# ooowedyn/InkLayer

Hardware: AMD Instinct MI355X
Metric: sketches/sec end-to-end (GroundingDINO+SAM) at 1024x1024 (higher is better)
Workload: dtype f16 (MFMA, f32 accumulate; f32 residual/norm/softmax; split-f16 = fp32-grade operands for patch-embed, neck, mask decoder); 1 GPU; full GroundingDINO Swin-T + SAM ViT-H pipeline, batch=8 per GPU, 1024x1024 synthetic sketches, 16 boxes/sketch, random-init weights; global_batch=8, parallelism=image-parallel x1

## Files before the change

### include/inklayer_hip.h

```cpp
#ifndef INKLAYER_HIP_H
#define INKLAYER_HIP_H

#include <stdint.h>

#ifdef __cplusplus
extern "C" {
#endif

#define INK_ABI_VERSION 10
int ink_abi_version(void);

typedef struct InkGemm {
  const void* A;
  const void* W;
  const float* bias;
  const float* col_scale;
  const float* residual;
  const int32_t* row_map;
  void* C;
  int32_t M, N, K;
  int32_t lda, ldw, ldr, ldc;
  int32_t act;
  int32_t c_f16;
} InkGemm;
#define INK_ACT_NONE 0
#define INK_ACT_GELU 1
#define INK_ACT_RELU 2
int ink_gemm_f16(const InkGemm* p, void* stream);
int ink_gemm_set_variant(int32_t v);
int ink_gemm_query_variant(int32_t M, int32_t N, int32_t K);

int ink_layernorm_rows(const float* x, int64_t ldx, const float* gamma, const float* beta,
                       float eps, const int32_t* gather, int32_t rows_out, int32_t C,
                       void* out_f16, float* out_f32, int64_t ldo, int32_t act, int32_t split,
                       const float* add, int64_t ld_add, const int32_t* add_batch_rows, int32_t rows_per_batch,
                       void* stream);

int ink_add_cvt_f16(const float* a, const float* b, int64_t n_b, void* out_f16, int64_t n,
                    void* stream);
int ink_add_split_f16(const float* a, const float* b, int64_t n_b, void* out_f16, int64_t n, int32_t C,
                      void* stream);
int ink_add_f32(const float* a, const float* b, int64_t n_b, float* out, int64_t n, void* stream);

typedef struct InkAttn {
  const void* Q; const void* K; const void* V;
  void* O;
  int64_t ldq, ldk, ldv, ldo;
  int32_t n_batch, n_heads, n_q, n_k, head_dim;
  float scale;
  int32_t bias_mode;
  int32_t grid_w;
  const int32_t* q_batch_rows;
  const int32_t* kv_batch_rows;
  const float* rel_h; const float* rel_w;
  const void* rel_aug;
  const float* dense_bias; const float* dense_mask;
  int32_t n_mask; int32_t rel_f16;
  const int32_t* tok_rows;
  const void* pad_k; const void* pad_v;
} InkAttn;
int ink_flash_attn(const InkAttn* p, void* stream);

int ink_swin_attn(const void* Q, const void* K, const void* V, int64_t ldq, int64_t ldk, int64_t ldv,
                  void* O, int64_t ldo, int32_t n_windows, int32_t n_heads, int32_t ws, float scale,
                  const float* bias_table, const uint8_t* region, int32_t nW, void* stream);

int ink_relpos_bias64_f16(const void* Q, int64_t ldq, const float* rel_pos_h, const float* rel_pos_w, int32_t n_batch,
                          int32_t n_heads, int32_t head_dim, float scale, void* out_h_f16, void* out_w_f16, void* stream);

int ink_relpos_bias(const void* Q, int64_t ldq, const float* rel_pos_h, const float* rel_pos_w,
                    int32_t S, int32_t n_batch, int32_t n_heads, int32_t head_dim, float scale,
                    const int32_t* tok_rows, float* out_h, float* out_w, void* out_aug_f16,
                    void* stream);

int ink_sam_patchify(const void* image_u8, int32_t h, int32_t w, int32_t L, int32_t P,
                     const float* mean3, const float* std3, int32_t chan_reverse, int32_t split,
                     void* out_f16, void* stream);

int ink_resize_u8(const void* src_u8, int32_t h, int32_t w, int32_t channels, void* dst_u8, int32_t oh, int32_t ow,
                  const int32_t* xbounds, const int32_t* xcoef, int32_t kx, const int32_t* ybounds,
                  const int32_t* ycoef, int32_t ky, void* tmp_u8, void* stream);

int ink_im2col3x3_f16(const void* in_f16, int32_t B, int32_t H, int32_t W, int32_t C, int32_t stride, int32_t relu,
                      void* out_f16, void* stream);

int ink_sam_pe_encode(const float* coords01, const float* gauss, int32_t N, int32_t F,
                      const float* add, int32_t n_add, float* out, void* stream);

int ink_sam_prompt_tokens(const float* points, const int32_t* labels, int32_t n_pts, int32_t pad, const float* boxes,
                          const float* gauss, int32_t F, const float* point_emb, const float* not_a_point,
                          const float* out_tok, float input_size, int32_t P, float* out, void* stream);

int ink_sam_mask_embed(const float* mask, const float* emb, const int32_t* emb_rows, const float* params,
                       int32_t n_params, float eps, int32_t P, int32_t g, float* keys, void* split_f16, void* stream);

int ink_sam_mask_logits(const float* up, const float* hyper, int32_t n, int32_t g, int32_t C,
                        float* out, void* stream);

int ink_sam_postprocess(const float* low, int32_t n, int32_t S, int32_t L, int32_t in_h,
                        int32_t in_w, int32_t out_h, int32_t out_w, float thr, void* out_u8,
                        float* out_logits, void* stream);

int ink_ms_deform_attn_forward(const float* value, const int64_t* spatial_shapes_host,
                               const int64_t* level_start_index_host, const float* sampling_loc,
                               const float* attn_weight, int32_t B, int32_t S, int32_t M, int32_t C,
                               int32_t Q, int32_t L, int32_t P, int32_t im2col_step, float* out,
                               void* stream);

int ink_ms_deform_attn_forward_dev(const void* value, const int64_t* spatial_shapes,
                                   const int64_t* level_start_index, const void* sampling_loc,
                                   const void* attn_weight, int32_t dtype, int32_t B, int32_t S, int32_t M,
                                   int32_t C, int32_t Q, int32_t L, int32_t P, int32_t im2col_step,
                                   void* out, void* stream);
int ink_ms_deform_attn_backward_dev(const void* value, const int64_t* spatial_shapes,
                                    const int64_t* level_start_index, const void* sampling_loc,
                                    const void* attn_weight, const void* grad_output, int32_t dtype,
                                    int32_t B, int32_t S, int32_t M, int32_t C, int32_t Q, int32_t L,
                                    int32_t P, int32_t im2col_step, void* grad_value,
                                    void* grad_sampling_loc, void* grad_attn_weight, void* stream);

int ink_msda_fused(const void* value_f16, const float* proj, int64_t ldp, const float* ref,
                   int32_t ref_dim, int64_t ref_q_stride, int64_t ref_b_stride,
                   const int32_t* shapes_host, int32_t B, int32_t S, int32_t Q, void* out_f16,
                   void* stream);

int ink_swin_patchify(const void* image_u8, int32_t h, int32_t w, const float* mean3,
                      const float* std3, void* out_f16, void* stream);

int ink_layernorm_merge4(const float* x, int64_t ldx, const float* gamma, const float* beta, float eps,
                         const int32_t* gather4, int32_t rows, int32_t C, void* out_f16, void* stream);

int ink_groupnorm_nhwc(const float* x, int32_t B, int32_t T, int32_t C, int32_t G, const float* gamma,
                       const float* beta, float eps, float* stats_ws, float* out,
                       int64_t out_batch_stride, void* stream);

int ink_gather_rows(const float* x, int64_t ldx, int64_t x_batch_rows, const int32_t* idx,
                    int64_t idx_batch_stride, int32_t rows_per_batch, int32_t B, int32_t C,
                    void* out_f16, float* out_f32, void* stream);

int ink_attn_fewkeys(const void* Q, int64_t ldq, const void* K, int64_t ldk, const void* V, int64_t ldv,
                     int32_t B, int32_t n_q, int32_t n_k, int32_t n_heads, int32_t head_dim, float scale,
                     const uint8_t* blocked, const int32_t* q_batch_rows, const float* q_add, int32_t io_f32, void* O,
                     int64_t ldo, void* stream);

int ink_attn_midkeys(const void* Q, int64_t ldq, const void* K, int64_t ldk, const void* V, int64_t ldv, int32_t B,
                     int32_t n_q, int32_t n_k, int32_t n_heads, int32_t head_dim, float scale, const uint8_t* blocked,
                     void* O, int64_t ldo, void* stream);

int ink_biattn_wide_workspace(int32_t B, int32_t S, int32_t T, int64_t* out_floats);
int ink_biattn_wide(const void* QV_f16, const void* KL_f16, int32_t B, int32_t S, int32_t T, int32_t E, float scale,
                    float* ws, void* out_v_f16, void* out_l_f16, void* stream);

int ink_biattn_wide_varlen(const void* QV_f16, const void* KL_f16, int32_t B, int32_t S, int32_t Tmax,
                           const int32_t* t_len , int32_t E, float scale, float* ws,
                           void* out_v_f16, void* out_l_f16 , void* stream);

int ink_attn_midkeys_varlen(const void* Q, int64_t ldq, const void* K, int64_t ldk, const void* V, int64_t ldv,
                            int32_t B, int32_t n_q, int32_t n_k, int32_t n_heads, int32_t head_dim, float scale,
                            const uint8_t* blocked, int64_t blocked_batch_stride, const int32_t* k_len,
                            void* O, int64_t ldo, void* stream);

int ink_text_embed_ln(const int32_t* ids, const int32_t* pos_ids, int32_t R, const float* word, int32_t V,
                      const float* pos, int32_t P, const float* type_row, const float* gamma, const float* beta,
                      float eps, int32_t C, float* out_f32, void* out_split_f16, void* stream);

int ink_attn_text_f32(const float* Q, int64_t ldq, const float* K, int64_t ldk, const float* V, int64_t ldv,
                      const int32_t* row_start , int32_t B, int32_t R, int32_t Tmax,
                      int32_t n_heads, int32_t head_dim, float scale, const uint8_t* blocked,
                      int64_t blocked_batch_stride, void* out_split_f16, int64_t ldo, float* out_f32, int64_t ldf,
                      void* stream);

int ink_attn_fewq(const void* Q, int64_t ldq, const void* K, int64_t ldk, const void* V, int64_t ldv,
                  int32_t n_batch, int32_t n_q, int32_t n_k, int32_t n_heads, int32_t head_dim, float scale,
                  const int32_t* q_batch_rows, const int32_t* kv_batch_rows, const float* k_add, void* O, int64_t ldo,
                  void* stream);

int ink_biattn_colstats(const float* scores, int32_t B, int32_t S, int32_t HT, float* part_ws, float* stats, void* stream);

int ink_fusion_fold_workspace(int32_t B, int32_t S, int64_t* out_floats);
int ink_fusion_fold(float* v_f32, int32_t B, int32_t S, const float* lnv_g, const float* lnv_b, float eps,
                    const float* text_k_f32, const float* text_vl_f32, int64_t ld_text, int32_t T, const void* Wq_f16,
                    const float* bq, const void* Wvv_f16, const float* bvv, const void* Wo_f16, const float* bo,
                    const float* gamma_v, float scale, float* ws, void* out_l_f16, const float* pos, void* out16_pos,
                    void* out16, void* stream);

int ink_sam_upscale_pack(const void* ws_f16, void* blob_f16, void* stream);
int ink_sam_upscale_tail(const float* u0, int64_t ld_tok, int32_t n, int32_t g, const float* ln_g, const float* ln_b, float eps,
                         const void* blob_f16, const float* b3, const float* hyper, int32_t n_masks, float* low,
                         void* stream);

int ink_proj256_ln_pack(const void* ws_f16, void* blob_f16, void* stream);
int ink_proj256_ln(const float* a_f32, const void* blob_f16, const float* bias, const float* res_f32,
                   const int32_t* res_batch_rows, int32_t rows_per_batch, const float* ln_g, const float* ln_b, float eps,
                   int64_t rows, float* out_f32, void* out_split_f16, void* stream);

int ink_ffn256_pack_bytes(int32_t hid, int32_t with_pre, int64_t* out_bytes);
int ink_ffn256_pack(const void* w1_f16, const float* b1, const void* w2_f16, int32_t hid, const void* wpre_f16, void* blob,
                    void* stream);
int ink_ffn256_fused(const void* x_f16, int64_t ldx, const float* res_f32, const void* blob, const float* b2,
                     const float* ln_g, const float* ln_b, float eps, int32_t M, int32_t hid, const float* pre_bias,
                     const float* pre_ln_g, const float* pre_ln_b, float* out_f32, void* stream);

int ink_topk_rowmax(const float* logits, int32_t B, int32_t S, int32_t T, int32_t K, int32_t* out_idx,
                    float* out_val, void* cand_ws, void* stream);

int ink_sine_embed4(const float* ref, const float* dim_t, int32_t N, void* out_f16, void* stream);

int ink_box_refine(const float* delta, int64_t ldd, const float* ref, int32_t N, int32_t ref_is_logit,
                   float* out, void* stream);

int ink_class_scores(const float* logits, int64_t ld_row, const float* pos_map, int64_t pm_image_stride,
                     const int32_t* n_cls, int32_t B, int32_t nq, int32_t T, int32_t C, float* out, void* stream);

int ink_select_boxes(const int32_t* idx, const float* boxes, const float* scale_wh, int32_t B, int32_t K, int32_t nq,
                     int32_t Cmax, float* out_boxes, int32_t* labels, int32_t* query, void* stream);

int ink_mask_cleanup_workspace_ints(int32_t n, int32_t H, int32_t W, int32_t k, int64_t* out_ints);
int ink_mask_cleanup(const void* masks_u8, int32_t n, int32_t H, int32_t W, int32_t k, int32_t area_threshold,
                     double aspect_threshold, void* tmp_a_u8, void* tmp_b_u8, int32_t* workspace, void* out_u8,
                     void* stream);

int ink_mask_sketch_iou_counts(const void* masks_u8, const void* sketch_rgb_u8, int32_t n, int32_t H, int32_t W,
                               void* bits_ws_u64, int32_t* counts, void* stream);

int ink_sam_amg_stats(const float* low, int32_t n, const int32_t* index, int32_t m, const int32_t* m_dev, int32_t S,
                      int32_t L, int32_t in_h, int32_t in_w, int32_t crop_h, int32_t crop_w, double thr, double offset,
                      int32_t x0, int32_t y0, int32_t orig_h, int32_t orig_w, int32_t* table, void* planes_u64,
                      float* out_logits, void* stream);

int ink_mask_rle_counts(const void* planes_u64, const int32_t* select, int32_t k, int32_t H, int32_t W,
                        int32_t* n_counts, void* stream);
int ink_mask_rle_write(const void* planes_u64, const int32_t* select, int32_t k, int32_t H, int32_t W,
                       const int32_t* offsets, int32_t* counts, void* stream);

int ink_mask_small_regions_workspace_ints(int32_t k, int32_t H, int32_t W, int64_t* out_ints);
int ink_mask_small_regions(const void* planes_u64, int32_t k, int32_t H, int32_t W, int32_t min_area, int32_t holes,
                           void* tmp_planes_u64, int32_t* workspace, void* out_planes_u64, int32_t* changed, void* stream);

int ink_box_nms(const float* boxes, const float* scores, int32_t n, float iou_threshold, void* workspace_u64,
                int32_t* keep, int32_t* n_keep, void* stream);

int ink_refine_sketch_planes(const void* rgb_u8, int32_t H, int32_t W, void* planes4_u64, int32_t* max_ws, void* stream);

int ink_bitplane_pack(const void* img_u8, int32_t n, int32_t H, int32_t W, int32_t thresh, void* planes_u64, void* stream);

int ink_refine_depth_samples(const void* mask_planes, int32_t n, const float* depth, const int32_t* pts_yx, int32_t P,
                             int32_t H, int32_t W, float* vals, void* inside_u8, void* stream);

int ink_refine_pair_tables(const void* mask_planes, const void* sketch_planes4, int32_t n, int32_t H, int32_t W,
                           const int32_t* rect, void* dil_ws_planes, int32_t* pair, int32_t* per_mask,
                           int32_t* sketch_area, void* stream);

int ink_refine_composite(const void* mask_planes, const int32_t* order, int32_t n_ranks, int32_t H, int32_t W,
                         void* label_u8, int32_t* hist256, void* stream);

int ink_refine_relabel_clean(const void* label_u8, const void* map256_u8, int32_t H, int32_t W, void* out_label_u8,
                             void* stream);

int ink_refine_grow_workspace(int32_t H, int32_t W, int64_t* plane_words, int64_t* cc_ints);
int ink_refine_grow(const void* label_u8, const void* sketch_planes4, int32_t H, int32_t W, void* planes_ws,
                    int32_t* cc_ws, int32_t* flags256, void* out_label_u8, int32_t* bbox256x4, int32_t* unl_yx,
                    int32_t unl_cap, int32_t* unl_count, void* stream);

int ink_refine_query_dists(const void* label_u8, const int32_t* q_yx, const void* cand256_bits, int32_t Q, int32_t H,
                           int32_t W, int32_t* d2_Qx256, void* stream);

int ink_refine_finalize(void* label_u8, const int32_t* assign_yxl, int32_t A, const void* sketch_planes4, int32_t H,
                        int32_t W, void* planes_ws3, void* extra_plane, int32_t* extra_count, void* stream);

int ink_host_sparse_sample(const uint8_t* rgb_u8, int32_t H, int32_t W, int32_t* out_yx, int32_t cap, int32_t* count);
int ink_host_assign_unlabeled(const int32_t* q_yx, int32_t Q, const int32_t* boxes, int32_t nb, const int32_t* box2mask,
                              const int32_t* d2, const uint8_t* nonempty, int32_t n_masks, int32_t* out_label);

int ink_depth_patchify(const void* image_u8, int32_t H, int32_t W, int32_t nh, int32_t nw, int32_t P, int32_t KP,
                       const double* mean3, const double* std3, int32_t chan_reverse, void* out_f16, void* stream);

int ink_resize_bilinear_ac_nhwc(const float* in, int32_t B, int32_t h, int32_t w, int32_t C, int32_t H, int32_t W,
                                float* out_f32, void* out_f16, void* stream);

int ink_conv3x3_f16(const void* in_f16, int32_t B, int32_t H, int32_t W, int32_t C, const void* wt_f16, int32_t N,
                    const float* bias, int32_t stride, int32_t relu_in, int32_t act, const float* residual, void* out,
                    int32_t out_f16, void* stream);

int ink_layers_otsu_planes(const void* gray_u8, int32_t n, int32_t H, int32_t W, int32_t invert, int32_t* hist,
                           int32_t* thresh, void* out_planes, void* stream);

int ink_layers_dilate(const void* planes, int32_t n, int32_t H, int32_t W, int32_t kernel_size, int32_t iterations,
                      void* tmp_planes, void* out_planes, void* stream);

int ink_layers_border_band(const void* planes, int32_t n, int32_t H, int32_t W, int32_t band, int32_t* flags,
                           void* stream);

int ink_layers_components_workspace_ints(int32_t n, int32_t H, int32_t W, int64_t* out_ints);
int ink_layers_components(const void* planes, int32_t n, int32_t H, int32_t W, int32_t mode, void* tmp_planes3,
                          int32_t* workspace, void* out_planes, void* stream);

int ink_layers_chamfer_workspace_ints(int32_t n, int32_t H, int32_t W, int64_t* out_ints);
int ink_layers_chamfer(const void* mask_planes, const void* stroke_planes, int32_t n, int32_t H, int32_t W,
                       int32_t safety_margin, int32_t full, int32_t* dist, int32_t* workspace, int32_t* min_out,
                       int32_t* shrink_out, void* out_planes, void* stream);

int ink_layers_mask_tables(const void* masks_u8, int32_t n, int32_t H, int32_t W, int32_t* bbox, int32_t* overlap,
                           void* stream);

int ink_layers_assemble(const void* sketch_rgb_u8, const void* masks_u8, const void* bg_planes, const int32_t* bbox,
                        const int32_t* overlap, int32_t n, int32_t H, int32_t W, void* sketch_layers_u8,
                        void* edit_masks_u8, void* debug_u8, void* stream);

int ink_layers_composite(const void* inpainted_rgb_u8, const void* sketch_layer_u8, int32_t H, int32_t W,
                         void* out_rgb_u8, void* stream);

int ink_layers_gray(const void* rgb_u8, int32_t n, int32_t H, int32_t W, void* gray_u8, void* stream);

int ink_layers_rgba(const void* gray_u8, const void* bg_planes, int32_t n, int32_t H, int32_t W, void* rgba_u8,
                    void* stream);


int ink_inp_contrast(const void* rgb_u8, int32_t H, int32_t W, float factor, void* sum_u64, void* out_rgb_u8,
                     void* stream);

int ink_inp_bilateral(const void* rgb_u8, int32_t H, int32_t W, const float* tables, void* out_rgb_u8, void* stream);

int ink_inp_mask_prepare(const void* mask_u8, int32_t H, int32_t W, int32_t dilate_iterations, int32_t blur,
                         void* tmp2_u8, void* out_u8, void* stream);

int ink_inp_condition(const void* rgb_u8, const void* mask_u8, int32_t H, int32_t W, float* out_f32, void* stream);

int ink_inp_cleanup(const void* result_rgb_u8, int32_t H, int32_t W, const float* taps11, float* tmp_f32,
                    void* thresh_u8, void* clean_rgb_u8, void* stream);

int ink_inp_soft_blend(const void* clean_rgb_u8, const void* original_rgb_u8, const void* mask_u8, int32_t H, int32_t W,
                       const double* taps2, double* tmp_f64, void* out_rgb_u8, void* stream);

int ink_inp_luma(const void* rgb_u8, int32_t H, int32_t W, int32_t out_channels, void* out_u8, void* stream);

int ink_inp_unsharp(const void* img_u8, int32_t H, int32_t W, int32_t channels, uint32_t ww, uint32_t fw,
                    int32_t percent, int32_t threshold, void* tmp2_u8, void* out_u8, void* stream);

int ink_inp_rgba_cut(const void* rgb_u8, const void* mask_u8, int32_t H, int32_t W, void* rgba_u8, void* stream);


int ink_vis_gray_min(const void* sketch_u8, int32_t channels, int32_t H, int32_t W, int32_t* gray_min, void* stream);
// ... 23 lines not shown
```

### inklayer_amd/_lib.py

```python
from __future__ import annotations

import ctypes as C
import os
from pathlib import Path

_LIB_PATH = Path(__file__).resolve().parent / "lib" / "libinklayer_hip.so"
_lib = None

c_void_p, c_int, c_i64, c_float = C.c_void_p, C.c_int32, C.c_int64, C.c_float


class InkGemm(C.Structure):
    _fields_ = [
        ("A", c_void_p), ("W", c_void_p), ("bias", c_void_p), ("col_scale", c_void_p),
        ("residual", c_void_p), ("row_map", c_void_p), ("C", c_void_p),
        ("M", c_int), ("N", c_int), ("K", c_int),
        ("lda", c_int), ("ldw", c_int), ("ldr", c_int), ("ldc", c_int),
        ("act", c_int), ("c_f16", c_int),
    ]


class InkAttn(C.Structure):
    _fields_ = [
        ("Q", c_void_p), ("K", c_void_p), ("V", c_void_p), ("O", c_void_p),
        ("ldq", c_i64), ("ldk", c_i64), ("ldv", c_i64), ("ldo", c_i64),
        ("n_batch", c_int), ("n_heads", c_int), ("n_q", c_int), ("n_k", c_int),
        ("head_dim", c_int), ("scale", c_float), ("bias_mode", c_int), ("grid_w", c_int),
        ("q_batch_rows", c_void_p), ("kv_batch_rows", c_void_p),
        ("rel_h", c_void_p), ("rel_w", c_void_p), ("rel_aug", c_void_p),
        ("dense_bias", c_void_p), ("dense_mask", c_void_p), ("n_mask", c_int), ("rel_f16", c_int),
        ("tok_rows", c_void_p), ("pad_k", c_void_p), ("pad_v", c_void_p),
    ]


SIGNATURES = {
    "ink_abi_version": [],
    "ink_gemm_f16": [C.POINTER(InkGemm), c_void_p],
    "ink_gemm_set_variant": [c_int],
    "ink_gemm_query_variant": [c_int, c_int, c_int],
    "ink_layernorm_rows": [c_void_p, c_i64, c_void_p, c_void_p, c_float, c_void_p, c_int, c_int,
                           c_void_p, c_void_p, c_i64, c_int, c_int, c_void_p, c_i64, c_void_p, c_int, c_void_p],
    "ink_add_split_f16": [c_void_p, c_void_p, c_i64, c_void_p, c_i64, c_int, c_void_p],
    "ink_add_cvt_f16": [c_void_p, c_void_p, c_i64, c_void_p, c_i64, c_void_p],
    "ink_add_f32": [c_void_p, c_void_p, c_i64, c_void_p, c_i64, c_void_p],
    "ink_flash_attn": [C.POINTER(InkAttn), c_void_p],
    "ink_swin_attn": [c_void_p, c_void_p, c_void_p, c_i64, c_i64, c_i64, c_void_p, c_i64, c_int, c_int, c_int, c_float,
                      c_void_p, c_void_p, c_int, c_void_p],
    "ink_sam_patchify": [c_void_p, c_int, c_int, c_int, c_int, C.POINTER(c_float), C.POINTER(c_float),
                         c_int, c_int, c_void_p, c_void_p],
    "ink_im2col3x3_f16": [c_void_p, c_int, c_int, c_int, c_int, c_int, c_int, c_void_p, c_void_p],
    "ink_resize_u8": [c_void_p, c_int, c_int, c_int, c_void_p, c_int, c_int, c_void_p, c_void_p, c_int,
                      c_void_p, c_void_p, c_int, c_void_p, c_void_p],
    "ink_sam_pe_encode": [c_void_p, c_void_p, c_int, c_int, c_void_p, c_int, c_void_p, c_void_p],
    "ink_sam_mask_logits": [c_void_p, c_void_p, c_int, c_int, c_int, c_void_p, c_void_p],
    "ink_sam_prompt_tokens": [c_void_p, c_void_p, c_int, c_int, c_void_p, c_void_p, c_int, c_void_p, c_void_p,
                              c_void_p, c_float, c_int, c_void_p, c_void_p],
    "ink_sam_mask_embed": [c_void_p, c_void_p, c_void_p, c_void_p, c_int, c_float, c_int, c_int, c_void_p, c_void_p,
                           c_void_p],
    "ink_sam_postprocess": [c_void_p, c_int, c_int, c_int, c_int, c_int, c_int, c_int, c_float,
                            c_void_p, c_void_p, c_void_p],
    "ink_sam_amg_stats": [c_void_p, c_int, c_void_p, c_int, c_void_p, c_int, c_int, c_int, c_int, c_int, c_int, C.c_double,
                          C.c_double, c_int, c_int, c_int, c_int, c_void_p, c_void_p, c_void_p, c_void_p],
    "ink_mask_rle_counts": [c_void_p, c_void_p, c_int, c_int, c_int, c_void_p, c_void_p],
    "ink_mask_rle_write": [c_void_p, c_void_p, c_int, c_int, c_int, c_void_p, c_void_p, c_void_p],
    "ink_mask_small_regions_workspace_ints": [c_int, c_int, c_int, C.POINTER(c_i64)],
    "ink_mask_small_regions": [c_void_p, c_int, c_int, c_int, c_int, c_int, c_void_p, c_void_p, c_void_p, c_void_p,
                               c_void_p],
    "ink_box_nms": [c_void_p, c_void_p, c_int, c_float, c_void_p, c_void_p, c_void_p, c_void_p],
    "ink_ms_deform_attn_forward": [c_void_p, C.POINTER(c_i64), C.POINTER(c_i64), c_void_p, c_void_p, c_int,
                                   c_int, c_int, c_int, c_int, c_int, c_int, c_int, c_void_p, c_void_p],
    "ink_ms_deform_attn_forward_dev": [c_void_p, c_void_p, c_void_p, c_void_p, c_void_p, c_int, c_int, c_int, c_int,
                                       c_int, c_int, c_int, c_int, c_int, c_void_p, c_void_p],
    "ink_ms_deform_attn_backward_dev": [c_void_p, c_void_p, c_void_p, c_void_p, c_void_p, c_void_p, c_int, c_int, c_int,
                                        c_int, c_int, c_int, c_int, c_int, c_int, c_void_p, c_void_p, c_void_p,
                                        c_void_p],
    "ink_msda_fused": [c_void_p, c_void_p, c_i64, c_void_p, c_int, c_i64, c_i64, C.POINTER(c_int), c_int,
                       c_int, c_int, c_void_p, c_void_p],
    "ink_swin_patchify": [c_void_p, c_int, c_int, C.POINTER(c_float), C.POINTER(c_float), c_void_p, c_void_p],
    "ink_layernorm_merge4": [c_void_p, c_i64, c_void_p, c_void_p, c_float, c_void_p, c_int, c_int, c_void_p,
                             c_void_p],
    "ink_groupnorm_nhwc": [c_void_p, c_int, c_int, c_int, c_int, c_void_p, c_void_p, c_float, c_void_p,
                           c_void_p, c_i64, c_void_p],
    "ink_gather_rows": [c_void_p, c_i64, c_i64, c_void_p, c_i64, c_int, c_int, c_int, c_void_p, c_void_p,
                        c_void_p],
    "ink_biattn_colstats": [c_void_p, c_int, c_int, c_int, c_void_p, c_void_p, c_void_p],
    "ink_fusion_fold_workspace": [c_int, c_int, C.POINTER(c_i64)],
    "ink_relpos_bias64_f16": [c_void_p, c_i64, c_void_p, c_void_p, c_int, c_int, c_int, c_float, c_void_p, c_void_p, c_void_p],
    "ink_proj256_ln_pack": [c_void_p, c_void_p, c_void_p],
    "ink_proj256_ln": [c_void_p, c_void_p, c_void_p, c_void_p, c_void_p, c_int, c_void_p, c_void_p, c_float, c_i64, c_void_p,
                       c_void_p, c_void_p],
    "ink_sam_upscale_pack": [c_void_p, c_void_p, c_void_p],
    "ink_sam_upscale_tail": [c_void_p, c_i64, c_int, c_int, c_void_p, c_void_p, c_float, c_void_p, c_void_p, c_void_p,
                             c_int, c_void_p, c_void_p],
    "ink_ffn256_pack_bytes": [c_int, c_int, C.POINTER(c_i64)],
    "ink_ffn256_pack": [c_void_p, c_void_p, c_void_p, c_int, c_void_p, c_void_p, c_void_p],
    "ink_ffn256_fused": [c_void_p, c_i64, c_void_p, c_void_p, c_void_p, c_void_p, c_void_p, c_float, c_int, c_int,
                         c_void_p, c_void_p, c_void_p, c_void_p, c_void_p],
    "ink_fusion_fold": [c_void_p, c_int, c_int, c_void_p, c_void_p, c_float, c_void_p, c_void_p, c_i64, c_int, c_void_p,
                        c_void_p, c_void_p, c_void_p, c_void_p, c_void_p, c_void_p, c_float, c_void_p, c_void_p, c_void_p,
                        c_void_p, c_void_p, c_void_p],
    "ink_attn_fewkeys": [c_void_p, c_i64, c_void_p, c_i64, c_void_p, c_i64, c_int, c_int, c_int, c_int, c_int,
                         c_float, c_void_p, c_void_p, c_void_p, c_int, c_void_p, c_i64, c_void_p],
    "ink_attn_midkeys": [c_void_p, c_i64, c_void_p, c_i64, c_void_p, c_i64, c_int, c_int, c_int, c_int, c_int,
                         c_float, c_void_p, c_void_p, c_i64, c_void_p],
    "ink_biattn_wide_workspace": [c_int, c_int, c_int, C.POINTER(c_i64)],
    "ink_biattn_wide": [c_void_p, c_void_p, c_int, c_int, c_int, c_int, c_float, c_void_p, c_void_p, c_void_p,
                        c_void_p],
    "ink_biattn_wide_varlen": [c_void_p, c_void_p, c_int, c_int, c_int, c_void_p, c_int, c_float, c_void_p, c_void_p,
                               c_void_p, c_void_p],
    "ink_attn_midkeys_varlen": [c_void_p, c_i64, c_void_p, c_i64, c_void_p, c_i64, c_int, c_int, c_int, c_int, c_int,
                                c_float, c_void_p, c_i64, c_void_p, c_void_p, c_i64, c_void_p],
    "ink_text_embed_ln": [c_void_p, c_void_p, c_int, c_void_p, c_int, c_void_p, c_int, c_void_p, c_void_p, c_void_p,
                          c_float, c_int, c_void_p, c_void_p, c_void_p],
    "ink_attn_text_f32": [c_void_p, c_i64, c_void_p, c_i64, c_void_p, c_i64, c_void_p, c_int, c_int, c_int, c_int, c_int,
                          c_float, c_void_p, c_i64, c_void_p, c_i64, c_void_p, c_i64, c_void_p],
    "ink_attn_fewq": [c_void_p, c_i64, c_void_p, c_i64, c_void_p, c_i64, c_int, c_int, c_int, c_int, c_int,
                      c_float, c_void_p, c_void_p, c_void_p, c_void_p, c_i64, c_void_p],
    "ink_topk_rowmax": [c_void_p, c_int, c_int, c_int, c_int, c_void_p, c_void_p, c_void_p, c_void_p],
    "ink_class_scores": [c_void_p, c_i64, c_void_p, c_i64, c_void_p, c_int, c_int, c_int, c_int, c_void_p, c_void_p],
    "ink_select_boxes": [c_void_p, c_void_p, c_void_p, c_int, c_int, c_int, c_int, c_void_p, c_void_p, c_void_p,
                         c_void_p],
    "ink_sine_embed4": [c_void_p, c_void_p, c_int, c_void_p, c_void_p],
    "ink_box_refine": [c_void_p, c_i64, c_void_p, c_int, c_int, c_void_p, c_void_p],
    "ink_mask_cleanup_workspace_ints": [c_int, c_int, c_int, c_int, C.POINTER(c_i64)],
    "ink_mask_cleanup": [c_void_p, c_int, c_int, c_int, c_int, c_int, C.c_double, c_void_p, c_void_p, c_void_p,
                         c_void_p, c_void_p],
    "ink_mask_sketch_iou_counts": [c_void_p, c_void_p, c_int, c_int, c_int, c_void_p, c_void_p, c_void_p],
    "ink_refine_sketch_planes": [c_void_p, c_int, c_int, c_void_p, c_void_p, c_void_p],
    "ink_bitplane_pack": [c_void_p, c_int, c_int, c_int, c_int, c_void_p, c_void_p],
    "ink_refine_depth_samples": [c_void_p, c_int, c_void_p, c_void_p, c_int, c_int, c_int, c_void_p, c_void_p, c_void_p],
    "ink_refine_pair_tables": [c_void_p, c_void_p, c_int, c_int, c_int, c_void_p, c_void_p, c_void_p, c_void_p,
                               c_void_p, c_void_p],
    "ink_refine_composite": [c_void_p, c_void_p, c_int, c_int, c_int, c_void_p, c_void_p, c_void_p],
    "ink_refine_relabel_clean": [c_void_p, c_void_p, c_int, c_int, c_void_p, c_void_p],
    "ink_refine_grow_workspace": [c_int, c_int, C.POINTER(c_i64), C.POINTER(c_i64)],
    "ink_refine_grow": [c_void_p, c_void_p, c_int, c_int, c_void_p, c_void_p, c_void_p, c_void_p, c_void_p, c_void_p,
                        c_int, c_void_p, c_void_p],
    "ink_refine_query_dists": [c_void_p, c_void_p, c_void_p, c_int, c_int, c_int, c_void_p, c_void_p],
    "ink_refine_finalize": [c_void_p, c_void_p, c_int, c_void_p, c_int, c_int, c_void_p, c_void_p, c_void_p, c_void_p],
    "ink_host_sparse_sample": [c_void_p, c_int, c_int, c_void_p, c_int, c_void_p],
    "ink_host_assign_unlabeled": [c_void_p, c_int, c_void_p, c_int, c_void_p, c_void_p, c_void_p, c_int, c_void_p],
    "ink_depth_patchify": [c_void_p, c_int, c_int, c_int, c_int, c_int, c_int, C.POINTER(C.c_double), C.POINTER(C.c_double),
                           c_int, c_void_p, c_void_p],
    "ink_resize_bilinear_ac_nhwc": [c_void_p, c_int, c_int, c_int, c_int, c_int, c_int, c_void_p, c_void_p, c_void_p],
    "ink_conv3x3_f16": [c_void_p, c_int, c_int, c_int, c_int, c_void_p, c_int, c_void_p, c_int, c_int, c_int, c_void_p,
                        c_void_p, c_int, c_void_p],
    "ink_layers_otsu_planes": [c_void_p, c_int, c_int, c_int, c_int, c_void_p, c_void_p, c_void_p, c_void_p],
    "ink_layers_dilate": [c_void_p, c_int, c_int, c_int, c_int, c_int, c_void_p, c_void_p, c_void_p],
    "ink_layers_border_band": [c_void_p, c_int, c_int, c_int, c_int, c_void_p, c_void_p],
    "ink_layers_components_workspace_ints": [c_int, c_int, c_int, C.POINTER(c_i64)],
    "ink_layers_components": [c_void_p, c_int, c_int, c_int, c_int, c_void_p, c_void_p, c_void_p, c_void_p],
    "ink_layers_chamfer_workspace_ints": [c_int, c_int, c_int, C.POINTER(c_i64)],
    "ink_layers_chamfer": [c_void_p, c_void_p, c_int, c_int, c_int, c_int, c_int, c_void_p, c_void_p, c_void_p, c_void_p,
                           c_void_p, c_void_p],
    "ink_layers_mask_tables": [c_void_p, c_int, c_int, c_int, c_void_p, c_void_p, c_void_p],
    "ink_layers_assemble": [c_void_p, c_void_p, c_void_p, c_void_p, c_void_p, c_int, c_int, c_int, c_void_p, c_void_p,
                            c_void_p, c_void_p],
    "ink_layers_composite": [c_void_p, c_void_p, c_int, c_int, c_void_p, c_void_p],
    "ink_layers_gray": [c_void_p, c_int, c_int, c_int, c_void_p, c_void_p],
    "ink_layers_rgba": [c_void_p, c_void_p, c_int, c_int, c_int, c_void_p, c_void_p],
    "ink_inp_contrast": [c_void_p, c_int, c_int, c_float, c_void_p, c_void_p, c_void_p],
    "ink_inp_bilateral": [c_void_p, c_int, c_int, c_void_p, c_void_p, c_void_p],
    "ink_inp_mask_prepare": [c_void_p, c_int, c_int, c_int, c_int, c_void_p, c_void_p, c_void_p],
    "ink_inp_condition": [c_void_p, c_void_p, c_int, c_int, c_void_p, c_void_p],
    "ink_inp_cleanup": [c_void_p, c_int, c_int, c_void_p, c_void_p, c_void_p, c_void_p, c_void_p],
    "ink_inp_soft_blend": [c_void_p, c_void_p, c_void_p, c_int, c_int, c_void_p, c_void_p, c_void_p, c_void_p],
    "ink_inp_luma": [c_void_p, c_int, c_int, c_int, c_void_p, c_void_p],
    "ink_inp_unsharp": [c_void_p, c_int, c_int, c_int, C.c_uint32, C.c_uint32, c_int, c_int, c_void_p, c_void_p, c_void_p],
    "ink_inp_rgba_cut": [c_void_p, c_void_p, c_int, c_int, c_void_p, c_void_p],
    "ink_vis_gray_min": [c_void_p, c_int, c_int, c_int, c_void_p, c_void_p],
    "ink_vis_colour": [c_void_p, c_int, c_void_p, c_int, c_int, c_void_p, c_void_p, c_int, c_int, c_void_p, c_void_p],
    "ink_eval_label_ranks": [c_void_p, c_int, c_int, c_int, c_void_p, c_void_p, c_int, c_void_p, c_void_p, c_void_p],
    "ink_eval_contingency": [c_void_p, c_int, c_int, c_void_p, c_int, c_void_p, c_int, c_int, c_int, c_int, c_void_p,
                             c_void_p],
    "ink_eval_label_boxes": [c_void_p, c_int, c_int, c_int, c_void_p, c_void_p],
    "ink_eval_paint_labels": [c_void_p, c_void_p, c_int, c_int, c_int, c_void_p, c_void_p],
    "ink_relpos_bias": [c_void_p, c_i64, c_void_p, c_void_p, c_int, c_int, c_int, c_int, c_float,
                        c_void_p, c_void_p, c_void_p, c_void_p, c_void_p],
}


class InkLayerHipError(RuntimeError):
    pass


def lib_path() -> Path:
    return Path(os.environ.get("INKLAYER_HIP_LIB", _LIB_PATH))


def lib() -> C.CDLL:
    global _lib
    if _lib is None:
        p = lib_path()
        if not p.exists():
            raise InkLayerHipError(
                f"{p} not found: build it with `python -m inklayer_amd.build` "
                "(there is no CPU/eager fallback for the InkLayer hot path)")
        try:
            import torch
        except ImportError:
            pass
        l = C.CDLL(str(p))
        for name, argtypes in SIGNATURES.items():
            fn = getattr(l, name)
            fn.argtypes = argtypes
            fn.restype = C.c_int
        _lib = l
    return _lib


def check(rc: int, what: str) -> None:
    if rc != 0:
        raise InkLayerHipError(f"{what} failed: " + {1: "bad argument", 2: "HIP launch error"}.get(rc, str(rc)))
```

### inklayer_amd/csrc/gemm.hip

```cpp
#include <stdlib.h>

#include "mfma_util.h"
#include "../../include/inklayer_hip.h"

namespace {

template <int BK> struct Swz;
template <> struct Swz<64> {
  static __device__ __forceinline__ int f(int row) { return row & 7; }
};
template <> struct Swz<32> {
  static __device__ __forceinline__ int f(int row) { return (-(row >> 2)) & 3; }
};

__device__ __forceinline__ bool residual_preloaded(const InkGemm& p) {
  return p.residual && p.act == INK_ACT_NONE && !p.col_scale;
}

template <int TM>
__device__ __forceinline__ void wave_rows(int (&rows)[TM], const InkGemm& p, int mw, int lane) {
#pragma unroll
  for (int ti = 0; ti < TM; ++ti) {
    const int m = mw + ti * 16 + (lane & 15);
    int r = -1;
    if (m < p.M) r = p.row_map ? p.row_map[m] : m;
    rows[ti] = r;
  }
}

template <int TM, int TN>
__device__ __forceinline__ void init_wave_tile(f32x4 (&acc)[TM][TN], const InkGemm& p, const int (&rows)[TM], int nw,
                                               int lane) {
  const int fq = lane >> 4;
  const bool pre = residual_preloaded(p);
#pragma unroll
  for (int ti = 0; ti < TM; ++ti) {
    const int r = pre ? rows[ti] : -1;
    const float* rp = p.residual + (size_t)max(r, 0) * p.ldr + nw + fq * 4;
#pragma unroll
    for (int j = 0; j < TN; ++j) {
      acc[ti][j] = (f32x4){0.f, 0.f, 0.f, 0.f};
      if (r >= 0 && nw + j * 16 + fq * 4 < p.N) acc[ti][j] = *(const f32x4*)(rp + j * 16);
    }
  }
}

template <int TM, int TN>
__device__ __forceinline__ void add_bias_wave_tile(f32x4 (&acc)[TM][TN], const InkGemm& p, int nw, int lane) {
  const int fq = lane >> 4;
#pragma unroll
  for (int j = 0; j < TN; ++j) {
    const int n = nw + j * 16 + fq * 4;
    f32x4 bv = (f32x4){0.f, 0.f, 0.f, 0.f};
    if (p.bias && n < p.N) bv = *(const f32x4*)(p.bias + n);
#pragma unroll
    for (int ti = 0; ti < TM; ++ti) acc[ti][j] += bv;
  }
}

template <int TM, int TN, int OUT, int MODE = -1>
__device__ __forceinline__ void store_wave_tile(f32x4 (&acc)[TM][TN], const InkGemm& p, char* er,
                                                const int (&rows)[TM], int nw, int lane) {
  constexpr bool F16O = OUT == 1;
  constexpr int WNC = TN * 16, EP = WNC * 4 + 16;
  constexpr int ES = OUT == 0 ? 4 : 8;
  constexpr int CPRW = WNC / ES;
  constexpr int NIT = (16 * CPRW + 63) / 64;
  const int fr = lane & 15, fq = lane >> 4;
  const bool wide16 = OUT != 0 && (p.ldc % 8 == 0);
  const bool res_late = MODE < 0 && p.residual && !residual_preloaded(p);
  const int act = MODE < 0 ? p.act : MODE;
  const bool scaled = MODE < 0 && p.col_scale != nullptr;
  int row_of[NIT], n_of[NIT];
#pragma unroll
  for (int it = 0; it < NIT; ++it) {
    const int c = it * 64 + lane;
    row_of[it] = c < 16 * CPRW ? c / CPRW : 16;
    n_of[it] = nw + (c % CPRW) * ES;
  }

  add_bias_wave_tile<TM, TN>(acc, p, nw, lane);

#pragma unroll
  for (int ti = 0; ti < TM; ++ti) {
#pragma unroll
    for (int j = 0; j < TN; ++j) {
      f32x4 v = acc[ti][j];
      if (act == INK_ACT_GELU) {
#pragma unroll
        for (int r = 0; r < 4; ++r) v[r] = gelu_erf(v[r]);
      } else if (act == INK_ACT_RELU) {
#pragma unroll
        for (int r = 0; r < 4; ++r) v[r] = fmaxf(v[r], 0.f);
      }
      if (scaled) {
        const int n = nw + j * 16 + fq * 4;
        if (n < p.N) v *= *(const f32x4*)(p.col_scale + n);
      }
      if (F16O) {
        *(f16x4*)(er + fr * EP + (j * 16 + fq * 4) * 2) = (f16x4){(f16)v[0], (f16)v[1], (f16)v[2], (f16)v[3]};
      } else {
        *(f32x4*)(er + fr * EP + (j * 16 + fq * 4) * 4) = v;
      }
    }
#pragma unroll
    for (int it = 0; it < NIT; ++it) {
      int r = __builtin_amdgcn_ds_bpermute((row_of[it] & 15) << 2, rows[ti]);
      if (row_of[it] >= 16 || n_of[it] >= p.N) r = -1;
      if (r >= 0) {
        const int c_n = n_of[it];
        const char* src = er + row_of[it] * EP + (c_n - nw) * (F16O ? 2 : 4);
        if (F16O) {
          f16x8 d = *(const f16x8*)src;
          f16* dst = (f16*)p.C + (size_t)r * p.ldc + c_n;
          if (res_late) {
            const float* rp = p.residual + (size_t)r * p.ldr + c_n;
#pragma unroll
            for (int e = 0; e < 8; ++e)
              if (c_n + e < p.N) d[e] = (f16)((float)d[e] + rp[e]);
          }
          if (wide16 && c_n + 8 <= p.N) {
            *(f16x8*)dst = d;
          } else {
            *(f16x4*)dst = (f16x4){d[0], d[1], d[2], d[3]};
            if (c_n + 8 <= p.N) *(f16x4*)(dst + 4) = (f16x4){d[4], d[5], d[6], d[7]};
          }
        } else {
          f32x4 d = *(const f32x4*)src;
          if (res_late) d += *(const f32x4*)(p.residual + (size_t)r * p.ldr + c_n);
          *(f32x4*)((float*)p.C + (size_t)r * p.ldc + c_n) = d;
        }
      }
    }
  }
}

__device__ __forceinline__ void tile_of(int id, int ntm, int ntn, int group_m, int& mt, int& nt) {
  if (group_m > 1) {
    const int per = group_m * ntn;
    const int first = (id / per) * group_m;
    const int gsz = min(ntm - first, group_m);
    mt = first + (id % per) % gsz;
    nt = (id % per) / gsz;
  } else {
    mt = id / ntn;
    nt = id % ntn;
  }
}

constexpr int NS = 2;
template <int BM, int BN, int BK, int WM, int WN>
__global__ __launch_bounds__(WM * WN * 64) void gemm_f16_nt(InkGemm p, int group_m) {
  constexpr int NT = WM * WN * 64;
  constexpr int CPR = BK / 8;
  constexpr int ROWB = BK * 2;
  constexpr int TILE_A = BM * ROWB, TILE_W = BN * ROWB;
  constexpr int STAGE = TILE_A + TILE_W;
  constexpr int IT_A = (BM * CPR) / NT, IT_W = (BN * CPR) / NT;
  constexpr int TM = BM / WM / 16, TN = BN / WN / 16;
  static_assert((BM * CPR) % NT == 0 && (BN * CPR) % NT == 0, "tile/threads mismatch");
  extern __shared__ __attribute__((aligned(16))) char smem[];

  const int tid = threadIdx.x;
  const int lane = tid & 63;
  const int wave = tid >> 6;
  const int wm = wave / WN, wn = wave % WN;

  const int ntn = (p.N + BN - 1) / BN;
  const int ntm = (p.M + BM - 1) / BM;
  int mt, nt;
  tile_of(xcd_remap(blockIdx.x, ntm * ntn), ntm, ntn, group_m, mt, nt);
  const int m0 = mt * BM;
  const int n0 = nt * BN;

  const f16* __restrict__ A = (const f16*)p.A;
  const f16* __restrict__ W = (const f16*)p.W;

  const f16* srcA[IT_A];
  const f16* srcW[IT_W];
#pragma unroll
  for (int it = 0; it < IT_A; ++it) {
    const int pch = it * NT + tid;
    const int row = pch / CPR;
    const int lch = (pch % CPR) ^ Swz<BK>::f(row);
    srcA[it] = A + (size_t)min(m0 + row, p.M - 1) * p.lda + lch * 8;
  }
#pragma unroll
  for (int it = 0; it < IT_W; ++it) {
    const int pch = it * NT + tid;
    const int row = pch / CPR;
    const int lch = (pch % CPR) ^ Swz<BK>::f(row);
    srcW[it] = W + (size_t)min(n0 + row, p.N - 1) * p.ldw + lch * 8;
  }

  auto stage = [&](int buf, int kt) {
    char* base = smem + buf * STAGE;
#pragma unroll
    for (int it = 0; it < IT_A; ++it)
      __builtin_amdgcn_global_load_lds((gptr_t)(srcA[it] + kt * BK), (lptr_t)(base + (it * NT + wave * 64) * 16), 16, 0, 0);
#pragma unroll
    for (int it = 0; it < IT_W; ++it)
      __builtin_amdgcn_global_load_lds((gptr_t)(srcW[it] + kt * BK), (lptr_t)(base + TILE_A + (it * NT + wave * 64) * 16), 16, 0, 0);
  };

  int rows[TM];
  wave_rows<TM>(rows, p, m0 + wm * (BM / WM), lane);
  f32x4 acc[TM][TN];

  const int fr = lane & 15, fq = lane >> 4;
  const int offA = (wm * (BM / WM) + fr) * ROWB;
  const int offW = (wn * (BN / WN) + fr) * ROWB;
  const int swz = Swz<BK>::f(fr);

  const int nk = p.K / BK;
  auto compute = [&](int cur) {
    const char* bA = smem + cur * STAGE;
    const char* bW = bA + TILE_A;
#pragma unroll
    for (int kk = 0; kk < BK / 32; ++kk) {
      constexpr int AG = TM > 4 ? 4 : TM;
      f16x8 a[AG], w[TN];
      const int co = ((kk * 4 + fq) ^ swz) << 4;
#pragma unroll
      for (int j = 0; j < TN; ++j) w[j] = *(const f16x8*)(bW + offW + j * 16 * ROWB + co);
#pragma unroll
      for (int i0 = 0; i0 < TM; i0 += AG) {
#pragma unroll
        for (int i = 0; i < AG; ++i) a[i] = *(const f16x8*)(bA + offA + (i0 + i) * 16 * ROWB + co);
#pragma unroll
        for (int i = 0; i < AG; ++i)
#pragma unroll
          for (int j = 0; j < TN; ++j)
            acc[i0 + i][j] = __builtin_amdgcn_mfma_f32_16x16x32_f16(w[j], a[i], acc[i0 + i][j], 0, 0, 0);
      }
    }
  };

  stage(0, 0);
  init_wave_tile<TM, TN>(acc, p, rows, n0 + wn * (BN / WN), lane);
  for (int kt = 0; kt < nk; ++kt) {
    asm volatile("s_waitcnt vmcnt(0)" ::: "memory");
    __syncthreads();
    if (kt + 1 < nk) stage((kt + 1) & 1, kt + 1);
    compute(kt & 1);
  }

  constexpr int WNC = BN / WN;
  constexpr int EP = WNC * 4 + 16;
  static_assert(WM * WN * 16 * EP <= NS * STAGE, "epilogue patch must fit in the staging LDS");
  __syncthreads();
  char* er = smem + wave * (16 * EP);
  if (p.c_f16 == 1) {
    store_wave_tile<TM, TN, 1>(acc, p, er, rows, n0 + wn * WNC, lane);
  } else {
    store_wave_tile<TM, TN, 0>(acc, p, er, rows, n0 + wn * WNC, lane);
  }
}

constexpr int PP_RING = 4, PP_TN = 5;
__global__ __launch_bounds__(512) void gemm_f16_nt_pp(InkGemm p, int group_m) {
  constexpr int RING = PP_RING, TN = PP_TN;
  constexpr int BM = 256, BN = 64 * TN, BK = 32, NT = 512;
  constexpr int CPR = BK / 8, ROWB = BK * 2;
  constexpr int TILE_A = BM * ROWB, TILE_W = BN * ROWB, GRAN = TILE_A + TILE_W;
  constexpr int IT_A = (BM * CPR) / NT, IT_W = (BN * CPR) / NT;
  constexpr bool W_TAIL = (BN * CPR) % NT != 0;
  static_assert(!W_TAIL || (BN * CPR) % NT == NT / 2, "tail is exactly the first four waves");
  constexpr int LOADS = IT_A + IT_W;
  constexpr int TM = 8, WNC = 16 * TN;
  constexpr int AHEAD = RING - 2;
  constexpr int AG = 4;
  constexpr int EP = WNC * 4 + 16;
  static_assert(8 * 16 * EP <= RING * GRAN, "patch fits");
  extern __shared__ __attribute__((aligned(16))) char smem[];
  const int tid = threadIdx.x, lane = tid & 63;
  const int wave = __builtin_amdgcn_readfirstlane(tid >> 6);
  const int grp = wave >> 2, wn = wave & 3;
  const int fr = lane & 15, fq = lane >> 4;

  const int ntn = (p.N + BN - 1) / BN, ntm = (p.M + BM - 1) / BM;
  int mt, nt;
  tile_of(xcd_remap(blockIdx.x, ntm * ntn), ntm, ntn, group_m, mt, nt);
  const int m0 = mt * BM, n0 = nt * BN;
  const int G = p.K / BK;
  const f16* __restrict__ A = (const f16*)p.A;
  const f16* __restrict__ W = (const f16*)p.W;
  const f16* srcA[IT_A];
  const f16* srcW[IT_W + (W_TAIL ? 1 : 0)];
#pragma unroll
  for (int it = 0; it < IT_A; ++it) {
    const int pch = it * NT + tid, row = pch / CPR, lch = (pch % CPR) ^ Swz<BK>::f(row);
    srcA[it] = A + (size_t)min(m0 + row, p.M - 1) * p.lda + lch * 8;
  }
#pragma unroll
  for (int it = 0; it < IT_W + (W_TAIL ? 1 : 0); ++it) {
    const int pch = it * NT + tid, row = min(pch / CPR, BN - 1), lch = (pch % CPR) ^ Swz<BK>::f(row);
    srcW[it] = W + (size_t)min(n0 + row, p.N - 1) * p.ldw + lch * 8;
  }
  auto dma = [&](int g, int slot) {
    char* base = smem + slot * GRAN;
#pragma unroll
    for (int it = 0; it < IT_A; ++it)
      __builtin_amdgcn_global_load_lds((gptr_t)(srcA[it] + g * BK), (lptr_t)(base + (it * NT + wave * 64) * 16), 16, 0, 0);
#pragma unroll
    for (int it = 0; it < IT_W; ++it)
      __builtin_amdgcn_global_load_lds((gptr_t)(srcW[it] + g * BK), (lptr_t)(base + TILE_A + (it * NT + wave * 64) * 16), 16, 0, 0);
    if (W_TAIL && grp == 0)
      __builtin_amdgcn_global_load_lds((gptr_t)(srcW[IT_W] + g * BK), (lptr_t)(base + TILE_A + (IT_W * NT + wave * 64) * 16), 16, 0, 0);
  };
  auto wait_ahead = [&]() {
    if (W_TAIL && grp == 0) {
      asm volatile("s_waitcnt vmcnt(%0)" ::"n"((AHEAD - 1) * (LOADS + 1)) : "memory");
    } else {
      asm volatile("s_waitcnt vmcnt(%0)" ::"n"((AHEAD - 1) * LOADS) : "memory");
    }
  };
  auto slot_end = [&]() {
    __builtin_amdgcn_sched_barrier(0);
    __builtin_amdgcn_s_barrier();
    __builtin_amdgcn_sched_barrier(0);
  };

  int rows[TM];
  wave_rows<TM>(rows, p, m0 + grp * 128, lane);
#pragma unroll
  for (int g = 0; g < AHEAD; ++g) dma(g, g);
  f32x4 acc[TM][TN];
  init_wave_tile<TM, TN>(acc, p, rows, n0 + wn * WNC, lane);
  if (residual_preloaded(p)) {
    asm volatile("s_waitcnt vmcnt(0)" ::: "memory");
  } else {
    wait_ahead();
  }
  slot_end();
  if (grp == 1) slot_end();

  const int offA = (grp * 128 + fr) * ROWB;
  const int offW = (wn * WNC + fr) * ROWB;
  const int co = (fq ^ Swz<BK>::f(fr)) << 4;
  f16x8 a[AG], w[TN];
  int cslot = 0, islot = AHEAD % RING;
  auto iter = [&](int g) __attribute__((always_inline)) {
    const char* bA = smem + cslot * GRAN;
    const char* bW = bA + TILE_A;
#pragma unroll
    for (int i = 0; i < AG; ++i) a[i] = *(const f16x8*)(bA + offA + i * 16 * ROWB + co);
#pragma unroll
    for (int j = 0; j < TN; ++j) w[j] = *(const f16x8*)(bW + offW + j * 16 * ROWB + co);
    if (g + AHEAD < G) {
      dma(g + AHEAD, islot);
      wait_ahead();
    } else {
      asm volatile("s_waitcnt vmcnt(0)" ::: "memory");
    }
    slot_end();
    asm volatile("s_waitcnt lgkmcnt(0)" ::: "memory");
    __builtin_amdgcn_sched_barrier(0);
    __builtin_amdgcn_s_setprio(1);
#pragma unroll
    for (int i0 = 0; i0 < TM; i0 += AG) {
#pragma unroll
      for (int i = 0; i < AG; ++i) {
#pragma unroll
        for (int j = 0; j < TN; ++j)
          acc[i0 + i][j] = __builtin_amdgcn_mfma_f32_16x16x32_f16(w[j], a[i], acc[i0 + i][j], 0, 0, 0);
        if (i0 + AG < TM) {
          a[i] = *(const f16x8*)(bA + offA + (i0 + AG + i) * 16 * ROWB + co);
          __builtin_amdgcn_sched_barrier(0);
        }
      }
    }
    __builtin_amdgcn_s_setprio(0);
    slot_end();
    cslot = (cslot + 1 == RING) ? 0 : cslot + 1;
    islot = (islot + 1 == RING) ? 0 : islot + 1;
  };
  for (int g = 0; g < G; ++g) iter(g);
  if (grp == 0) slot_end();

  char* er = smem + wave * (16 * EP);
  const bool plain = !p.col_scale && !(p.residual && !residual_preloaded(p));
  if (p.c_f16) {
    if (plain && p.act == INK_ACT_GELU) {
      store_wave_tile<TM, TN, 1, INK_ACT_GELU>(acc, p, er, rows, n0 + wn * WNC, lane);
    } else if (plain && p.act == INK_ACT_NONE) {
      store_wave_tile<TM, TN, 1, INK_ACT_NONE>(acc, p, er, rows, n0 + wn * WNC, lane);
    } else {
      store_wave_tile<TM, TN, 1>(acc, p, er, rows, n0 + wn * WNC, lane);
    }
  } else {
    if (plain && p.act == INK_ACT_NONE) {
      store_wave_tile<TM, TN, 0, INK_ACT_NONE>(acc, p, er, rows, n0 + wn * WNC, lane);
    } else {
      store_wave_tile<TM, TN, 0>(acc, p, er, rows, n0 + wn * WNC, lane);
    }
  }
}

static int launch_gemm_pp(const InkGemm& p, hipStream_t s, int group_m) {
  if (p.K / 32 < PP_RING) return INK_ERR_ARG;
  constexpr int BN = 64 * PP_TN;
  constexpr int lds = PP_RING * (256 + BN) * 32 * 2;
  static_assert(lds <= 160 * 1024, "LDS budget");
  ink_dyn_lds<gemm_f16_nt_pp>(lds);
  const int ntiles = ((p.M + 255) / 256) * ((p.N + BN - 1) / BN);
  hipLaunchKernelGGL(gemm_f16_nt_pp, dim3(ntiles), dim3(512), lds, s, p, group_m);
  return ink_launch_status();
}

template <int BM, int BN, int BK, int WM, int WN>
static int launch_gemm(const InkGemm& p, hipStream_t s, int group_m = 1) {
  constexpr int lds = NS * (BM + BN) * BK * 2;
  static_assert(lds <= 160 * 1024, "LDS budget");
  ink_dyn_lds<gemm_f16_nt<BM, BN, BK, WM, WN>>(lds);
  const int ntm = (p.M + BM - 1) / BM, ntn = (p.N + BN - 1) / BN;
  hipLaunchKernelGGL((gemm_f16_nt<BM, BN, BK, WM, WN>), dim3(ntm * ntn), dim3(WM * WN * 64), lds, s, p, group_m);
  return ink_launch_status();
}

struct ConvGeom {
  int H, W, C, OH, OW, stride;
};
__device__ __attribute__((aligned(128))) const uint32_t g_conv_zero_row[32] = {};

template <int BK, bool RELU_IN>
__global__ __launch_bounds__(256) void conv3x3_f16_nt(InkGemm p, ConvGeom g) {
  constexpr int BM = 128, BN = 128, WM = 2, WN = 2;
  constexpr int NT = WM * WN * 64;
  constexpr int CPR = BK / 8;
  constexpr int ROWB = BK * 2;
  constexpr int TILE_A = BM * ROWB, TILE_W = BN * ROWB;
  constexpr int STAGE = TILE_A + TILE_W;
  constexpr int IT_A = (BM * CPR) / NT, IT_W = (BN * CPR) / NT;
  constexpr int TM = BM / WM / 16, TN = BN / WN / 16;
  extern __shared__ __attribute__((aligned(16))) char smem[];

  const int tid = threadIdx.x;
  const int lane = tid & 63;
  const int wave = tid >> 6;
  const int wm = wave / WN, wn = wave % WN;

  const int ntn = (p.N + BN - 1) / BN;
  const int ntm = (p.M + BM - 1) / BM;
  int mt, nt;
  tile_of(xcd_remap(blockIdx.x, ntm * ntn), ntm, ntn, 1, mt, nt);
  const int m0 = mt * BM;
  const int n0 = nt * BN;

  const f16* __restrict__ A = (const f16*)p.A;
  const f16* __restrict__ W = (const f16*)p.W;

  const f16* ctrA[IT_A];
  const f16* zeroA[IT_A];
  int maskA[IT_A];
  const f16* srcW[IT_W];
#pragma unroll
  for (int it = 0; it < IT_A; ++it) {
    const int pch = it * NT + tid;
    const int row = pch / CPR;
    const int lch = (pch % CPR) ^ Swz<BK>::f(row);
    const int m = min(m0 + row, p.M - 1);
    const int b = m / (g.OH * g.OW);
    const int rem = m - b * (g.OH * g.OW);
    const int oy = rem / g.OW;
    const int iy = oy * g.stride, ix = (rem - oy * g.OW) * g.stride;
    ctrA[it] = A + (((size_t)b * g.H + iy) * g.W + ix) * g.C + lch * 8;
    zeroA[it] = (const f16*)g_conv_zero_row + lch * 8;
    const int rowok = (iy > 0 ? 1 : 0) | 2 | (iy + 1 < g.H ? 4 : 0);
    const int colok = (ix > 0 ? 1 : 0) | 2 | (ix + 1 < g.W ? 4 : 0);
    int mask = 0;
#pragma unroll
    for (int ky = 0; ky < 3; ++ky)
      if ((rowok >> ky) & 1) mask |= colok << (ky * 3);
    maskA[it] = mask;
  }
#pragma unroll
  for (int it = 0; it < IT_W; ++it) {
    const int pch = it * NT + tid;
    const int row = pch / CPR;
    const int lch = (pch % CPR) ^ Swz<BK>::f(row);
    srcW[it] = W + (size_t)min(n0 + row, p.N - 1) * p.ldw + lch * 8;
  }

  int s_tap = 0, s_c0 = 0;
  auto stage = [&](int buf, int kt) {
    char* base = smem + buf * STAGE;
    const int ky = s_tap / 3, kx = s_tap - ky * 3;
    const ptrdiff_t doff = ((ptrdiff_t)(ky - 1) * g.W + (kx - 1)) * g.C + s_c0;
#pragma unroll
    for (int it = 0; it < IT_A; ++it) {
      const f16* src = ((maskA[it] >> s_tap) & 1) ? ctrA[it] + doff : zeroA[it];
      __builtin_amdgcn_global_load_lds((gptr_t)src, (lptr_t)(base + (it * NT + wave * 64) * 16), 16, 0, 0);
    }
#pragma unroll
    for (int it = 0; it < IT_W; ++it)
      __builtin_amdgcn_global_load_lds((gptr_t)(srcW[it] + kt * BK), (lptr_t)(base + TILE_A + (it * NT + wave * 64) * 16), 16, 0, 0);
    s_c0 += BK;
    if (s_c0 == g.C) {
      s_c0 = 0;
      ++s_tap;
    }
  };

  int rows[TM];
  wave_rows<TM>(rows, p, m0 + wm * (BM / WM), lane);
  f32x4 acc[TM][TN];

  const int fr = lane & 15, fq = lane >> 4;
  const int offA = (wm * (BM / WM) + fr) * ROWB;
  const int offW = (wn * (BN / WN) + fr) * ROWB;
  const int swz = Swz<BK>::f(fr);

  const int nk = p.K / BK;
  auto compute = [&](int cur) {
    const char* bA = smem + cur * STAGE;
    const char* bW = bA + TILE_A;
#pragma unroll
    for (int kk = 0; kk < BK / 32; ++kk) {
      f16x8 a[TM], w[TN];
      const int co = ((kk * 4 + fq) ^ swz) << 4;
#pragma unroll
      for (int j = 0; j < TN; ++j) w[j] = *(const f16x8*)(bW + offW + j * 16 * ROWB + co);
#pragma unroll
      for (int i = 0; i < TM; ++i) {
        a[i] = *(const f16x8*)(bA + offA + i * 16 * ROWB + co);
        if (RELU_IN) a[i] = __builtin_elementwise_max(a[i], (f16x8)(f16)0);
      }
#pragma unroll
      for (int i = 0; i < TM; ++i)
#pragma unroll
        for (int j = 0; j < TN; ++j)
          acc[i][j] = __builtin_amdgcn_mfma_f32_16x16x32_f16(w[j], a[i], acc[i][j], 0, 0, 0);
    }
  };

  stage(0, 0);
  init_wave_tile<TM, TN>(acc, p, rows, n0 + wn * (BN / WN), lane);
  for (int kt = 0; kt < nk; ++kt) {
    asm volatile("s_waitcnt vmcnt(0)" ::: "memory");
    __syncthreads();
    if (kt + 1 < nk) stage((kt + 1) & 1, kt + 1);
    compute(kt & 1);
  }

  constexpr int WNC = BN / WN;
  constexpr int EP = WNC * 4 + 16;
  static_assert(WM * WN * 16 * EP <= NS * STAGE, "epilogue patch must fit in the staging LDS");
  __syncthreads();
  char* er = smem + wave * (16 * EP);
  if (p.c_f16 == 1) {
    store_wave_tile<TM, TN, 1>(acc, p, er, rows, n0 + wn * WNC, lane);
  } else {
    store_wave_tile<TM, TN, 0>(acc, p, er, rows, n0 + wn * WNC, lane);
  }
}

template <int BK, bool RELU_IN>
static int launch_conv3x3(const InkGemm& p, const ConvGeom& g, hipStream_t s) {
  constexpr int lds = NS * (128 + 128) * BK * 2;
  ink_dyn_lds<conv3x3_f16_nt<BK, RELU_IN>>(lds);
  const int ntm = (p.M + 127) / 128, ntn = (p.N + 127) / 128;
  hipLaunchKernelGGL((conv3x3_f16_nt<BK, RELU_IN>), dim3(ntm * ntn), dim3(256), lds, s, p, g);
  return ink_launch_status();
}

}

extern "C" int ink_conv3x3_f16(const void* in_f16, int32_t B, int32_t H, int32_t W, int32_t C, const void* wt_f16,
                               int32_t N, const float* bias, int32_t stride, int32_t relu_in, int32_t act,
                               const float* residual, void* out, int32_t out_f16, void* stream) {
  INK_CHECK_ARG(in_f16 && wt_f16 && out);
  INK_CHECK_ARG(B > 0 && H > 0 && W > 0 && C > 0 && N > 0);
  INK_CHECK_ARG(C % 32 == 0 && N % 4 == 0);
  INK_CHECK_ARG(stride == 1 || stride == 2);
  INK_CHECK_ARG(ink_aligned<16>(in_f16, wt_f16, out, residual, bias));
  INK_CHECK_ARG(relu_in == 0 || relu_in == 1);
  INK_CHECK_ARG(act == INK_ACT_NONE || act == INK_ACT_RELU);
  INK_CHECK_ARG(out_f16 == 0 || out_f16 == 1);
  const int OH = (H - 1) / stride + 1, OW = (W - 1) / stride + 1;
  const int64_t M = (int64_t)B * OH * OW;
  INK_CHECK_ARG(M <= INT32_MAX - 128 && (int64_t)9 * C <= INT32_MAX);
  InkGemm p = {};
  p.A = in_f16;
  p.W = wt_f16;
  p.bias = bias;
  p.residual = residual;
  p.C = out;
  p.M = (int32_t)M;
  p.N = N;
  p.K = 9 * C;
  p.lda = p.ldw = 9 * C;
  p.ldr = p.ldc = N;
  p.act = act;
  p.c_f16 = out_f16;
  const ConvGeom g = {H, W, C, OH, OW, stride};
  hipStream_t s = (hipStream_t)stream;
  if (C % 64 == 0) return relu_in ? launch_conv3x3<64, true>(p, g, s) : launch_conv3x3<64, false>(p, g, s);
  return relu_in ? launch_conv3x3<32, true>(p, g, s) : launch_conv3x3<32, false>(p, g, s);
}

static int g_variant = -1;
extern "C" int ink_gemm_query_variant(int32_t M, int32_t N, int32_t K) {
  if (K % 64 != 0) return 32;
  if (N % 320 == 0 && K >= 128 && (long)((M + 255) / 256) * (N / 320) >= 384) return 45;
  const long tiles256 = (long)((M + 255) / 256) * ((N + 255) / 256);
  const bool n_fits = (N % 256 == 0) || N >= 1024;
  return (tiles256 >= 200 && n_fits) ? 10 : 0;
}
extern "C" int ink_abi_version(void) { return INK_ABI_VERSION; }
extern "C" int ink_gemm_set_variant(int32_t v) {
  INK_CHECK_ARG(v == -1 || v == 0 || v == 10 || v == 45);
  g_variant = v;
  return INK_OK;
}

extern "C" int ink_gemm_f16(const InkGemm* pp, void* stream) {
  INK_CHECK_ARG(pp != nullptr);
  const InkGemm& p = *pp;
  INK_CHECK_ARG(p.A && p.W && p.C);
  INK_CHECK_ARG(p.M > 0 && p.N > 0 && p.K > 0);
  INK_CHECK_ARG(p.K % 32 == 0 && p.N % 4 == 0);
  INK_CHECK_ARG(p.lda % 8 == 0 && p.ldw % 8 == 0 && p.lda >= p.K && p.ldw >= p.K);
  INK_CHECK_ARG(p.ldc % 4 == 0 && p.ldc >= p.N);
  INK_CHECK_ARG(!p.residual || (p.ldr % 4 == 0 && p.ldr >= p.N));
  INK_CHECK_ARG(ink_aligned<16>(p.A, p.W, p.C));
  INK_CHECK_ARG(p.act >= 0 && p.act <= 2);
  INK_CHECK_ARG(p.c_f16 == 0 || p.c_f16 == 1);
  hipStream_t s = (hipStream_t)stream;
  if (p.K % 64 != 0) return launch_gemm<128, 128, 32, 2, 2>(p, s);
  int v = g_variant;
  if (v < 0) v = ink_gemm_query_variant(p.M, p.N, p.K);
  switch (v) {
    case 10: return launch_gemm<256, 256, 64, 4, 4>(p, s, 4);
    case 45: return launch_gemm_pp(p, s, 4);
    default: return launch_gemm<128, 128, 64, 2, 2>(p, s);
  }
}
```

### inklayer_amd/csrc/norm.hip

```cpp
#include "common.h"
#include "../../include/inklayer_hip.h"

namespace {

template <int NV>
__global__ __launch_bounds__(256) void layernorm_rows_kernel(
    const float* __restrict__ x, int64_t ldx, const float* __restrict__ gamma,
    const float* __restrict__ beta, float eps, const int32_t* __restrict__ gather, int rows_out,
    int C, f16* __restrict__ out_h, float* __restrict__ out_f, int64_t ldo, int act, int split,
    const float* __restrict__ add, int64_t ld_add, const int32_t* __restrict__ add_batch_rows, int rows_per_batch) {
  const int lane = threadIdx.x & 63;
  const int row = blockIdx.x * 4 + (threadIdx.x >> 6);
  if (row >= rows_out) return;
  const int nv = C >> 2;
  const int64_t ldf = split ? ldo / 3 : ldo;
  const int src = gather ? gather[row] : row;
  if (src < 0) {
    for (int v = lane; v < nv; v += 64) {
      if (out_h && split) split_store(out_h + row * ldo + v * 4, C, (f32x4){0.f, 0.f, 0.f, 0.f});
      else if (out_h) *(f16x4*)(out_h + row * ldo + v * 4) = (f16x4){0, 0, 0, 0};
      if (out_f) *(f32x4*)(out_f + row * ldf + v * 4) = (f32x4){0.f, 0.f, 0.f, 0.f};
    }
    return;
  }
  const float* xr = x + (int64_t)src * ldx;
  const float* ar = nullptr;
  if (add) {
    const int b = row / rows_per_batch, i = row - b * rows_per_batch;
    ar = add + ((int64_t)(add_batch_rows ? add_batch_rows[b] : b * rows_per_batch) + i) * ld_add;
  }
  f32x4 r[NV];
  float s = 0.f;
#pragma unroll
  for (int j = 0; j < NV; ++j) {
    const int v = lane + 64 * j;
    r[j] = v < nv ? *(const f32x4*)(xr + v * 4) : (f32x4){0.f, 0.f, 0.f, 0.f};
    if (ar && v < nv) r[j] += *(const f32x4*)(ar + v * 4);
    s += (r[j][0] + r[j][1]) + (r[j][2] + r[j][3]);
  }
  const float mean = wave_sum(s) / (float)C;
  float q = 0.f;
#pragma unroll
  for (int j = 0; j < NV; ++j) {
    const int v = lane + 64 * j;
    if (v < nv) {
      const f32x4 d = r[j] - mean;
      q += (d[0] * d[0] + d[1] * d[1]) + (d[2] * d[2] + d[3] * d[3]);
    }
  }
  const float rstd = 1.0f / sqrtf(wave_sum(q) / (float)C + eps);
#pragma unroll
  for (int j = 0; j < NV; ++j) {
    const int v = lane + 64 * j;
    if (v < nv) {
      f32x4 y = (r[j] - mean) * rstd;
      if (gamma) y *= *(const f32x4*)(gamma + v * 4);
      if (beta) y += *(const f32x4*)(beta + v * 4);
      if (act == INK_ACT_GELU) {
#pragma unroll
        for (int e = 0; e < 4; ++e) y[e] = gelu_erf(y[e]);
      }
      if (out_h && split) split_store(out_h + row * ldo + v * 4, C, y);
      else if (out_h) *(f16x4*)(out_h + row * ldo + v * 4) = (f16x4){(f16)y[0], (f16)y[1], (f16)y[2], (f16)y[3]};
      if (out_f) *(f32x4*)(out_f + row * ldf + v * 4) = y;
    }
  }
}

__global__ __launch_bounds__(256) void add_split_f16_kernel(const float* __restrict__ a,
                                                            const float* __restrict__ b,
                                                            f16* __restrict__ o, int64_t n4, int64_t nb4,
                                                            int C) {
  const int c4n = C >> 2;
  for (int64_t i = blockIdx.x * 256 + threadIdx.x; i < n4; i += (int64_t)gridDim.x * 256) {
    f32x4 v = *(const f32x4*)(a + i * 4);
    if (b) v += *(const f32x4*)(b + (i % nb4) * 4);
    const int64_t row = i / c4n;
    const int c = (int)(i - row * c4n) * 4;
    split_store(o + row * 3 * C + c, C, v);
  }
}

__global__ __launch_bounds__(256) void add_cvt_f16_kernel(const float* __restrict__ a,
                                                          const float* __restrict__ b,
                                                          f16* __restrict__ o,
                                                          float* __restrict__ of, int64_t n4,
                                                          int64_t nb4) {
  for (int64_t i = blockIdx.x * 256 + threadIdx.x; i < n4; i += (int64_t)gridDim.x * 256) {
    f32x4 v = *(const f32x4*)(a + i * 4);
    if (b) v += *(const f32x4*)(b + (i % nb4) * 4);
    if (o) *(f16x4*)(o + i * 4) = (f16x4){(f16)v[0], (f16)v[1], (f16)v[2], (f16)v[3]};
    if (of) *(f32x4*)(of + i * 4) = v;
  }
}

}

extern "C" int ink_layernorm_rows(const float* x, int64_t ldx, const float* gamma,
                                  const float* beta, float eps, const int32_t* gather,
                                  int32_t rows_out, int32_t C, void* out_f16, float* out_f32,
                                  int64_t ldo, int32_t act, int32_t split, const float* add, int64_t ld_add,
                                  const int32_t* add_batch_rows, int32_t rows_per_batch, void* stream) {
  INK_CHECK_ARG(x && (out_f16 || out_f32));
  INK_CHECK_ARG(!add || (!gather && rows_per_batch > 0 && ld_add >= C && ld_add % 4 == 0));
  INK_CHECK_ARG(split == 0 || (split == 1 && out_f16 && ldo >= 3 * (int64_t)C && (!out_f32 || ldo % 12 == 0)));
  INK_CHECK_ARG(act == INK_ACT_NONE || act == INK_ACT_GELU);
  INK_CHECK_ARG(rows_out > 0 && C > 0 && C % 4 == 0 && C <= 2048);
  INK_CHECK_ARG(ldx % 4 == 0 && ldo % 4 == 0 && ldx >= C && ldo >= C);
  const dim3 grid((rows_out + 3) / 4), block(256);
  hipStream_t s = (hipStream_t)stream;
  const int nv = (C / 4 + 63) / 64;
#define INK_LN(NV)                                                                          \
  hipLaunchKernelGGL(layernorm_rows_kernel<NV>, grid, block, 0, s, x, ldx, gamma, beta, eps, \
                     gather, rows_out, C, (f16*)out_f16, out_f32, ldo, act, split, add, ld_add, add_batch_rows, \
                     rows_per_batch)
  switch (nv) {
    case 1: INK_LN(1); break;
    case 2: INK_LN(2); break;
    case 3: INK_LN(3); break;
    case 4: INK_LN(4); break;
    case 5: INK_LN(5); break;
    default: INK_LN(8); break;
  }
#undef INK_LN
  return ink_launch_status();
}

extern "C" int ink_add_cvt_f16(const float* a, const float* b, int64_t n_b, void* out_f16,
                               int64_t n, void* stream) {
  INK_CHECK_ARG(a && out_f16 && n > 0 && n % 4 == 0);
  INK_CHECK_ARG(!b || (n_b > 0 && n_b % 4 == 0 && n % n_b == 0));
  const int64_t n4 = n / 4;
  const int blocks = (int)((n4 + 255) / 256 < 2048 ? (n4 + 255) / 256 : 2048);
  hipLaunchKernelGGL(add_cvt_f16_kernel, dim3(blocks), dim3(256), 0, (hipStream_t)stream, a, b,
                     (f16*)out_f16, (float*)nullptr, n4, b ? n_b / 4 : 1);
  return ink_launch_status();
}

extern "C" int ink_add_split_f16(const float* a, const float* b, int64_t n_b, void* out_f16, int64_t n,
                                 int32_t C, void* stream) {
  INK_CHECK_ARG(a && out_f16 && n > 0 && C > 0 && C % 4 == 0 && n % C == 0);
  INK_CHECK_ARG(!b || (n_b > 0 && n_b % 4 == 0 && n % n_b == 0));
  const int64_t n4 = n / 4;
  const int blocks = (int)((n4 + 255) / 256 < 4096 ? (n4 + 255) / 256 : 4096);
  hipLaunchKernelGGL(add_split_f16_kernel, dim3(blocks), dim3(256), 0, (hipStream_t)stream, a, b,
                     (f16*)out_f16, n4, b ? n_b / 4 : 1, C);
  return ink_launch_status();
}

extern "C" int ink_add_f32(const float* a, const float* b, int64_t n_b, float* out, int64_t n,
                           void* stream) {
  INK_CHECK_ARG(a && out && n > 0 && n % 4 == 0);
  INK_CHECK_ARG(!b || (n_b > 0 && n_b % 4 == 0 && n % n_b == 0));
  const int64_t n4 = n / 4;
  const int blocks = (int)((n4 + 255) / 256 < 2048 ? (n4 + 255) / 256 : 2048);
  hipLaunchKernelGGL(add_cvt_f16_kernel, dim3(blocks), dim3(256), 0, (hipStream_t)stream, a, b,
                     (f16*)nullptr, out, n4, b ? n_b / 4 : 1);
  return ink_launch_status();
}
```

### inklayer_amd/gdino.py

```python
from __future__ import annotations

import math
from dataclasses import dataclass, replace
from typing import Dict, List, NamedTuple, Optional, Sequence, Tuple

import numpy as np
import torch

from . import ops
from ._lru import LRU

F16, F32, I32 = torch.float16, torch.float32, torch.int32


@dataclass
class GDinoConfig:
    embed_dim: int = 96
    depths: Tuple[int, ...] = (2, 2, 6, 2)
    num_heads: Tuple[int, ...] = (3, 6, 12, 24)
    window_size: int = 7
    out_indices: Tuple[int, ...] = (1, 2, 3)
    hidden_dim: int = 256
    nheads: int = 8
    enc_layers: int = 6
# ... 2 lines not shown
    num_queries: int = 900
    num_feature_levels: int = 4
    n_points: int = 4
    max_text_len: int = 256
    pe_temperature: float = 20.0
    box_threshold: float = 0.2
    pixel_mean: Tuple[float, ...] = (0.485, 0.456, 0.406)
    pixel_std: Tuple[float, ...] = (0.229, 0.224, 0.225)


GDINO_CONFIGS: Dict[str, GDinoConfig] = {
    "swin_T_224_1k": GDinoConfig(),
    "swin_B_224_22k": GDinoConfig(embed_dim=128, depths=(2, 2, 18, 2), num_heads=(4, 8, 16, 32), window_size=7),
    "swin_B_384_22k": GDinoConfig(embed_dim=128, depths=(2, 2, 18, 2), num_heads=(4, 8, 16, 32), window_size=12),
}
GDINO_ALIASES = {"swin_t": "swin_T_224_1k", "swin_b": "swin_B_384_22k"}
WINDOW_SIZES = (7, 12)
HEAD_DIM = 32


def config_for(name: str) -> GDinoConfig:
    key = GDINO_ALIASES.get(name, name)
    if key not in GDINO_CONFIGS:
        raise ValueError(f"unknown GroundingDINO model {name!r}: one of {sorted(GDINO_CONFIGS) + sorted(GDINO_ALIASES)}")
    return replace(GDINO_CONFIGS[key])


def model_name(cfg: GDinoConfig) -> Optional[str]:
    key = (cfg.embed_dim, tuple(cfg.depths), tuple(cfg.num_heads), cfg.window_size)
    return next((n for n, c in GDINO_CONFIGS.items()
                 if (c.embed_dim, tuple(c.depths), tuple(c.num_heads), c.window_size) == key), None)


def check_config(cfg: GDinoConfig) -> None:
    widths = [cfg.embed_dim * 2 ** i / nh for i, nh in enumerate(cfg.num_heads)]
    if len(cfg.depths) != len(cfg.num_heads) or any(wd != HEAD_DIM for wd in widths):
        raise ValueError(f"no kernels for this Swin backbone: head widths {widths} (embed dim {cfg.embed_dim}, heads "
                         f"{tuple(cfg.num_heads)}, depths {tuple(cfg.depths)}); the window attention kernels serve head "
                         f"width {HEAD_DIM}")
    if cfg.window_size not in WINDOW_SIZES:
        raise ValueError(f"no kernels for this Swin backbone: window size {cfg.window_size}; the window attention "
                         f"kernels serve {' and '.join(map(str, WINDOW_SIZES))}")
    if cfg.embed_dim * 2 ** (len(cfg.depths) - 1) > 2048:
        raise ValueError(f"no kernels for this Swin backbone: {cfg.embed_dim * 2 ** (len(cfg.depths) - 1)} channels in "
                         f"the last stage; the row LayerNorm serves at most 2048 (and the patch merging half of that)")
    if (cfg.hidden_dim, cfg.nheads, cfg.num_feature_levels, cfg.n_points) != (256, 8, 4, 4):
        raise ValueError(f"no kernels for this detector transformer: hidden_dim {cfg.hidden_dim}, nheads {cfg.nheads}, "
                         f"num_feature_levels {cfg.num_feature_levels}, n_points {cfg.n_points}; the kernels serve "
                         f"hidden_dim 256, 8 heads, 4 levels, 4 points")


def config_from_state_dict(sd) -> GDinoConfig:
    sd = clean_state_dict(sd)

    def shape(k):
        if k not in sd:
            raise ValueError(f"not a GroundingDINO state dict: {k} is missing")
        v = sd[k]
        return tuple(int(d) for d in (v.shape if hasattr(v, "shape") else v))

    def count(prefix):
        ids = {int(k[len(prefix):].split(".", 1)[0]) for k in sd if k.startswith(prefix)}
        if ids != set(range(len(ids))):
            raise ValueError(f"not a GroundingDINO state dict: {prefix}* holds indices {sorted(ids)}")
        return len(ids)

    bb, t = "backbone.0.", "transformer."
    C0 = shape(bb + "patch_embed.proj.weight")[0]
    depths = tuple(count(f"{bb}layers.{i}.blocks.") for i in range(count(bb + "layers.")))
    if not depths or 0 in depths:
        raise ValueError(f"not a GroundingDINO state dict: Swin stage depths {depths}")
    tabs = [[shape(f"{bb}layers.{i}.blocks.{b}.attn.relative_position_bias_table") for b in range(d)]
            for i, d in enumerate(depths)]
    flat = [tb for st in tabs for tb in st]
    sides = sorted({math.isqrt(tb[0]) for tb in flat})
    heads = tuple(st[0][1] for st in tabs)
    if (any(len(tb) != 2 for tb in flat) or any(tb[1] != st[0][1] for st in tabs for tb in st) or len(sides) != 1
            or sides[0] ** 2 != flat[0][0] or sides[0] % 2 == 0):
        raise ValueError(f"inconsistent Swin backbone: relative_position_bias_table shapes {sorted(set(flat))}")
    ws = (sides[0] + 1) // 2
    out_indices = tuple(i for i in range(len(depths)) if f"{bb}norm{i}.weight" in sd)
    lv = shape(t + "level_embed")
    so = shape(t + "encoder.layers.0.self_attn.sampling_offsets.weight")
    cfg = GDinoConfig(embed_dim=C0, depths=depths, num_heads=heads, window_size=ws, out_indices=out_indices,
                      hidden_dim=lv[1], num_feature_levels=lv[0], enc_layers=count(t + "encoder.layers."),
                      dec_layers=count(t + "decoder.layers."), num_queries=shape(t + "tgt_embed.weight")[0],
                      dim_feedforward=shape(t + "encoder.layers.0.linear1.weight")[0])
    check_config(cfg)
    if so != (cfg.nheads * lv[0] * cfg.n_points * 2, lv[1]):
        raise ValueError(f"no kernels for this detector transformer: sampling_offsets.weight has shape {so}, not "
                         f"{(cfg.nheads * lv[0] * cfg.n_points * 2, lv[1])} (8 heads x 4 levels x 4 points x 2)")
    return cfg


DEFAULT_TOKEN_IDS = (101, 4874, 1012, 102)
SPECIAL_TOKENS = (101, 102, 1012, 1029)


def resize_shape(w: int, h: int, size: int = 800, max_size: int = 1333) -> Tuple[int, int]:
    mn, mx = float(min(w, h)), float(max(w, h))
    if mx / mn * size > max_size:
        size = int(round(max_size * mn / mx))
    if (w <= h and w == size) or (h <= w and h == size):
        return h, w
    if w < h:
        return int(size * h / w), size
    return size, int(size * w / h)


def resize_for_detector(image_rgb: np.ndarray) -> np.ndarray:
    from PIL import Image
    im = Image.fromarray(image_rgb)
    oh, ow = resize_shape(im.size[0], im.size[1])
    if (ow, oh) != im.size:
        im = im.resize((ow, oh), Image.BILINEAR)
    return np.ascontiguousarray(np.asarray(im))


def text_masks_and_position_ids(input_ids: Sequence[int], special: Sequence[int] = SPECIAL_TOKENS):
    n = len(input_ids)
    attn = torch.eye(n, dtype=torch.bool)
    pos = torch.zeros(n, dtype=torch.long)
    prev = 0
    for col, tok in enumerate(input_ids):
        if tok not in special:
            continue
        if col == 0 or col == n - 1:
            attn[col, col] = True
            pos[col] = 0
        else:
            attn[prev + 1: col + 1, prev + 1: col + 1] = True
            pos[prev + 1: col + 1] = torch.arange(0, col - prev)
        prev = col
    return attn, pos


SEPARATOR_TOKENS = (101, 102, 1012)


def phrase_token_ids(posmap: Sequence[bool], token_ids: Sequence[int], left_idx: int = 0, right_idx: int = 255) -> List[int]:
    return [int(token_ids[i]) for i, on in enumerate(posmap) if on and left_idx < i < right_idx]


def phrases_from_probs(probs: torch.Tensor, token_ids: Sequence[int], text_threshold: float,
                       remove_combined: bool = False, tokenizer=None) -> list:
    import bisect
    T = len(token_ids)
    sep_idx = [i for i, t in enumerate(token_ids) if t in SEPARATOR_TOKENS]
    out = []
    for row in probs:
        posmap = (row > text_threshold).tolist()
        left, right = 0, 255
        if remove_combined:
            at = bisect.bisect_left(sep_idx, int(row.argmax()))
            right = sep_idx[at] if at < len(sep_idx) else T
            left = sep_idx[at - 1]
        ids = phrase_token_ids(posmap, token_ids, left, right)
        out.append(tokenizer.decode(ids).replace(".", "") if tokenizer is not None
                   else tuple(t for t in ids if t != 1012))
    return out


def _interleaved_sincos(v: torch.Tensor) -> torch.Tensor:
    return torch.stack((v[..., 0::2].sin(), v[..., 1::2].cos()), dim=-1).flatten(-2)


class _Plan:

    def __init__(self, eng: "GDinoEngine", h: int, w: int, B: int):
        cfg, dev = eng.cfg, eng.dev
        ws, sh = cfg.window_size, cfg.window_size // 2
        self.B = B
        H, W = -(-h // 4), -(-w // 4)
        self.stage_hw: List[Tuple[int, int]] = []
        self.win_map: List[List[torch.Tensor]] = []
        self.nW: List[int] = []
        self.shift_mask: List[torch.Tensor] = []
        self.region: List[torch.Tensor] = []
        self.merge_map: List[Optional[torch.Tensor]] = []
        scale = HEAD_DIM ** -0.5
        for i in range(len(cfg.depths)):
            self.stage_hw.append((H, W))
            Hp, Wp = -(-H // ws) * ws, -(-W // ws) * ws
            nW = (Hp // ws) * (Wp // ws)
            self.nW.append(nW)
            wy, wx, iy, ix = torch.meshgrid(torch.arange(Hp // ws), torch.arange(Wp // ws), torch.arange(ws),
                                            torch.arange(ws), indexing="ij")
            maps = []
            for shift in (0, sh):
                y = (wy * ws + iy + shift) % Hp
                x = (wx * ws + ix + shift) % Wp
                tok = torch.where((y < H) & (x < W), y * W + x, torch.full_like(y, -1)).reshape(-1)
                full = torch.cat([torch.where(tok >= 0, tok + b * H * W, tok) for b in range(B)])
                maps.append(full.to(I32).to(dev))
            self.win_map.append(maps)
            mw = swin_regions(Hp, Wp, ws)
            if ws == 7:
                diff = mw[:, None, :] - mw[:, :, None]
                m = torch.zeros((nW, ws * ws, 64))
                m[:, :, :ws * ws] = torch.where(diff != 0, torch.tensor(-100.0), torch.tensor(0.0)) / scale
                self.shift_mask.append(m.to(dev).contiguous())
            else:
                self.region.append(mw.to(torch.uint8).to(dev).contiguous())
            if i < len(cfg.depths) - 1:
                H2, W2 = (H + 1) // 2, (W + 1) // 2
                y2, x2 = torch.meshgrid(torch.arange(H2), torch.arange(W2), indexing="ij")
                cols = []
                for dy, dx in ((0, 0), (1, 0), (0, 1), (1, 1)):
                    yy, xx = 2 * y2 + dy, 2 * x2 + dx
                    cols.append(torch.where((yy < H) & (xx < W), yy * W + xx, torch.full_like(yy, -1)).reshape(-1))
                g4 = torch.stack(cols, -1)
                full = torch.cat([torch.where(g4 >= 0, g4 + b * H * W, g4) for b in range(B)])
                self.merge_map.append(full.to(I32).contiguous().to(dev))
                H, W = H2, W2
            else:
                self.merge_map.append(None)
        shapes = [self.stage_hw[i] for i in cfg.out_indices]
        H3, W3 = shapes[-1]
        for _ in range(cfg.num_feature_levels - len(shapes)):
            shapes.append(((shapes[-1][0] - 1) // 2 + 1, (shapes[-1][1] - 1) // 2 + 1))
        self.shapes = shapes
        self.S = sum(a * b for a, b in shapes)
        starts = np.cumsum([0] + [a * b for a, b in shapes])[:-1]
        self.level_start = [int(s) for s in starts]
        H4, W4 = shapes[len(cfg.out_indices)]
        y4, x4, ky, kx = torch.meshgrid(torch.arange(H4), torch.arange(W4), torch.arange(3), torch.arange(3),
                                        indexing="ij")
        yy, xx = 2 * y4 + ky - 1, 2 * x4 + kx - 1
        self.lvl4_map = torch.where((yy >= 0) & (yy < H3) & (xx >= 0) & (xx < W3), yy * W3 + xx,
                                    torch.full_like(yy, -1)).reshape(-1).to(I32).to(dev)
        npf = cfg.hidden_dim // 2
        dim_t = torch.arange(npf, dtype=torch.float32)
        dim_t = cfg.pe_temperature ** (2 * torch.div(dim_t, 2, rounding_mode="floor") / npf)
        pos = []
        for l, (hh, ww) in enumerate(shapes):
            ye = torch.arange(1, hh + 1, dtype=torch.float32)[:, None].expand(hh, ww) / (float(hh) + 1e-6) * (2 * math.pi)
            xe = torch.arange(1, ww + 1, dtype=torch.float32)[None, :].expand(hh, ww) / (float(ww) + 1e-6) * (2 * math.pi)
            px, py = _interleaved_sincos(xe[:, :, None] / dim_t), _interleaved_sincos(ye[:, :, None] / dim_t)
            pos.append(torch.cat((py, px), dim=2).reshape(hh * ww, 2 * npf) + eng.level_embed_cpu[l])
        self.pos = torch.cat(pos, 0).to(dev).contiguous()
        refs, props = [], []
        for lvl, (hh, ww) in enumerate(shapes):
            ry, rx = torch.meshgrid(torch.linspace(0.5, hh - 0.5, hh), torch.linspace(0.5, ww - 0.5, ww), indexing="ij")
            refs.append(torch.stack((rx.reshape(-1) / ww, ry.reshape(-1) / hh), -1))
            gy, gx = torch.meshgrid(torch.linspace(0, hh - 1, hh), torch.linspace(0, ww - 1, ww), indexing="ij")
            grid = (torch.stack((gx, gy), -1) + 0.5) / torch.tensor([float(ww), float(hh)])
            props.append(torch.cat((grid, torch.ones_like(grid) * 0.05 * (2.0 ** lvl)), -1).view(-1, 4))
        self.enc_ref = torch.cat(refs, 0).to(dev).contiguous()
        pr = torch.cat(props, 0)
        valid = ((pr > 0.01) & (pr < 0.99)).all(-1)
        pr = torch.log(pr / (1 - pr)).masked_fill(~valid[:, None], float("inf"))
        self.props_unsig = pr.to(dev).contiguous()
        self.valid_map = torch.where(valid, torch.arange(self.S), torch.full((self.S,), -1)).to(I32).to(dev)


def swin_regions(Hp: int, Wp: int, ws: int) -> torch.Tensor:
    sh = ws // 2
    img = torch.zeros((Hp, Wp))
    cnt = 0
    for hs in (slice(0, -ws), slice(-ws, -sh), slice(-sh, None)):
        for wsl in (slice(0, -ws), slice(-ws, -sh), slice(-sh, None)):
            img[hs, wsl] = cnt
            cnt += 1
    return img.view(Hp // ws, ws, Wp // ws, ws).permute(0, 2, 1, 3).reshape(-1, ws * ws)


def swin_dense_bias(table: torch.Tensor, ws: int, nh: int, scale: float) -> torch.Tensor:
    co = torch.stack(torch.meshgrid(torch.arange(ws), torch.arange(ws), indexing="ij")).flatten(1)
    rel = (co[:, :, None] - co[:, None, :]).permute(1, 2, 0).contiguous()
    rel[:, :, 0] += ws - 1
    rel[:, :, 1] += ws - 1
    rel[:, :, 0] *= 2 * ws - 1
    rel_index = rel.sum(-1).view(-1)
    bias = torch.zeros((nh, ws * ws, 64))
    bias[:, :, :ws * ws] = table[rel_index].view(ws * ws, ws * ws, nh).permute(2, 0, 1) / scale
    return bias


def swin_bias_table(table: torch.Tensor, ws: int, nh: int) -> torch.Tensor:
    assert tuple(table.shape) == ((2 * ws - 1) ** 2, nh)
    return table.to(torch.float32).t().contiguous()


def clean_state_dict(sd: Dict[str, torch.Tensor]) -> Dict[str, torch.Tensor]:
    if any(k.startswith("module.") for k in sd):
        return {(k[7:] if k.startswith("module.") else k): v for k, v in sd.items()}
    return sd


class _TextBatch(NamedTuple):
    text0: torch.Tensor
    t_len: torch.Tensor
    blocked: torch.Tensor
    pos_text: torch.Tensor
    bias: torch.Tensor
    Tmax: int
    Tc: int


class GDinoEngine:
    fuse_ffn = True
    fuse_ffn_pre = True
    fold_fusion = True

    def __init__(self, state_dict: Dict[str, torch.Tensor], cfg: Optional[GDinoConfig] = None,
                 device: str | torch.device = "cuda", encoded_text: Optional[torch.Tensor] = None,
                 token_ids: Sequence[int] = DEFAULT_TOKEN_IDS):
        cfg = cfg or GDinoConfig()
        self.cfg, self.dev = cfg, torch.device(device)
        assert self.dev.type == "cuda", "the InkLayer detector runs on MI355X only"
        check_config(cfg)
        sd, dev = clean_state_dict(state_dict), self.dev
        self.w: Dict[str, torch.Tensor] = {}
        w = self.w

        def h(name, shape=None):
            t = sd[name].detach().to(torch.float32)
            return (t.reshape(shape) if shape is not None else t).to(dev, F16).contiguous()

        def f(name):
            return ops.own_f32(sd[name], dev)

        def lin(dst, src):
            w[dst + ".w"], w[dst + ".b"] = h(src + ".weight"), f(src + ".bias")

        def ln(dst, src):
            w[dst + ".w"], w[dst + ".b"] = f(src + ".weight"), f(src + ".bias")

        def cat_lin(dst, srcs):
            w[dst + ".w"] = torch.cat([h(s + ".weight") for s in srcs]).contiguous()
            w[dst + ".b"] = torch.cat([f(s + ".bias") for s in srcs]).contiguous()

        bb = "backbone.0."
        pw = sd[bb + "patch_embed.proj.weight"].detach().to(torch.float32).cpu().reshape(cfg.embed_dim, 48)
        w["pe.w"] = torch.cat([pw, torch.zeros(cfg.embed_dim, 16)], 1).to(dev, F16).contiguous()
        w["pe.b"] = f(bb + "patch_embed.proj.bias")
        ln("pe.norm", bb + "patch_embed.norm")
        ws = cfg.window_size
        scale = HEAD_DIM ** -0.5
        for i, (dep, nh) in enumerate(zip(cfg.depths, cfg.num_heads)):
            for b in range(dep):
                p, d = f"{bb}layers.{i}.blocks.{b}.", f"s{i}b{b}"
                ln(d + ".norm1", p + "norm1")
                ln(d + ".norm2", p + "norm2")
                lin(d + ".qkv", p + "attn.qkv")
                lin(d + ".proj", p + "attn.proj")
                lin(d + ".fc1", p + "mlp.fc1")
                lin(d + ".fc2", p + "mlp.fc2")
                tab = sd[p + "attn.relative_position_bias_table"].detach().to(torch.float32).cpu()
                if ws == 7:
                    w[d + ".bias"] = swin_dense_bias(tab, ws, nh, scale).to(dev).contiguous()
                else:
                    w[d + ".table"] = swin_bias_table(tab, ws, nh).to(dev).contiguous()
            if i < len(cfg.depths) - 1:
                ln(f"s{i}.merge.norm", f"{bb}layers.{i}.downsample.norm")
                w[f"s{i}.merge.w"] = h(f"{bb}layers.{i}.downsample.reduction.weight")
            if i in cfg.out_indices:
                ln(f"s{i}.outnorm", f"{bb}norm{i}")
        for l in range(cfg.num_feature_levels):
            cw = sd[f"input_proj.{l}.0.weight"].detach().to(torch.float32)
            if cw.shape[-1] == 1:
                w[f"ip{l}.w"] = cw.reshape(cw.shape[0], cw.shape[1]).to(dev, F16).contiguous()
            else:
                w[f"ip{l}.w"] = cw.permute(0, 2, 3, 1).reshape(cw.shape[0], -1).to(dev, F16).contiguous()
            w[f"ip{l}.b"] = f(f"input_proj.{l}.0.bias")
            ln(f"ip{l}.gn", f"input_proj.{l}.1")
        t = "transformer."
        self.level_embed_cpu = sd[t + "level_embed"].detach().to(torch.float32).cpu()

        def msda(dst, src):
            cat_lin(dst + ".proj", [src + "sampling_offsets", src + "attention_weights"])
            lin(dst + ".value", src + "value_proj")
            lin(dst + ".out", src + "output_proj")

        def mha(dst, src):
            W, b = sd[src + "in_proj_weight"].detach().to(torch.float32), sd[src + "in_proj_bias"].detach().to(torch.float32)
            D = W.shape[1]
            w[dst + ".qk.w"], w[dst + ".qk.b"] = W[:2 * D].to(dev, F16).contiguous(), b[:2 * D].to(dev).contiguous()
            w[dst + ".q.w"], w[dst + ".q.b"] = W[:D].to(dev, F16).contiguous(), b[:D].to(dev).contiguous()
            w[dst + ".kv.w"], w[dst + ".kv.b"] = W[D:].to(dev, F16).contiguous(), b[D:].to(dev).contiguous()
            w[dst + ".v.w"], w[dst + ".v.b"] = W[2 * D:].to(dev, F16).contiguous(), b[2 * D:].to(dev).contiguous()
            lin(dst + ".out", src + "out_proj")

        for i in range(cfg.enc_layers):
            p, d = f"{t}encoder.layers.{i}.", f"e{i}"
            msda(d + ".msda", p + "self_attn.")
            ln(d + ".norm1", p + "norm1"); lin(d + ".lin1", p + "linear1"); lin(d + ".lin2", p + "linear2"); ln(d + ".norm2", p + "norm2")
            if w[d + ".lin1.w"].shape[1] == 256 and w[d + ".lin1.w"].shape[0] % 64 == 0 and w[d + ".lin1.w"].shape[0] <= 2048:
                w[d + ".ffn.blob"] = ops.ffn256_pack(w[d + ".lin1.w"], w[d + ".lin1.b"], w[d + ".lin2.w"])
                w[d + ".ffn.blob_pre"] = ops.ffn256_pack(w[d + ".lin1.w"], w[d + ".lin1.b"], w[d + ".lin2.w"],
                                                         w[d + ".msda.out.w"])
            p = f"{t}encoder.text_layers.{i}."
            mha(d + ".txt", p + "self_attn.")
            lin(d + ".txt.lin1", p + "linear1"); lin(d + ".txt.lin2", p + "linear2")
            ln(d + ".txt.norm1", p + "norm1"); ln(d + ".txt.norm2", p + "norm2")
            p = f"{t}encoder.fusion_layers.{i}."
            ln(d + ".fu.lnv", p + "layer_norm_v"); ln(d + ".fu.lnl", p + "layer_norm_l")
            cat_lin(d + ".fu.qv", [p + "attn.v_proj", p + "attn.values_v_proj"])
            cat_lin(d + ".fu.kl", [p + "attn.l_proj", p + "attn.values_l_proj"])
            lin(d + ".fu.outv", p + "attn.out_v_proj"); lin(d + ".fu.outl", p + "attn.out_l_proj")
            w[d + ".fu.gv"], w[d + ".fu.gl"] = f(p + "gamma_v"), f(p + "gamma_l")
        for i in range(cfg.dec_layers):
            p, d = f"{t}decoder.layers.{i}.", f"d{i}"
            msda(d + ".msda", p + "cross_attn.")
            ln(d + ".norm1", p + "norm1")
            mha(d + ".ca", p + "ca_text."); ln(d + ".canorm", p + "catext_norm")
            mha(d + ".sa", p + "self_attn."); ln(d + ".norm2", p + "norm2")
            lin(d + ".lin1", p + "linear1"); lin(d + ".lin2", p + "linear2"); ln(d + ".norm3", p + "norm3")
        ln("dec.norm", t + "decoder.norm")
        lin("rph0", t + "decoder.ref_point_head.layers.0")
        lin("rph1", t + "decoder.ref_point_head.layers.1")
        w["tgt"] = f(t + "tgt_embed.weight")
        lin("enc_output", t + "enc_output"); ln("enc_output_norm", t + "enc_output_norm")
        for j in range(3):
            lin(f"encbox{j}", f"{t}enc_out_bbox_embed.layers.{j}")
            lin(f"box{j}", f"bbox_embed.0.layers.{j}")
        dt = torch.arange(128, dtype=torch.float32)
        w["dim_t"] = (10000 ** (2 * torch.div(dt, 2, rounding_mode="floor") / 128)).to(dev)
        self._graphs = LRU(self.graph_cache_size)
        self._plans = LRU(self.plan_cache_size)
        self._seen: Dict[Tuple[int, int, int], int] = {}
        self._captions = LRU(self.caption_cache_size)
        self.text_weights: Optional[Dict[str, torch.Tensor]] = None
        self.set_text(encoded_text, token_ids)

    @classmethod
    def text_state_only(cls, cfg: Optional[GDinoConfig] = None, device: str | torch.device = "cpu") -> "GDinoEngine":
        eng = cls.__new__(cls)
        eng.cfg, eng.dev, eng.w = cfg or GDinoConfig(), torch.device(device), {}
        eng._graphs, eng._plans, eng._seen = LRU(cls.graph_cache_size), LRU(cls.plan_cache_size), {}
        eng._captions, eng.text_weights = LRU(cls.caption_cache_size), None
        return eng

    def set_text(self, encoded_text: Optional[torch.Tensor], token_ids: Sequence[int]) -> None:
        if encoded_text is None:
            raise ValueError("encoded_text [T,256] is required: fold BERT + feat_map once at load "
                             "(inklayer_amd.text_branch) or pass precomputed features")
        assert encoded_text.shape[0] == len(token_ids), "one feature row per token id"
        token_ids = list(token_ids)[:self.cfg.max_text_len]
        encoded_text = encoded_text[:self.cfg.max_text_len]
        T = len(token_ids)
        assert T >= 1
        self._graphs.clear()
        self._seen.clear()
        self.captions = self.t_lens = self.t_len = self.Tmax = self.text_position_ids = None
        self.T = T
        self.token_ids = tuple(int(t) for t in token_ids)
        self._text_attn = ops.attn_fewkeys if T <= 16 else ops.attn_midkeys
        self.text0 = encoded_text.detach().to(self.dev, F32).contiguous()
        self._captions.put(self.token_ids, encoded_text.detach().to("cpu", F32))
        self.Tc, self.logit_bias = -(-T // 4) * 4, None
        if self.Tc != T:
            self.logit_bias = torch.zeros(self.Tc, dtype=F32)
            self.logit_bias[T:] = float("-inf")
            self.logit_bias = self.logit_bias.to(self.dev)
        sm, pid = text_masks_and_position_ids(token_ids)
        self.text_blocked = (~sm).to(torch.uint8).to(self.dev).contiguous()
        dim_t = torch.arange(256, dtype=torch.float32)
        dim_t = 10000.0 ** (2 * torch.div(dim_t, 2, rounding_mode="floor") / 256)
        self.pos_text = _interleaved_sincos(pid.float()[:, None] * (2 * math.pi) / dim_t).to(self.dev).contiguous()

    caption_cache_size = 8
    tokenizer = None

    text_encoder = "auto"
    _text_enc = None

    def set_caption(self, token_ids: Sequence[int], sd: Optional[Dict[str, torch.Tensor]] = None,
                    encoded_text: Optional[torch.Tensor] = None) -> None:
        ids = tuple(int(t) for t in token_ids)[:self.cfg.max_text_len]
        self._take_text_weights(sd)
        self.set_text(self._captions_features([ids], [encoded_text])[0], ids)

    def _take_text_weights(self, sd: Optional[Dict[str, torch.Tensor]]) -> None:
        if sd is not None:
            sd = clean_state_dict(sd)
            self.text_weights = {k: v for k, v in sd.items() if k.startswith(("bert.", "feat_map."))}
            self._captions.clear()
            self.release_text_encoder()

    def release_text_encoder(self) -> None:
        self._text_enc = None

    def _gpu_text(self) -> bool:
        mode = self.text_encoder
        if mode not in ("auto", "gpu", "host"):
            raise ValueError(f'text_encoder is "auto", "gpu" or "host", not {mode!r}')
        if mode == "gpu" and self.dev.type != "cuda":
            raise ValueError('text_encoder = "gpu" needs an engine on a GPU; this one is on ' + str(self.dev))
        if mode == "host" or self.dev.type != "cuda":
            return False
        from . import _lib
        from .text_encoder import HIDDEN, bert_hidden_size
        able = bool(self.text_weights) and bert_hidden_size(self.text_weights) == HIDDEN and _lib.lib_path().exists()
        if mode == "gpu" and not able:
            raise ValueError('text_encoder = "gpu" needs the built library and a state dict with a 768-wide bert.*')
        return able

    def _captions_features(self, caps: Sequence[Tuple[int, ...]],
                           encoded_texts: Sequence[Optional[torch.Tensor]]) -> List[torch.Tensor]:
        gpu = self._gpu_text()
        feats = [f if f is not None else self._captions.get(ids) for ids, f in zip(caps, encoded_texts)]
        missing = list(dict.fromkeys(ids for ids, f in zip(caps, feats) if f is None))
        if missing:
            if not self.text_weights:
                raise ValueError("set_caption needs encoded_text [T, 256] or a state dict with the checkpoint's bert.* "
                                 "and feat_map.* tensors")
            if gpu:
                if self._text_enc is None:
                    from .text_encoder import BertTextEncoder
                    self._text_enc = BertTextEncoder(self.text_weights, self.dev)
                new = [f.to("cpu", F32) for f in self._text_enc.encode(missing)]
            else:
                from .text_branch import encode_caption_from_checkpoint
                new = [encode_caption_from_checkpoint(self.text_weights, ids) for ids in missing]
            new = dict(zip(missing, new))
            feats = [f if f is not None else new[ids] for ids, f in zip(caps, feats)]
        return [f[:len(ids)] for ids, f in zip(caps, feats)]

    def set_captions(self, token_id_lists: Sequence[Sequence[int]], sd: Optional[Dict[str, torch.Tensor]] = None,
                     encoded_texts: Optional[Sequence[Optional[torch.Tensor]]] = None) -> None:
        caps = [tuple(int(t) for t in ids)[:self.cfg.max_text_len] for ids in token_id_lists]
        if not caps or any(len(c) < 1 for c in caps):
            raise ValueError("set_captions needs at least one caption, each of at least one token id")
        if encoded_texts is not None and len(encoded_texts) != len(caps):
            raise ValueError("one encoded_text (or None) per caption")
        feats_in = list(encoded_texts) if encoded_texts is not None else [None] * len(caps)
        if len(set(caps)) == 1:
            return self.set_caption(caps[0], sd=sd, encoded_text=feats_in[0])
        self._take_text_weights(sd)
        feats = [f.detach().to("cpu", F32) for f in self._captions_features(caps, feats_in)]
        for ids, f in zip(caps, feats):
            assert f.shape[0] == len(ids), "one feature row per token id"
            self._captions.put(ids, f)
        B, Tmax = len(caps), max(len(c) for c in caps)
        self._graphs.clear()
        self._seen.clear()
        self.T = self.token_ids = self._text_attn = None
        self.captions, self.t_lens, self.Tmax, self.Tc = tuple(caps), tuple(len(c) for c in caps), Tmax, -(-Tmax // 4) * 4
        text0 = torch.zeros(B, Tmax, 256, dtype=F32)
        blocked = ~torch.eye(Tmax, dtype=torch.bool).repeat(B, 1, 1)
        pid = torch.zeros(B, Tmax, dtype=torch.long)
        bias = torch.zeros(B, self.Tc, dtype=F32)
        for b, (ids, f) in enumerate(zip(caps, feats)):
            n = len(ids)
            sm, p = text_masks_and_position_ids(ids)
            text0[b, :n], blocked[b, :n, :n], pid[b, :n] = f, ~sm, p
            bias[b, n:] = float("-inf")
        self.text_position_ids = pid
        self.text0 = text0.view(B * Tmax, 256).to(self.dev).contiguous()
        self.t_len = torch.tensor(self.t_lens, dtype=I32).to(self.dev)
        self.text_blocked = blocked.to(torch.uint8).to(self.dev).contiguous()
        dim_t = torch.arange(256, dtype=torch.float32)
        dim_t = 10000.0 ** (2 * torch.div(dim_t, 2, rounding_mode="floor") / 256)
        self.pos_text = _interleaved_sincos(pid.view(-1).float()[:, None] * (2 * math.pi) / dim_t).to(self.dev).contiguous()
        self.logit_bias = bias.to(self.dev)

    def predict(self, images_u8: Sequence[torch.Tensor], box_threshold: float, text_threshold: float,
                remove_combined: bool = False):
        logits, boxes = self.forward(images_u8)
        both = torch.cat([logits, boxes], dim=-1).cpu()
        TL, res = logits.shape[-1], []
        for b in range(both.shape[0]):
            T, ids = (self.T, self.token_ids) if self.captions is None else (self.t_lens[b], self.captions[b])
            prob = both[b, :, :T].contiguous().sigmoid()
            keep = prob.max(dim=1)[0] > box_threshold
            kept = prob[keep]
            phrases = phrases_from_probs(kept, ids, text_threshold, remove_combined, self.tokenizer)
            res.append((both[b, keep, TL:], kept.max(dim=1)[0] if len(kept) else kept.new_zeros(0), phrases))
        return res

    def _positive_maps(self, positive_maps, B: int):
        T = self.T if self.captions is None else self.Tmax
        t_of = [self.T] * B if self.captions is None else list(self.t_lens)

        def cut(pm, Tb):
            pm = torch.as_tensor(pm, dtype=F32).detach().cpu()
            if pm.dim() != 2 or pm.shape[0] < 1 or pm.shape[1] < Tb:
                raise ValueError(f"a positive map is [C >= 1, >= {Tb} token columns], not {tuple(pm.shape)}")
            if bool((pm[:, Tb:] != 0).any()):
                raise ValueError(f"a positive map marks tokens beyond its caption's {Tb}: it was built for another caption")
            return pm[:, :Tb]

        if not isinstance(positive_maps, (list, tuple)):
            if self.captions is not None:
                raise ValueError("one positive map for all images needs one caption for all images (set_caption); after "
                                 "set_captions pass one map per image")
            pm = cut(positive_maps, self.T)
            return pm.contiguous().to(self.dev), None, [pm.shape[0]] * B
        if len(positive_maps) != B:
            raise ValueError(f"{len(positive_maps)} positive maps for {B} images")
        maps = [cut(pm, t_of[b]) for b, pm in enumerate(positive_maps)]
        counts = [m.shape[0] for m in maps]
        full = torch.zeros((B, max(counts), T), dtype=F32)
        for b, m in enumerate(maps):
            full[b, :m.shape[0], :m.shape[1]] = m
        return full.to(self.dev), torch.tensor(counts, dtype=I32).to(self.dev), counts

    def predict_classes(self, images_u8: Sequence[torch.Tensor], positive_maps, num_select: int = 300,
                        sizes: Optional[Sequence[Tuple[int, int]]] = None):
        B, nq = len(images_u8), self.cfg.num_queries
        pm, n_cls, counts = self._positive_maps(positive_maps, B)
        if num_select < 1:
            raise ValueError("num_select >= 1")
        if sizes is not None and len(sizes) != B:
            raise ValueError(f"{len(sizes)} sizes for {B} images")
        Cmax = pm.shape[-2]
        K = min(int(num_select), nq * Cmax)
        nchunk = -(-(nq * Cmax) // 16384)
        if nchunk > 1 and (nchunk * K > 16384 or (nq * Cmax) // nchunk < K):
            raise ValueError(f"num_select = {num_select} of {nq * Cmax} (query, class) pairs is more than the selection "
                             f"kernel merges ({16384 // nchunk} here)")
        scale = torch.ones((B, 2), dtype=F32) if sizes is None else \
            torch.tensor([[float(w_), float(h)] for h, w_ in sizes], dtype=F32)
        logits, boxes = self.forward(images_u8)
        prob = ops.class_scores(logits, pm, n_cls)
        idx, val = ops.topk_rowmax(prob.view(B, nq * Cmax, 1), K, want_values=True)
        xyxy, labels, _ = ops.select_boxes(idx, boxes.contiguous(), scale.to(self.dev), Cmax)
        out = torch.cat([val[..., None], labels.to(F32)[..., None], xyxy], dim=-1).cpu()
        res = []
        for b in range(B):
            k = min(K, nq * counts[b])
            res.append((out[b, :k, 2:].contiguous(), out[b, :k, 0].contiguous(), out[b, :k, 1].to(torch.int64)))
        return res

    def predict_spans(self, images_u8: Sequence[torch.Tensor], positive_maps, box_threshold: float):
        B = len(images_u8)
        pm, n_cls, counts = self._positive_maps(positive_maps, B)
        logits, boxes = self.forward(images_u8)
        prob = ops.class_scores(logits, pm, n_cls)
        both = torch.cat([prob, boxes], dim=-1).cpu()
        P, res = prob.shape[-1], []
        for b in range(B):
            bx, sc, ph = [], [], []
            for p in range(counts[b]):
                keep = both[b, :, p] > box_threshold
                bx.append(both[b, keep, P:])
                sc.append(both[b, keep, p])
                ph.append(torch.full((int(keep.sum()),), p, dtype=torch.int64))
            res.append((torch.cat(bx), torch.cat(sc), torch.cat(ph)))
        return res

    graph_max_batch = 1
    graph_cache_size = 4
    plan_cache_size = 8

    def _forward_graphed(self, images_u8: Sequence[torch.Tensor], h: int, w_: int):
        B = len(images_u8)
        key = (h, w_, B)
        g = self._graphs.get(key)
        if g is None:
            self._seen[key] = self._seen.get(key, 0) + 1
            if len(self._seen) > 4096:
                self._seen.clear()
            if self._seen[key] < 2:
                return self._forward_eager(images_u8)
            static_in = [torch.empty_like(im) for im in images_u8]
            for dst, src in zip(static_in, images_u8):
                dst.copy_(src)
            side = torch.cuda.Stream(device=self.dev)
            side.wait_stream(torch.cuda.current_stream(self.dev))
            with torch.cuda.stream(side):
                for _ in range(2):
                    self._forward_eager(static_in)
            torch.cuda.current_stream(self.dev).wait_stream(side)
            graph = torch.cuda.CUDAGraph()
            with torch.cuda.graph(graph):
                out = self._forward_eager(static_in)
            g = (graph, static_in, out, self.plan(h, w_, B))
            self._graphs.put(key, g)
        graph, static_in, out = g[:3]
        for dst, src in zip(static_in, images_u8):
            dst.copy_(src)
        graph.replay()
        return out[0].clone(), out[1].clone()

    def plan(self, h: int, w: int, B: int) -> _Plan:
        return self._plans.get_or_make((h, w, B), lambda: _Plan(self, h, w, B))

    def _mlp3(self, prefix: str, x16: torch.Tensor) -> torch.Tensor:
        w = self.w
        a = ops.gemm(x16, w[prefix + "0.w"], w[prefix + "0.b"], act="relu", out_dtype=F16)
        a = ops.gemm(a, w[prefix + "1.w"], w[prefix + "1.b"], act="relu", out_dtype=F16)
        return ops.gemm(a, w[prefix + "2.w"], w[prefix + "2.b"])

    def _swin_block(self, x: torch.Tensor, i: int, b: int, pl: _Plan) -> None:
        cfg, w = self.cfg, self.w
        C, nh, nW = cfg.embed_dim * 2 ** i, cfg.num_heads[i], pl.nW[i]
        d = f"s{i}b{b}"
        shifted = b % 2 == 1
        wm = pl.win_map[i][1 if shifted else 0]
        y = ops.layernorm_rows(x, w[d + ".norm1.w"], w[d + ".norm1.b"], 1e-5, gather=wm)
        qkv = ops.gemm(y, w[d + ".qkv.w"], w[d + ".qkv.b"], out_dtype=F16)
        ws, scale = cfg.window_size, HEAD_DIM ** -0.5
        if ws == 7:
            o = ops.flash_attn(qkv[:, :C], qkv[:, C:2 * C], qkv[:, 2 * C:], n_batch=pl.B * nW, n_heads=nh,
                               head_dim=HEAD_DIM, scale=scale, n_q=ws * ws, n_k=ws * ws, dense_bias=w[d + ".bias"],
                               dense_mask=pl.shift_mask[i] if shifted else None)
        else:
            o = ops.swin_attn(qkv[:, :C], qkv[:, C:2 * C], qkv[:, 2 * C:], n_windows=pl.B * nW, n_heads=nh, ws=ws,
                              scale=scale, bias_table=w[d + ".table"], region=pl.region[i] if shifted else None, nW=nW)
        ops.gemm(o, w[d + ".proj.w"], w[d + ".proj.b"], residual=x, row_map=wm, out=x)
        y = ops.layernorm_rows(x, w[d + ".norm2.w"], w[d + ".norm2.b"], 1e-5)
        hmid = ops.gemm(y, w[d + ".fc1.w"], w[d + ".fc1.b"], act="gelu", out_dtype=F16)
        ops.gemm(hmid, w[d + ".fc2.w"], w[d + ".fc2.b"], residual=x, out=x)

    def backbone(self, images_u8: Sequence[torch.Tensor], pl: _Plan) -> Dict[int, Tuple[torch.Tensor, torch.Tensor]]:
        cfg, w, dev = self.cfg, self.w, self.dev
        B = len(images_u8)
        H0, W0 = pl.stage_hw[0]
        T0 = H0 * W0
        patches = torch.empty((B * T0, 64), device=dev, dtype=F16)
        for b, img in enumerate(images_u8):
            ops.swin_patchify(img, cfg.pixel_mean, cfg.pixel_std, patches[b * T0:(b + 1) * T0])
        x = ops.gemm(patches, w["pe.w"], w["pe.b"])
        x = ops.layernorm_rows(x, w["pe.norm.w"], w["pe.norm.b"], 1e-5, out_dtype=F32)
        outs = {}
        for i, dep in enumerate(cfg.depths):
            for b in range(dep):
                self._swin_block(x, i, b, pl)
            if i in cfg.out_indices:
                o32 = torch.empty_like(x)
                o16 = torch.empty(x.shape, device=dev, dtype=F16)
                ops.layernorm_rows(x, w[f"s{i}.outnorm.w"], w[f"s{i}.outnorm.b"], 1e-5, out=o32, out2=o16)
                outs[i] = (o32, o16)
            if i < len(cfg.depths) - 1:
                m = ops.layernorm_merge4(x, w[f"s{i}.merge.norm.w"], w[f"s{i}.merge.norm.b"], 1e-5, pl.merge_map[i])
                x = ops.gemm(m, w[f"s{i}.merge.w"])
        return outs

    def neck(self, feats, pl: _Plan, B: int) -> torch.Tensor:
        cfg, w, dev = self.cfg, self.w, self.dev
        S = pl.S
        src = torch.empty((B * S, 256), device=dev, dtype=F32)
        nfeat = len(cfg.out_indices)
        for l in range(cfg.num_feature_levels):
            hh, ww = pl.shapes[l]
            Tl = hh * ww
            if l < nfeat:
                a16 = feats[cfg.out_indices[l]][1]
            else:
                f32_last = feats[cfg.out_indices[-1]][0]
                T3 = pl.shapes[nfeat - 1][0] * pl.shapes[nfeat - 1][1]
                col = ops.gather_rows(f32_last, pl.lvl4_map, B, Tl * 9, x_batch_rows=T3, idx_batch_stride=0)
                a16 = col.view(B * Tl, -1)
            y = ops.gemm(a16, w[f"ip{l}.w"], w[f"ip{l}.b"])
            ops.groupnorm_nhwc(y, B, Tl, 32, w[f"ip{l}.gn.w"], w[f"ip{l}.gn.b"], 1e-5,
                               src[pl.level_start[l]:], S * 256)
        return src

    def encoder(self, src: torch.Tensor, pl: _Plan, B: int):
        S = pl.S
        tb = self._tb
        text = self.text0.repeat(B, 1) if tb is None else tb.text0.clone()
        s16 = torch.empty((B * S, 256), device=self.dev, dtype=F16)
        s16p = torch.empty((B * S, 256), device=self.dev, dtype=F16)
        for i in range(self.cfg.enc_layers):
            src, text = self._enc_layer(i, src, text, pl, B, s16, s16p)
        return src, text

    def _enc_layer(self, i: int, src: torch.Tensor, text: torch.Tensor, pl: _Plan, B: int, s16: torch.Tensor,
                   s16p: torch.Tensor):
        w, dev, T, S, tb = self.w, self.dev, self.T, pl.S, self._tb
        d = f"e{i}"
        have16 = False
        ln32 = torch.empty_like(text)
        l16 = torch.empty(text.shape, device=dev, dtype=F16)
        ops.layernorm_rows(text, w[d + ".fu.lnl.w"], w[d + ".fu.lnl.b"], 1e-5, out=ln32, out2=l16)
        if tb is None and self.fold_fusion and T <= 4:
            kl = ops.gemm(l16, w[d + ".fu.kl.w"], w[d + ".fu.kl.b"])
            ol = ops.fusion_fold(src, B, S, w[d + ".fu.lnv.w"], w[d + ".fu.lnv.b"], 1e-5, kl, T, w[d + ".fu.qv.w"],
                                 w[d + ".fu.qv.b"], w[d + ".fu.outv.w"], w[d + ".fu.outv.b"], w[d + ".fu.gv"],
                                 256 ** -0.5, pos=pl.pos, out16_pos=s16p, out16=s16)
            have16 = True
        else:
            vn = torch.empty_like(src)
            ops.layernorm_rows(src, w[d + ".fu.lnv.w"], w[d + ".fu.lnv.b"], 1e-5, out=vn, out2=s16)
            qv = ops.gemm(s16, w[d + ".fu.qv.w"], w[d + ".fu.qv.b"], out_dtype=F16)
            kl = ops.gemm(l16, w[d + ".fu.kl.w"], w[d + ".fu.kl.b"], out_dtype=F16)
            if tb is None:
                ov, ol = ops.biattn_wide(qv, kl, B, S, T, 256 ** -0.5)
            else:
                ov, ol = ops.biattn_wide_varlen(qv, kl, B, S, tb.Tmax, tb.t_len, 256 ** -0.5)
            src = ops.gemm(ov, w[d + ".fu.outv.w"], w[d + ".fu.outv.b"], col_scale=w[d + ".fu.gv"], residual=vn, out=vn)
        text = ops.gemm(ol, w[d + ".fu.outl.w"], w[d + ".fu.outl.b"], col_scale=w[d + ".fu.gl"], residual=ln32)
        qk = ops.gemm(ops.add_cvt_f16(text, self.pos_text if tb is None else tb.pos_text), w[d + ".txt.qk.w"],
                      w[d + ".txt.qk.b"], out_dtype=F16)
        vv = ops.gemm(ops.add_cvt_f16(text), w[d + ".txt.v.w"], w[d + ".txt.v.b"], out_dtype=F16)
        if tb is None:
            a = self._text_attn(qk[:, :256], qk[:, 256:], vv, B=B, n_heads=4, head_dim=64, scale=64 ** -0.5,
                                blocked=self.text_blocked)
        else:
            a = ops.attn_midkeys_varlen(qk[:, :256], qk[:, 256:], vv, B=B, n_heads=4, head_dim=64, scale=64 ** -0.5,
                                        blocked=tb.blocked, k_len=tb.t_len)
        text = ops.layernorm_rows(ops.gemm(a, w[d + ".txt.out.w"], w[d + ".txt.out.b"], residual=text),
                                  w[d + ".txt.norm1.w"], w[d + ".txt.norm1.b"], 1e-5, out_dtype=F32)
        ff = ops.gemm(ops.add_cvt_f16(text), w[d + ".txt.lin1.w"], w[d + ".txt.lin1.b"], act="relu", out_dtype=F16)
        text = ops.layernorm_rows(ops.gemm(ff, w[d + ".txt.lin2.w"], w[d + ".txt.lin2.b"], residual=text),
                                  w[d + ".txt.norm2.w"], w[d + ".txt.norm2.b"], 1e-5, out_dtype=F32)
        if have16:
            proj = ops.gemm(s16p, w[d + ".msda.proj.w"], w[d + ".msda.proj.b"])
            val = ops.gemm(s16, w[d + ".msda.value.w"], w[d + ".msda.value.b"], out_dtype=F16)
        else:
            proj = ops.gemm(ops.add_cvt_f16(src, pl.pos, out=s16), w[d + ".msda.proj.w"], w[d + ".msda.proj.b"])
            val = ops.gemm(ops.add_cvt_f16(src, out=s16), w[d + ".msda.value.w"], w[d + ".msda.value.b"], out_dtype=F16)
        o = ops.msda_fused(val, proj, pl.enc_ref, pl.shapes, B, S, ref_batched=False)
        if self.fuse_ffn and self.fuse_ffn_pre and (d + ".ffn.blob_pre") in w:
            ops.ffn256_fused(o, src, w[d + ".ffn.blob_pre"], int(w[d + ".lin1.b"].numel()), w[d + ".lin2.b"],
                             w[d + ".norm2.w"], w[d + ".norm2.b"], 1e-5, out=src,
                             pre=(w[d + ".msda.out.b"], w[d + ".norm1.w"], w[d + ".norm1.b"]))
            return src, text
        y = ops.gemm(o, w[d + ".msda.out.w"], w[d + ".msda.out.b"], residual=src, out=src)
        ops.layernorm_rows(y, w[d + ".norm1.w"], w[d + ".norm1.b"], 1e-5, out=src, out2=s16)
        if self.fuse_ffn and (d + ".ffn.blob") in w:
            ops.ffn256_fused(s16, src, w[d + ".ffn.blob"], int(w[d + ".lin1.b"].numel()), w[d + ".lin2.b"],
                             w[d + ".norm2.w"], w[d + ".norm2.b"], 1e-5, out=src)
        else:
            ff = ops.gemm(s16, w[d + ".lin1.w"], w[d + ".lin1.b"], act="relu", out_dtype=F16)
            y = ops.gemm(ff, w[d + ".lin2.w"], w[d + ".lin2.b"], residual=src, out=src)
            ops.layernorm_rows(y, w[d + ".norm2.w"], w[d + ".norm2.b"], 1e-5, out=src)
        return src, text

    def decoder(self, memory: torch.Tensor, text: torch.Tensor, pl: _Plan, B: int, stages: Optional[dict] = None):
        cfg, w, dev, S, nq, tb = self.cfg, self.w, self.dev, pl.S, self.cfg.num_queries, self._tb
        T = self.T if tb is None else tb.Tmax
        om16 = ops.gather_rows(memory, pl.valid_map, B, S, x_batch_rows=S, idx_batch_stride=0)
        om = ops.gemm(om16, w["enc_output.w"], w["enc_output.b"])
        omn16 = torch.empty((B * S, 256), device=dev, dtype=F16)
        omn = ops.layernorm_rows(om, w["enc_output_norm.w"], w["enc_output_norm.b"], 1e-5, out=om, out2=omn16)
        text16 = ops.add_cvt_f16(text)
        Tc, tw16 = (self.Tc if tb is None else tb.Tc), text16
        tbias = [self.logit_bias] * B if tb is None else list(tb.bias.unbind(0))
        if Tc != T:
            tw16 = torch.zeros((B, Tc, 256), device=dev, dtype=F16)
            tw16[:, :T] = text16.view(B, T, 256)
            tw16 = tw16.view(B * Tc, 256)
        logits = torch.empty((B, S, Tc), device=dev, dtype=F32)
        for b in range(B):
            ops.gemm(omn16[b * S:(b + 1) * S], tw16[b * Tc:(b + 1) * Tc], tbias[b], out=logits[b])
        idx = ops.topk_rowmax(logits, nq)
        if stages is not None:
            stages["topk_logits"] = logits if Tc == T else logits[:, :, :T]
            if "force_topk" in stages:
                idx = stages["force_topk"].to(I32).to(dev).contiguous()
        sel16 = ops.gather_rows(omn, idx, B, nq, x_batch_rows=S, idx_batch_stride=nq)
        delta = self._mlp3("encbox", sel16)
        prop = ops.gather_rows(pl.props_unsig, idx, B, nq, x_batch_rows=0, idx_batch_stride=nq, out_dtype=F32)
        ref = ops.box_refine(delta, prop, ref_is_logit=True)
        if stages is not None:
            stages["topk"], stages["ref0"] = idx, ref
        output = w["tgt"].repeat(B, 1)
        mem16 = ops.add_cvt_f16(memory)
        hs16 = None
        if stages is not None:
            stages["hs"], stages["refs"] = [], [ref.clone()]
        for i in range(cfg.dec_layers):
            output = self._dec_layer(i, output, ref, mem16, text16, pl, B)
            if stages is not None:
                stages["hs"].append(output.clone())
            if i < cfg.dec_layers - 1:
                ref = ops.box_refine(self._mlp3("box", ops.add_cvt_f16(output)), ref)
                if stages is not None:
                    stages["refs"].append(ref.clone())
            else:
                if stages is not None:
                    stages["refs"].append(ops.box_refine(self._mlp3("box", ops.add_cvt_f16(output)), ref))
                hs16 = ops.layernorm_rows(output, w["dec.norm.w"], w["dec.norm.b"], 1e-5)
        boxes = ops.box_refine(self._mlp3("box", hs16), ref).view(B, nq, 4)
        out_logits = torch.empty((B, nq, Tc), device=dev, dtype=F32)
        for b in range(B):
            ops.gemm(hs16[b * nq:(b + 1) * nq], tw16[b * Tc:(b + 1) * Tc], tbias[b], out=out_logits[b])
        return (out_logits if Tc == T else out_logits[:, :, :T]), boxes

    def _dec_layer(self, i: int, output: torch.Tensor, ref: torch.Tensor, mem16: torch.Tensor, text16: torch.Tensor,
                   pl: _Plan, B: int) -> torch.Tensor:
        w = self.w
        nq = output.shape[0] // B
        d = f"d{i}"
        qse = ops.sine_embed4(ref, w["dim_t"])
        qpos = ops.gemm(ops.gemm(qse, w["rph0.w"], w["rph0.b"], act="relu", out_dtype=F16), w["rph1.w"], w["rph1.b"])
        qk = ops.gemm(ops.add_cvt_f16(output, qpos), w[d + ".sa.qk.w"], w[d + ".sa.qk.b"], out_dtype=F16)
        vv = ops.gemm(ops.add_cvt_f16(output), w[d + ".sa.v.w"], w[d + ".sa.v.b"], out_dtype=F16)
        a = ops.flash_attn(qk[:, :256], qk[:, 256:], vv, n_batch=B, n_heads=8, head_dim=32, scale=32 ** -0.5,
                           n_q=nq, n_k=nq)
        output = ops.layernorm_rows(ops.gemm(a, w[d + ".sa.out.w"], w[d + ".sa.out.b"], residual=output),
                                    w[d + ".norm2.w"], w[d + ".norm2.b"], 1e-5, out_dtype=F32)
        q = ops.gemm(ops.add_cvt_f16(output, qpos), w[d + ".ca.q.w"], w[d + ".ca.q.b"], out_dtype=F16)
        kv = ops.gemm(text16, w[d + ".ca.kv.w"], w[d + ".ca.kv.b"], out_dtype=F16)
        if self._tb is None:
            a = self._text_attn(q, kv[:, :256], kv[:, 256:], B=B, n_heads=8, head_dim=32, scale=32 ** -0.5)
        else:
            a = ops.attn_midkeys_varlen(q, kv[:, :256], kv[:, 256:], B=B, n_heads=8, head_dim=32, scale=32 ** -0.5,
                                        k_len=self._tb.t_len)
        output = ops.layernorm_rows(ops.gemm(a, w[d + ".ca.out.w"], w[d + ".ca.out.b"], residual=output),
                                    w[d + ".canorm.w"], w[d + ".canorm.b"], 1e-5, out_dtype=F32)
        proj = ops.gemm(ops.add_cvt_f16(output, qpos), w[d + ".msda.proj.w"], w[d + ".msda.proj.b"])
        val = ops.gemm(mem16, w[d + ".msda.value.w"], w[d + ".msda.value.b"], out_dtype=F16)
        o = ops.msda_fused(val, proj, ref, pl.shapes, B, nq, ref_batched=True)
        output = ops.layernorm_rows(ops.gemm(o, w[d + ".msda.out.w"], w[d + ".msda.out.b"], residual=output),
                                    w[d + ".norm1.w"], w[d + ".norm1.b"], 1e-5, out_dtype=F32)
        ff = ops.gemm(ops.add_cvt_f16(output), w[d + ".lin1.w"], w[d + ".lin1.b"], act="relu", out_dtype=F16)
        output = ops.layernorm_rows(ops.gemm(ff, w[d + ".lin2.w"], w[d + ".lin2.b"], residual=output),
                                    w[d + ".norm3.w"], w[d + ".norm3.b"], 1e-5, out_dtype=F32)
        return output

    def forward(self, images_u8: Sequence[torch.Tensor], stages: Optional[dict] = None, allow_graph: bool = True):
        B = len(images_u8)
        if self.captions is not None:
            return self._forward_captions(images_u8, stages)
        sizes = [tuple(im.shape[:2]) for im in images_u8]
        if len(set(sizes)) > 1:
            assert stages is None
            logits = torch.empty((B, self.cfg.num_queries, self.T), device=self.dev, dtype=F32)
            boxes = torch.empty((B, self.cfg.num_queries, 4), device=self.dev, dtype=F32)
            for sz in dict.fromkeys(sizes):
                idx = [i for i, s_ in enumerate(sizes) if s_ == sz]
                lg, bx = self.forward([images_u8[i] for i in idx], allow_graph=allow_graph)
                ii = torch.tensor(idx, device=self.dev)
                logits[ii] = lg
                boxes[ii] = bx
            return logits, boxes
        h, w_ = sizes[0]
        if allow_graph and stages is None and 0 < B <= self.graph_max_batch:
            return self._forward_graphed(images_u8, h, w_)
        return self._forward_eager(images_u8, stages)

    _tb: Optional["_TextBatch"] = None

    def _forward_captions(self, images_u8: Sequence[torch.Tensor], stages: Optional[dict] = None):
        B = len(images_u8)
        if B != len(self.captions):
            raise ValueError(f"{B} images for {len(self.captions)} captions: set_captions takes one caption per image")
        sizes = [tuple(im.shape[:2]) for im in images_u8]
        groups = [[i for i, s_ in enumerate(sizes) if s_ == sz] for sz in dict.fromkeys(sizes)]
        Tmax = self.Tmax
        if len(groups) == 1:
            self._tb = _TextBatch(self.text0, self.t_len, self.text_blocked, self.pos_text, self.logit_bias, Tmax, self.Tc)
            try:
                return self._forward_eager(images_u8, stages)
            finally:
                self._tb = None
        assert stages is None
        logits = torch.full((B, self.cfg.num_queries, Tmax), float("-inf"), device=self.dev, dtype=F32)
        boxes = torch.empty((B, self.cfg.num_queries, 4), device=self.dev, dtype=F32)
        for idx in groups:
            ii = torch.tensor(idx, device=self.dev)
            Tg = max(self.t_lens[i] for i in idx)
            Tcg = -(-Tg // 4) * 4
            self._tb = _TextBatch(self.text0.view(B, Tmax, 256)[ii, :Tg].reshape(-1, 256), self.t_len[ii].contiguous(),
                                  self.text_blocked[ii, :Tg, :Tg].contiguous(),
                                  self.pos_text.view(B, Tmax, 256)[ii, :Tg].reshape(-1, 256),
                                  self.logit_bias[ii, :Tcg].contiguous(), Tg, Tcg)
            try:
                lg, bx = self._forward_eager([images_u8[i] for i in idx])
            finally:
                self._tb = None
            logits[ii, :, :Tg] = lg
            boxes[ii] = bx
        return logits, boxes

    def _forward_eager(self, images_u8: Sequence[torch.Tensor], stages: Optional[dict] = None):
        B = len(images_u8)
        h, w_ = tuple(images_u8[0].shape[:2])
        pl = self.plan(h, w_, B)
        feats = self.backbone(images_u8, pl)
        src = self.neck(feats, pl, B)
        if stages is not None:
            stages["src"], stages["feats"] = src.clone(), feats
        memory, text = self.encoder(src, pl, B)
        if stages is not None:
            stages["memory"], stages["memory_text"] = memory.clone(), text.clone()
        return self.decoder(memory, text, pl, B, stages)

    def detect(self, images_u8: Sequence[torch.Tensor], top_n: Optional[int] = None):
        logits, boxes = self.forward(images_u8)
        both = torch.cat([logits, boxes], dim=-1).cpu()
        return self.postprocess(both, top_n)

    def postprocess(self, both: torch.Tensor, top_n: Optional[int] = None):
        T = self.T if self.captions is None else self.Tmax
        res = []
        for b in range(both.shape[0]):
            prob = both[b, :, :T].sigmoid()
            score = prob.max(dim=1)[0]
            if top_n is None:
                keep = score > self.cfg.box_threshold
                res.append((both[b, keep, T:], score[keep]))
            else:
                order = torch.sort(score, descending=True, stable=True)[1][:top_n]
                res.append((both[b, order, T:], score[order]))
        return res
```

### inklayer_amd/ops.py

```python
from __future__ import annotations

import ctypes as C
from typing import Optional, Sequence, Tuple

import torch

from . import _lib
from ._lib import InkAttn, InkGemm, check

ACT = {None: 0, "none": 0, "gelu": 1, "relu": 2}
F16, F32 = torch.float16, torch.float32


_GEMM_TRACE = None


def set_gemm_trace(lst) -> None:
    global _GEMM_TRACE
    _GEMM_TRACE = lst


_ATTN_TRACE = None


def set_attn_trace(lst) -> None:
    global _ATTN_TRACE
    _ATTN_TRACE = lst


def tracing_off() -> bool:
    return _GEMM_TRACE is None and _ATTN_TRACE is None


_raw_stream = getattr(torch._C, "_cuda_getCurrentRawStream", None)
_cur_device = getattr(torch._C, "_cuda_getDevice", None)


def _stream() -> int:
    if _raw_stream is not None and _cur_device is not None:
        return _raw_stream(_cur_device())
    return torch.cuda.current_stream().cuda_stream


def own_f32(t: torch.Tensor, dev) -> torch.Tensor:
    t = t.detach().to(dev, F32).contiguous()
    if t.untyped_storage().nbytes() > t.numel() * t.element_size():
        t = t.clone()
    return t


def _p(t: Optional[torch.Tensor]) -> Optional[int]:
    if t is None:
        return None
    assert t.is_cuda, "InkLayer HIP ops need GPU tensors (no CPU fallback)"
    return t.data_ptr()


def gemm(a: torch.Tensor, w: torch.Tensor, bias: Optional[torch.Tensor] = None, *,
         act: Optional[str] = None, residual: Optional[torch.Tensor] = None,
         col_scale: Optional[torch.Tensor] = None, row_map: Optional[torch.Tensor] = None,
         out: Optional[torch.Tensor] = None, out_dtype: torch.dtype = F32,
         out_rows: Optional[int] = None) -> torch.Tensor:
    assert a.dtype == F16 and w.dtype == F16
    assert a.dim() == 2 and w.dim() == 2 and a.stride(1) == 1 and w.stride(1) == 1
    M, K = a.shape
    N = w.shape[0]
    assert w.shape[1] == K
    p = InkGemm()
    if out is None:
        rows = out_rows if out_rows is not None else M
        out = torch.empty((rows, N), device=a.device, dtype=out_dtype)
    assert out.dim() == 2 and out.stride(1) == 1 and out.shape[1] == N
    p.A, p.W, p.C = a.data_ptr(), w.data_ptr(), out.data_ptr()
    p.bias, p.col_scale = _p(bias), _p(col_scale)
    p.residual, p.row_map = _p(residual), _p(row_map)
    if bias is not None:
        assert bias.dtype == F32 and bias.numel() == N
    if col_scale is not None:
        assert col_scale.dtype == F32 and col_scale.numel() == N
    if residual is not None:
        assert residual.dtype == F32 and residual.stride(1) == 1 and residual.shape[1] == N
        p.ldr = residual.stride(0)
    if row_map is not None:
        assert row_map.dtype == torch.int32 and row_map.numel() == M
    p.M, p.N, p.K = M, N, K
    p.lda, p.ldw, p.ldc = a.stride(0), w.stride(0), out.stride(0)
    p.act = ACT[act]
    p.c_f16 = 1 if out.dtype == F16 else 0
    assert out.dtype in (F16, F32)
    if _GEMM_TRACE is None:
        check(_lib.lib().ink_gemm_f16(C.byref(p), _stream()), "ink_gemm_f16")
    else:
        e0, e1 = torch.cuda.Event(enable_timing=True), torch.cuda.Event(enable_timing=True)
        e0.record()
        check(_lib.lib().ink_gemm_f16(C.byref(p), _stream()), "ink_gemm_f16")
        e1.record()
        _GEMM_TRACE.append((2.0 * M * N * K, e0, e1, (M, N, K, act or '-', 'res' if residual is not None else '-',
                                                      'map' if row_map is not None else '-', 'f16' if p.c_f16 else 'f32')))
    return out


def layernorm_rows(x: torch.Tensor, gamma: Optional[torch.Tensor], beta: Optional[torch.Tensor],
                   eps: float, *, gather: Optional[torch.Tensor] = None,
                   out_dtype: torch.dtype = F16, out: Optional[torch.Tensor] = None,
                   out2: Optional[torch.Tensor] = None, act: Optional[str] = None,
                   split: bool = False, add: Optional[torch.Tensor] = None,
                   add_batch_rows: Optional[torch.Tensor] = None, rows_per_batch: int = 0,
                   split_f32: Optional[torch.Tensor] = None) -> torch.Tensor:
    assert x.dtype == F32 and x.dim() == 2 and x.stride(1) == 1
    Cdim = x.shape[1]
    rows = gather.numel() if gather is not None else x.shape[0]
    wcols = 3 * Cdim if split else Cdim
    if split:
        assert out_dtype == F16 and out2 is None
    if out is None:
        out = torch.empty((rows, wcols), device=x.device, dtype=out_dtype)
    assert out.shape == (rows, wcols) and out.stride(1) == 1
    oh = out.data_ptr() if out.dtype == F16 else None
    of = out.data_ptr() if out.dtype == F32 else None
    if out2 is not None:
        assert out2.shape == out.shape and out2.stride(0) == out.stride(0) and out2.dtype != out.dtype
        if out2.dtype == F16:
            oh = out2.data_ptr()
        else:
            of = out2.data_ptr()
    if split_f32 is not None:
        assert split and out.stride(0) == 3 * Cdim and split_f32.dtype == F32 and split_f32.is_contiguous()
        assert tuple(split_f32.shape) == (rows, Cdim)
        of = split_f32.data_ptr()
    if gather is not None:
        assert gather.dtype == torch.int32
    if add is not None:
        assert gather is None and add.dtype == F32 and add.dim() == 2 and add.stride(1) == 1 and add.shape[1] == Cdim
        if add_batch_rows is not None:
            assert add_batch_rows.dtype == torch.int32 and add_batch_rows.is_cuda and rows_per_batch > 0
            assert add_batch_rows.numel() * rows_per_batch == rows
        else:
            rows_per_batch = rows
    check(_lib.lib().ink_layernorm_rows(x.data_ptr(), x.stride(0), _p(gamma), _p(beta), eps,
                                        _p(gather), rows, Cdim, oh, of, out.stride(0), ACT[act], int(split),
                                        _p(add), add.stride(0) if add is not None else 0, _p(add_batch_rows),
                                        rows_per_batch, _stream()), "ink_layernorm_rows")
    return out


def add_cvt_f16(a: torch.Tensor, b: Optional[torch.Tensor] = None,
                out: Optional[torch.Tensor] = None) -> torch.Tensor:
    assert a.dtype == F32 and a.is_contiguous()
    nb = 0
    if b is not None:
        assert b.dtype == F32 and b.is_contiguous() and a.numel() % b.numel() == 0
        nb = b.numel()
    if out is None:
        out = torch.empty(a.shape, device=a.device, dtype=F16)
    assert out.dtype == F16 and out.is_contiguous() and out.numel() == a.numel()
    check(_lib.lib().ink_add_cvt_f16(a.data_ptr(), _p(b), nb, out.data_ptr(), a.numel(), _stream()),
          "ink_add_cvt_f16")
    return out


def add_split_f16(a: torch.Tensor, b: Optional[torch.Tensor] = None) -> torch.Tensor:
    assert a.dtype == F32 and a.is_contiguous() and a.dim() == 2
    nb = 0
    if b is not None:
        assert b.dtype == F32 and b.is_contiguous() and a.numel() % b.numel() == 0
        nb = b.numel()
    R, Cn = a.shape
    out = torch.empty((R, 3 * Cn), device=a.device, dtype=F16)
    check(_lib.lib().ink_add_split_f16(a.data_ptr(), _p(b), nb, out.data_ptr(), a.numel(), Cn, _stream()),
          "ink_add_split_f16")
    return out


def split_weight(w32: torch.Tensor) -> torch.Tensor:
    w32 = w32.to(torch.float32)
    hi = w32.to(F16)
    lo = ((w32 - hi.to(torch.float32)) * 64.0).to(F16)
    return torch.cat([hi, (hi.to(torch.float32) / 64.0).to(F16), lo], dim=-1).contiguous()


def add_f32(a: torch.Tensor, b: torch.Tensor, out: Optional[torch.Tensor] = None) -> torch.Tensor:
    assert a.dtype == F32 and b.dtype == F32 and a.is_contiguous() and b.is_contiguous()
    assert a.numel() % b.numel() == 0
    if out is None:
        out = torch.empty(a.shape, device=a.device, dtype=F32)
    assert out.is_contiguous() and out.numel() == a.numel()
    check(_lib.lib().ink_add_f32(a.data_ptr(), b.data_ptr(), b.numel(), out.data_ptr(), a.numel(),
                                 _stream()), "ink_add_f32")
    return out


def flash_attn(q: torch.Tensor, k: torch.Tensor, v: torch.Tensor, *, n_batch: int, n_heads: int,
               head_dim: int, scale: float, n_q: Optional[int] = None, n_k: Optional[int] = None,
               rel_h: Optional[torch.Tensor] = None, rel_w: Optional[torch.Tensor] = None,
               rel_aug: Optional[torch.Tensor] = None, grid_w: int = 0,
               dense_bias: Optional[torch.Tensor] = None, dense_mask: Optional[torch.Tensor] = None,
               q_batch_rows: Optional[torch.Tensor] = None,
               kv_batch_rows: Optional[torch.Tensor] = None,
               tok_rows: Optional[torch.Tensor] = None, pad_k: Optional[torch.Tensor] = None,
               pad_v: Optional[torch.Tensor] = None,
               out: Optional[torch.Tensor] = None) -> torch.Tensor:
    for t in (q, k, v):
        assert t.dtype == F16 and t.dim() == 2 and t.stride(1) == 1 and t.is_cuda
    if n_q is None:
        n_q = q.shape[0] // n_batch
    if n_k is None:
        n_k = k.shape[0] // n_batch
    if tok_rows is not None:
        assert rel_aug is not None and out is not None and n_q == n_k
        assert tok_rows.dtype == torch.int32 and tok_rows.is_cuda and tok_rows.numel() == n_batch * n_q
        for t in (pad_k, pad_v):
            assert t is not None and t.dtype == F16 and t.is_contiguous() and t.numel() == n_heads * head_dim
        assert out.dtype == F16 and out.stride(1) == 1
        assert out.shape[0] * out.stride(0) * 2 < 2 ** 31 and q.shape[0] * q.stride(0) * 2 < 2 ** 32
    else:
        if out is None:
            out = torch.empty((n_batch * n_q, n_heads * head_dim), device=q.device, dtype=F16)
        assert out.dtype == F16 and out.shape[0] == n_batch * n_q and out.stride(1) == 1
    p = InkAttn()
    p.Q, p.K, p.V, p.O = q.data_ptr(), k.data_ptr(), v.data_ptr(), out.data_ptr()
    p.ldq, p.ldk, p.ldv, p.ldo = q.stride(0), k.stride(0), v.stride(0), out.stride(0)
    p.n_batch, p.n_heads, p.n_q, p.n_k, p.head_dim = n_batch, n_heads, n_q, n_k, head_dim
    p.scale = scale
    p.grid_w = grid_w
    for name, t in (("q_batch_rows", q_batch_rows), ("kv_batch_rows", kv_batch_rows)):
        if t is not None:
            assert t.dtype == torch.int32 and t.numel() == n_batch and t.is_cuda
            setattr(p, name, t.data_ptr())
    if dense_bias is not None:
        assert dense_bias.dtype == F32 and dense_bias.is_contiguous() and dense_bias.shape == (n_heads, n_q, 64)
        p.bias_mode, p.dense_bias = 3, dense_bias.data_ptr()
        if dense_mask is not None:
            assert dense_mask.dtype == F32 and dense_mask.is_contiguous() and dense_mask.shape[1:] == (n_q, 64)
            p.dense_mask, p.n_mask = dense_mask.data_ptr(), dense_mask.shape[0]
    elif rel_aug is not None:
        assert rel_aug.dtype == F16 and rel_aug.is_contiguous()
        p.bias_mode, p.rel_aug = 2, rel_aug.data_ptr()
        if tok_rows is not None:
            p.tok_rows, p.pad_k, p.pad_v = tok_rows.data_ptr(), pad_k.data_ptr(), pad_v.data_ptr()
    elif rel_h is not None:
        assert rel_h.dtype == rel_w.dtype and rel_h.dtype in (F32, F16)
        assert rel_h.is_contiguous() and rel_w.is_contiguous()
        p.bias_mode, p.rel_h, p.rel_w = 1, rel_h.data_ptr(), rel_w.data_ptr()
        p.rel_f16 = int(rel_h.dtype == F16)
    else:
        p.bias_mode = 0
    if _ATTN_TRACE is None:
        check(_lib.lib().ink_flash_attn(C.byref(p), _stream()), "ink_flash_attn")
    else:
        e0, e1 = torch.cuda.Event(enable_timing=True), torch.cuda.Event(enable_timing=True)
        e0.record()
        check(_lib.lib().ink_flash_attn(C.byref(p), _stream()), "ink_flash_attn")
        e1.record()
        _ATTN_TRACE.append((n_batch, n_heads, n_q, n_k, head_dim, int(p.bias_mode), int(out.shape[0]), e0, e1))
    return out


SWIN_ATTN_WINDOWS = (7, 12)


def swin_attn(q: torch.Tensor, k: torch.Tensor, v: torch.Tensor, *, n_windows: int, n_heads: int, ws: int, scale: float,
              bias_table: torch.Tensor, region: Optional[torch.Tensor] = None, nW: int = 0,
              out: Optional[torch.Tensor] = None) -> torch.Tensor:
    assert ws in SWIN_ATTN_WINDOWS, f"swin_attn serves window sizes {SWIN_ATTN_WINDOWS}, not {ws}"
    rows = n_windows * ws * ws
    for t in (q, k, v):
        assert t.dtype == F16 and t.dim() == 2 and t.stride(1) == 1 and t.is_cuda
        assert t.shape[0] >= rows and t.shape[1] >= n_heads * 32 and t.stride(0) % 8 == 0 and t.data_ptr() % 16 == 0
    assert bias_table.dtype == F32 and bias_table.is_contiguous() and bias_table.is_cuda
    assert bias_table.shape == (n_heads, (2 * ws - 1) ** 2)
    if region is not None:
        assert region.dtype == torch.uint8 and region.is_contiguous() and region.is_cuda
        assert nW > 0 and region.shape == (nW, ws * ws) and n_windows % nW == 0
    if out is None:
        out = torch.empty((rows, n_heads * 32), device=q.device, dtype=F16)
    assert out.dtype == F16 and out.is_cuda and out.shape == (rows, n_heads * 32) and out.stride(1) == 1
    assert out.stride(0) % 8 == 0 and out.data_ptr() % 8 == 0
    check(_lib.lib().ink_swin_attn(q.data_ptr(), k.data_ptr(), v.data_ptr(), q.stride(0), k.stride(0), v.stride(0),
                                   out.data_ptr(), out.stride(0), n_windows, n_heads, ws, scale, bias_table.data_ptr(),
                                   _p(region), nW if region is not None else 0, _stream()), "ink_swin_attn")
    return out


def relpos_bias(q: torch.Tensor, rel_pos_h: torch.Tensor, rel_pos_w: torch.Tensor, *, S: int,
                n_batch: int, n_heads: int, head_dim: int, scale: float, out=None,
                tok_rows: Optional[torch.Tensor] = None, f16_tables: bool = False):
    assert q.dtype == F16 and q.stride(1) == 1
    assert rel_pos_h.dtype == F32 and rel_pos_h.is_contiguous()
    assert rel_pos_w.dtype == F32 and rel_pos_w.is_contiguous()
    assert rel_pos_h.shape == (2 * S - 1, head_dim)
    n = n_batch * n_heads * S * S
    fn = _lib.lib().ink_relpos_bias
    if S == 64 and f16_tables:
        oh, ow = out if out is not None else (torch.empty((n, 64), device=q.device, dtype=F16),
                                              torch.empty((n, 64), device=q.device, dtype=F16))
        assert oh.dtype == F16 and ow.dtype == F16 and oh.numel() >= n * 64 and ow.numel() >= n * 64
        check(_lib.lib().ink_relpos_bias64_f16(q.data_ptr(), q.stride(0), rel_pos_h.data_ptr(), rel_pos_w.data_ptr(), n_batch,
                                               n_heads, head_dim, scale, oh.data_ptr(), ow.data_ptr(), _stream()),
              "ink_relpos_bias64_f16")
        return oh, ow
    if S == 64:
        oh, ow = out if out is not None else (torch.empty((n, 64), device=q.device, dtype=F32),
                                              torch.empty((n, 64), device=q.device, dtype=F32))
        assert oh.numel() >= n * 64 and ow.numel() >= n * 64
        check(fn(q.data_ptr(), q.stride(0), rel_pos_h.data_ptr(), rel_pos_w.data_ptr(), S, n_batch,
                 n_heads, head_dim, scale, None, oh.data_ptr(), ow.data_ptr(), None, _stream()),
              "ink_relpos_bias")
        return oh, ow
    aug = out if out is not None else torch.empty((n, 32), device=q.device, dtype=F16)
    assert aug.numel() >= n * 32
    if tok_rows is not None:
        assert tok_rows.dtype == torch.int32 and tok_rows.is_cuda and tok_rows.numel() == n_batch * S * S
    check(fn(q.data_ptr(), q.stride(0), rel_pos_h.data_ptr(), rel_pos_w.data_ptr(), S, n_batch,
             n_heads, head_dim, scale, tok_rows.data_ptr() if tok_rows is not None else None,
             None, None, aug.data_ptr(), _stream()), "ink_relpos_bias")
    return aug


def _resize_u8(image_u8: torch.Tensor, oh: int, ow: int, filter: str, out: Optional[torch.Tensor]) -> torch.Tensor:
    from .resize import plan_for
    assert image_u8.dtype == torch.uint8 and image_u8.is_cuda and image_u8.is_contiguous() and oh > 0 and ow > 0
    assert image_u8.dim() == 2 or (image_u8.dim() == 3 and image_u8.shape[2] == 3), "[H, W] or [H, W, 3] expected"
    h, w, ch = int(image_u8.shape[0]), int(image_u8.shape[1]), 1 if image_u8.dim() == 2 else 3
    shape = (oh, ow) if ch == 1 else (oh, ow, 3)
    if out is None:
        out = torch.empty(shape, device=image_u8.device, dtype=torch.uint8)
    assert out.dtype == torch.uint8 and out.is_contiguous() and tuple(out.shape) == shape
    pl = plan_for(h, w, oh, ow, image_u8.device, filter, ch)
    ptr = lambda t: t.data_ptr() if t is not None else None
    check(_lib.lib().ink_resize_u8(image_u8.data_ptr(), h, w, ch, out.data_ptr(), oh, ow, ptr(pl.xb), ptr(pl.xk), pl.kx,
                                   ptr(pl.yb), ptr(pl.yk), pl.ky, ptr(pl.tmp), _stream()), "ink_resize_u8")
    return out


def resize_bilinear_u8(image_u8: torch.Tensor, oh: int, ow: int, out: Optional[torch.Tensor] = None) -> torch.Tensor:
    assert image_u8.dim() == 3 and image_u8.shape[2] == 3
    if (oh, ow) == tuple(image_u8.shape[:2]):
        return image_u8
    return _resize_u8(image_u8, oh, ow, "bilinear", out)


def sam_patchify(image_u8: torch.Tensor, L: int, P: int, mean: Sequence[float],
                 std: Sequence[float], chan_reverse: bool, out: torch.Tensor, split: bool = False) -> torch.Tensor:
    assert image_u8.dtype == torch.uint8 and image_u8.is_cuda and image_u8.is_contiguous()
    h, w, c = image_u8.shape
    assert c == 3 and out.dtype == F16 and out.is_contiguous()
    assert out.numel() == (L // P) ** 2 * 3 * P * P * (3 if split else 1)
    m = (C.c_float * 3)(*mean)
    s = (C.c_float * 3)(*std)
    check(_lib.lib().ink_sam_patchify(image_u8.data_ptr(), h, w, L, P, m, s, int(chan_reverse), int(split),
                                      out.data_ptr(), _stream()), "ink_sam_patchify")
    return out


def im2col3x3(x: torch.Tensor, B: int, H: int, W: int, stride: int = 1, relu: bool = False,
              out: Optional[torch.Tensor] = None) -> torch.Tensor:
    assert x.dtype == F16 and x.is_contiguous() and x.shape[0] == B * H * W
    Cn = x.shape[1]
    OH, OW = (H - 1) // stride + 1, (W - 1) // stride + 1
    if out is None:
        out = torch.empty((B * OH * OW, 9 * Cn), device=x.device, dtype=F16)
    assert out.dtype == F16 and out.is_contiguous() and out.numel() >= B * OH * OW * 9 * Cn
    check(_lib.lib().ink_im2col3x3_f16(x.data_ptr(), B, H, W, Cn, stride, int(relu), out.data_ptr(), _stream()),
          "ink_im2col3x3_f16")
    return out


def sam_pe_encode(coords01: torch.Tensor, gauss: torch.Tensor,
                  add: Optional[torch.Tensor] = None, out: Optional[torch.Tensor] = None) -> torch.Tensor:
    assert coords01.dtype == F32 and coords01.is_contiguous() and coords01.shape[-1] == 2
    assert gauss.dtype == F32 and gauss.is_contiguous() and gauss.shape[0] == 2
    N, Fd = coords01.numel() // 2, gauss.shape[1]
    if out is None:
        out = torch.empty((N, 2 * Fd), device=coords01.device, dtype=F32)
    assert out.dtype == F32 and out.is_contiguous() and tuple(out.shape) == (N, 2 * Fd)
    n_add = 0
    if add is not None:
        assert add.dtype == F32 and add.is_contiguous() and add.shape[-1] == 2 * Fd
        n_add = add.numel() // (2 * Fd)
    check(_lib.lib().ink_sam_pe_encode(coords01.data_ptr(), gauss.data_ptr(), N, Fd, _p(add), n_add,
                                       out.data_ptr(), _stream()), "ink_sam_pe_encode")
    return out


def sam_prompt_tokens(gauss: torch.Tensor, point_emb: torch.Tensor, not_a_point: torch.Tensor, out_tok: torch.Tensor,
                      input_size: float, P: int, points: Optional[torch.Tensor] = None,
                      labels: Optional[torch.Tensor] = None, boxes: Optional[torch.Tensor] = None, pad: bool = False,
                      out: Optional[torch.Tensor] = None) -> torch.Tensor:
    Fd = gauss.shape[1]
    assert gauss.dtype == F32 and gauss.is_contiguous() and gauss.shape[0] == 2
    for t, n in ((point_emb, 4), (not_a_point, 1), (out_tok, 5)):
        assert t.dtype == F32 and t.is_contiguous() and t.numel() == n * 2 * Fd
    n_pts = 0
    if points is not None:
        assert labels is not None and points.dtype == F32 and labels.dtype == torch.int32
        assert points.is_contiguous() and labels.is_contiguous() and points.dim() == 3 and points.shape[0] == P
        n_pts = points.shape[1]
        assert tuple(points.shape) == (P, n_pts, 2) and tuple(labels.shape) == (P, n_pts)
    if boxes is not None:
        assert boxes.dtype == F32 and boxes.is_contiguous() and tuple(boxes.shape) == (P, 4)
    NT = 5 + n_pts + int(pad) + (2 if boxes is not None else 0)
    if out is None:
        out = torch.empty((P, NT, 2 * Fd), device=gauss.device, dtype=F32)
    assert out.dtype == F32 and out.is_contiguous() and tuple(out.shape) == (P, NT, 2 * Fd)
    check(_lib.lib().ink_sam_prompt_tokens(_p(points), _p(labels), n_pts, int(pad), _p(boxes), _p(gauss), Fd,
                                           _p(point_emb), _p(not_a_point), _p(out_tok),
                                           float(input_size), P, _p(out), _stream()), "ink_sam_prompt_tokens")
    return out


SAM_MASK_EMBED_PARAMS = 4684


def sam_mask_embed(mask: torch.Tensor, emb: torch.Tensor, emb_rows: torch.Tensor, params: torch.Tensor, eps: float,
                   split: bool = False):
    assert mask.dtype == F32 and mask.is_contiguous() and mask.dim() == 4 and mask.shape[1] == 1
    P, S = mask.shape[0], mask.shape[2]
    assert mask.shape[3] == S and S % 4 == 0
    g = S // 4
    assert emb.dtype == F32 and emb.is_contiguous() and emb.dim() == 2 and emb.shape[1] == 256
    assert emb_rows.dtype == torch.int32 and emb_rows.is_cuda and emb_rows.numel() == P
    assert params.dtype == F32 and params.is_contiguous() and params.numel() == SAM_MASK_EMBED_PARAMS
    keys = torch.empty((P * g * g, 256), device=mask.device, dtype=F32)
    ks = torch.empty((P * g * g, 768), device=mask.device, dtype=F16) if split else None
    check(_lib.lib().ink_sam_mask_embed(_p(mask), _p(emb), _p(emb_rows), _p(params),
                                        params.numel(), eps, P, g, _p(keys), _p(ks), _stream()),
          "ink_sam_mask_embed")
    return (keys, ks) if split else keys


def sam_mask_logits(up: torch.Tensor, hyper: torch.Tensor, n: int, g: int) -> torch.Tensor:
    assert up.dtype == F32 and up.is_contiguous() and hyper.dtype == F32 and hyper.is_contiguous()
    Cn = hyper.shape[1]
    assert up.numel() == n * g * g * 16 * Cn
    out = torch.empty((n, 4 * g, 4 * g), device=up.device, dtype=F32)
    check(_lib.lib().ink_sam_mask_logits(up.data_ptr(), hyper.data_ptr(), n, g, Cn, out.data_ptr(),
                                         _stream()), "ink_sam_mask_logits")
    return out


def sam_postprocess(low: torch.Tensor, L: int, input_hw: Tuple[int, int], orig_hw: Tuple[int, int],
                    thr: float = 0.0, want_logits: bool = False):
    assert low.dtype == F32 and low.is_contiguous() and low.dim() == 3
    n, S, _ = low.shape
    oh, ow = orig_hw
    out = torch.empty((n, oh, ow), device=low.device, dtype=torch.uint8)
    lg = torch.empty((n, oh, ow), device=low.device, dtype=F32) if want_logits else None
    check(_lib.lib().ink_sam_postprocess(low.data_ptr(), n, S, L, input_hw[0], input_hw[1], oh, ow,
                                         thr, out.data_ptr(), _p(lg), _stream()),
          "ink_sam_postprocess")
    return (out, lg) if want_logits else out


NMS_MAX_BOXES = 4096


def sam_amg_stats(low: torch.Tensor, L: int, input_hw: Tuple[int, int], crop_hw: Tuple[int, int], thr: float,
                  offset: float, xy0: Tuple[int, int] = (0, 0), orig_hw: Optional[Tuple[int, int]] = None,
                  index: Optional[torch.Tensor] = None, count: Optional[torch.Tensor] = None,
                  want_logits: bool = False):
    assert low.dtype == F32 and low.is_contiguous() and low.dim() == 3
# ... 1023 lines not shown
```

Before: 116.6 sketches/s.

## Add grouped GEMM launches and fused add/convert/layernorm kernels for GroundingDINO

```diff
diff --git a/include/inklayer_hip.h b/include/inklayer_hip.h
--- a/include/inklayer_hip.h
+++ b/include/inklayer_hip.h
@@ -29,6 +29,9 @@
 int ink_gemm_f16(const InkGemm* p, void* stream);
 int ink_gemm_set_variant(int32_t v);
 int ink_gemm_query_variant(int32_t M, int32_t N, int32_t K);
+#define INK_GEMM_GROUP_MAX 8
+#define INK_GEMM_MIXED 3
+int ink_gemm_grouped(const InkGemm* problems, const int32_t* c_rows, int32_t n, void* stream);
 
 int ink_layernorm_rows(const float* x, int64_t ldx, const float* gamma, const float* beta,
                        float eps, const int32_t* gather, int32_t rows_out, int32_t C,
@@ -38,6 +41,12 @@
 
 int ink_add_cvt_f16(const float* a, const float* b, int64_t n_b, void* out_f16, int64_t n,
                     void* stream);
+int ink_add_cvt_f16_pair(const float* a, const float* b, int64_t n_b, void* out_a_f16, void* out_ab_f16, int64_t n,
+                         void* stream);
+int ink_layernorm_rows3(const float* x, int64_t ldx, const float* gamma, const float* beta,
+                        float eps, int32_t rows_out, int32_t C,
+                        void* out_f16, float* out_f32, void* out3_f16, int64_t ldo, int32_t act,
+                        const float* add3, int64_t ld_add3, void* stream);
 int ink_add_split_f16(const float* a, const float* b, int64_t n_b, void* out_f16, int64_t n, int32_t C,
                       void* stream);
 int ink_add_f32(const float* a, const float* b, int64_t n_b, float* out, int64_t n, void* stream);
diff --git a/inklayer_amd/_lib.py b/inklayer_amd/_lib.py
--- a/inklayer_amd/_lib.py
+++ b/inklayer_amd/_lib.py
@@ -43,6 +43,10 @@
     "ink_add_split_f16": [c_void_p, c_void_p, c_i64, c_void_p, c_i64, c_int, c_void_p],
     "ink_add_cvt_f16": [c_void_p, c_void_p, c_i64, c_void_p, c_i64, c_void_p],
     "ink_add_f32": [c_void_p, c_void_p, c_i64, c_void_p, c_i64, c_void_p],
+    "ink_gemm_grouped": [C.POINTER(InkGemm), C.POINTER(c_int), c_int, c_void_p],
+    "ink_add_cvt_f16_pair": [c_void_p, c_void_p, c_i64, c_void_p, c_void_p, c_i64, c_void_p],
+    "ink_layernorm_rows3": [c_void_p, c_i64, c_void_p, c_void_p, c_float, c_int, c_int, c_void_p, c_void_p, c_void_p,
+                            c_i64, c_int, c_void_p, c_i64, c_void_p],
     "ink_flash_attn": [C.POINTER(InkAttn), c_void_p],
     "ink_swin_attn": [c_void_p, c_void_p, c_void_p, c_i64, c_i64, c_i64, c_void_p, c_i64, c_int, c_int, c_int, c_float,
                       c_void_p, c_void_p, c_int, c_void_p],
diff --git a/inklayer_amd/csrc/gemm.hip b/inklayer_amd/csrc/gemm.hip
--- a/inklayer_amd/csrc/gemm.hip
+++ b/inklayer_amd/csrc/gemm.hip
@@ -149,8 +149,29 @@
 }
 
 constexpr int NS = 2;
-template <int BM, int BN, int BK, int WM, int WN>
-__global__ __launch_bounds__(WM * WN * 64) void gemm_f16_nt(InkGemm p, int group_m) {
+struct InkGemmGroup {
+  int n;
+  int tile_start[INK_GEMM_GROUP_MAX + 1];
+  InkGemm p[INK_GEMM_GROUP_MAX];
+};
+__device__ __forceinline__ int group_problem(const InkGemm&) { return 0; }
+__device__ __forceinline__ int group_problem(const InkGemmGroup& g) {
+  const int bid = blockIdx.x;
+  int i = 0;
+#pragma unroll
+  for (int k = 1; k < INK_GEMM_GROUP_MAX; ++k)
+    if (k < g.n && bid >= g.tile_start[k]) i = k;
+  return __builtin_amdgcn_readfirstlane(i);
+}
+__device__ __forceinline__ const InkGemm& problem_at(const InkGemm& a, int) { return a; }
+__device__ __forceinline__ const InkGemm& problem_at(const InkGemmGroup& g, int i) { return g.p[i]; }
+__device__ __forceinline__ int first_tile_of(const InkGemm&, int) { return 0; }
+__device__ __forceinline__ int first_tile_of(const InkGemmGroup& g, int i) { return g.tile_start[i]; }
+
+template <int BM, int BN, int BK, int WM, int WN, class ARG>
+__global__ __launch_bounds__(WM * WN * 64) void gemm_f16_nt(ARG arg, int group_m) {
+  const int which = group_problem(arg);
+  const InkGemm& p = problem_at(arg, which);
   constexpr int NT = WM * WN * 64;
   constexpr int CPR = BK / 8;
   constexpr int ROWB = BK * 2;
@@ -169,7 +190,7 @@
   const int ntn = (p.N + BN - 1) / BN;
   const int ntm = (p.M + BM - 1) / BM;
   int mt, nt;
-  tile_of(xcd_remap(blockIdx.x, ntm * ntn), ntm, ntn, group_m, mt, nt);
+  tile_of(xcd_remap(blockIdx.x - first_tile_of(arg, which), ntm * ntn), ntm, ntn, group_m, mt, nt);
   const int m0 = mt * BM;
   const int n0 = nt * BN;
 
@@ -412,9 +433,18 @@
 static int launch_gemm(const InkGemm& p, hipStream_t s, int group_m = 1) {
   constexpr int lds = NS * (BM + BN) * BK * 2;
   static_assert(lds <= 160 * 1024, "LDS budget");
-  ink_dyn_lds<gemm_f16_nt<BM, BN, BK, WM, WN>>(lds);
+  ink_dyn_lds<gemm_f16_nt<BM, BN, BK, WM, WN, InkGemm>>(lds);
   const int ntm = (p.M + BM - 1) / BM, ntn = (p.N + BN - 1) / BN;
-  hipLaunchKernelGGL((gemm_f16_nt<BM, BN, BK, WM, WN>), dim3(ntm * ntn), dim3(WM * WN * 64), lds, s, p, group_m);
+  hipLaunchKernelGGL((gemm_f16_nt<BM, BN, BK, WM, WN, InkGemm>), dim3(ntm * ntn), dim3(WM * WN * 64), lds, s, p, group_m);
+  return ink_launch_status();
+}
+
+template <int BM, int BN, int BK, int WM, int WN>
+static int launch_gemm_grouped(const InkGemmGroup& g, hipStream_t s, int group_m = 1) {
+  constexpr int lds = NS * (BM + BN) * BK * 2;
+  ink_dyn_lds<gemm_f16_nt<BM, BN, BK, WM, WN, InkGemmGroup>>(lds);
+  hipLaunchKernelGGL((gemm_f16_nt<BM, BN, BK, WM, WN, InkGemmGroup>), dim3(g.tile_start[g.n]), dim3(WM * WN * 64), lds, s, g,
+                     group_m);
   return ink_launch_status();
 }
 
@@ -614,9 +644,7 @@
   return INK_OK;
 }
 
-extern "C" int ink_gemm_f16(const InkGemm* pp, void* stream) {
-  INK_CHECK_ARG(pp != nullptr);
-  const InkGemm& p = *pp;
+static int gemm_check_args(const InkGemm& p) {
   INK_CHECK_ARG(p.A && p.W && p.C);
   INK_CHECK_ARG(p.M > 0 && p.N > 0 && p.K > 0);
   INK_CHECK_ARG(p.K % 32 == 0 && p.N % 4 == 0);
@@ -626,13 +654,92 @@
   INK_CHECK_ARG(ink_aligned<16>(p.A, p.W, p.C));
   INK_CHECK_ARG(p.act >= 0 && p.act <= 2);
   INK_CHECK_ARG(p.c_f16 == 0 || p.c_f16 == 1);
-  hipStream_t s = (hipStream_t)stream;
-  if (p.K % 64 != 0) return launch_gemm<128, 128, 32, 2, 2>(p, s);
+  return INK_OK;
+}
+
+static int gemm_family(const InkGemm& p) {
+  if (p.K % 64 != 0) return 32;
   int v = g_variant;
   if (v < 0) v = ink_gemm_query_variant(p.M, p.N, p.K);
-  switch (v) {
+  return v;
+}
+
+extern "C" int ink_gemm_f16(const InkGemm* pp, void* stream) {
+  INK_CHECK_ARG(pp != nullptr);
+  const InkGemm& p = *pp;
+  if (gemm_check_args(p) != INK_OK) return INK_ERR_ARG;
+  hipStream_t s = (hipStream_t)stream;
+  switch (gemm_family(p)) {
+    case 32: return launch_gemm<128, 128, 32, 2, 2>(p, s);
     case 10: return launch_gemm<256, 256, 64, 4, 4>(p, s, 4);
     case 45: return launch_gemm_pp(p, s, 4);
     default: return launch_gemm<128, 128, 64, 2, 2>(p, s);
   }
 }
+
+namespace {
+struct ByteRect {
+  uintptr_t base;
+  int64_t rows, ld, width;
+};
+static ByteRect rect_of(const void* ptr, int64_t rows, int64_t ld_elems, int64_t cols, int elem) {
+  return {(uintptr_t)ptr, rows, ld_elems * elem, cols * elem};
+}
+static bool rects_may_overlap(const ByteRect& a, const ByteRect& b) {
+  if (!a.base || !b.base || a.rows <= 0 || b.rows <= 0) return false;
+  const uintptr_t a_end = a.base + (uintptr_t)((a.rows - 1) * a.ld + a.width);
+  const uintptr_t b_end = b.base + (uintptr_t)((b.rows - 1) * b.ld + b.width);
+  if (a_end <= b.base || b_end <= a.base) return false;
+  if (a.ld != b.ld) return true;
+  const ByteRect& lo = a.base <= b.base ? a : b;
+  const ByteRect& hi = a.base <= b.base ? b : a;
+  const int64_t dc = (int64_t)((hi.base - lo.base) % (uintptr_t)lo.ld);
+  return !(dc >= lo.width && dc + hi.width <= lo.ld);
+}
+}
+
+extern "C" int ink_gemm_grouped(const InkGemm* problems, const int32_t* c_rows, int32_t n, void* stream) {
+  INK_CHECK_ARG(problems != nullptr && c_rows != nullptr && n >= 1 && n <= INK_GEMM_GROUP_MAX);
+  InkGemmGroup g = {};
+  int rows_of[INK_GEMM_GROUP_MAX];
+  for (int i = 0; i < n; ++i) {
+    if (problems[i].M == 0) continue;
+    if (gemm_check_args(problems[i]) != INK_OK) return INK_ERR_ARG;
+    INK_CHECK_ARG(c_rows[i] > 0 && (problems[i].row_map || c_rows[i] >= problems[i].M));
+    rows_of[g.n] = c_rows[i];
+    g.p[g.n++] = problems[i];
+  }
+  if (g.n == 0) return INK_OK;
+  const int family = gemm_family(g.p[0]);
+  for (int i = 1; i < g.n; ++i)
+    if (gemm_family(g.p[i]) != family) return INK_GEMM_MIXED;
+  if (family == 45) return INK_GEMM_MIXED;
+  for (int i = 0; i < g.n; ++i) {
+    const InkGemm& p = g.p[i];
+    const ByteRect out = rect_of(p.C, rows_of[i], p.ldc, p.N, p.c_f16 ? 2 : 4);
+    for (int j = 0; j < g.n; ++j) {
+      if (j == i) continue;
+      const InkGemm& q = g.p[j];
+      const ByteRect in[] = {rect_of(q.A, q.M, q.lda, q.K, 2),          rect_of(q.W, q.N, q.ldw, q.K, 2),
+                             rect_of(q.bias, 1, q.N, q.N, 4),           rect_of(q.col_scale, 1, q.N, q.N, 4),
+                             rect_of(q.residual, rows_of[j], q.ldr, q.N, 4), rect_of(q.row_map, 1, q.M, q.M, 4)};
+      for (const ByteRect& r : in)
+        if (rects_may_overlap(out, r)) return INK_ERR_ARG;
+      if (j > i && rects_may_overlap(out, rect_of(q.C, rows_of[j], q.ldc, q.N, q.c_f16 ? 2 : 4))) return INK_ERR_ARG;
+    }
+  }
+  const int bm = family == 10 ? 256 : 128;
+  int64_t tiles = 0;
+  for (int i = 0; i < g.n; ++i) {
+    g.tile_start[i] = (int)tiles;
+    tiles += (int64_t)((g.p[i].M + bm - 1) / bm) * ((g.p[i].N + bm - 1) / bm);
+    INK_CHECK_ARG(tiles <= INT32_MAX);
+  }
+  for (int i = g.n; i <= INK_GEMM_GROUP_MAX; ++i) g.tile_start[i] = (int)tiles;
+  hipStream_t s = (hipStream_t)stream;
+  switch (family) {
+    case 32: return launch_gemm_grouped<128, 128, 32, 2, 2>(g, s);
+    case 10: return launch_gemm_grouped<256, 256, 64, 4, 4>(g, s, 4);
+    default: return launch_gemm_grouped<128, 128, 64, 2, 2>(g, s);
+  }
+}
diff --git a/inklayer_amd/csrc/norm.hip b/inklayer_amd/csrc/norm.hip
--- a/inklayer_amd/csrc/norm.hip
+++ b/inklayer_amd/csrc/norm.hip
@@ -67,6 +67,54 @@
   }
 }
 
+template <int NV>
+__global__ __launch_bounds__(256) void layernorm_rows3_kernel(
+    const float* __restrict__ x, int64_t ldx, const float* __restrict__ gamma, const float* __restrict__ beta, float eps,
+    int rows_out, int C, f16* __restrict__ out_h, float* __restrict__ out_f, f16* __restrict__ out3, int64_t ldo, int act,
+    const float* __restrict__ add3, int64_t ld_add3) {
+  const int lane = threadIdx.x & 63;
+  const int row = blockIdx.x * 4 + (threadIdx.x >> 6);
+  if (row >= rows_out) return;
+  const int nv = C >> 2;
+  const float* xr = x + (int64_t)row * ldx;
+  f32x4 r[NV];
+  float s = 0.f;
+#pragma unroll
+  for (int j = 0; j < NV; ++j) {
+    const int v = lane + 64 * j;
+    r[j] = v < nv ? *(const f32x4*)(xr + v * 4) : (f32x4){0.f, 0.f, 0.f, 0.f};
+    s += (r[j][0] + r[j][1]) + (r[j][2] + r[j][3]);
+  }
+  const float mean = wave_sum(s) / (float)C;
+  float q = 0.f;
+#pragma unroll
+  for (int j = 0; j < NV; ++j) {
+    const int v = lane + 64 * j;
+    if (v < nv) {
+      const f32x4 d = r[j] - mean;
+      q += (d[0] * d[0] + d[1] * d[1]) + (d[2] * d[2] + d[3] * d[3]);
+    }
+  }
+  const float rstd = 1.0f / sqrtf(wave_sum(q) / (float)C + eps);
+#pragma unroll
+  for (int j = 0; j < NV; ++j) {
+    const int v = lane + 64 * j;
+    if (v < nv) {
+      f32x4 y = (r[j] - mean) * rstd;
+      if (gamma) y *= *(const f32x4*)(gamma + v * 4);
+      if (beta) y += *(const f32x4*)(beta + v * 4);
+      if (act == INK_ACT_GELU) {
+#pragma unroll
+        for (int e = 0; e < 4; ++e) y[e] = gelu_erf(y[e]);
+      }
+      if (out_h) *(f16x4*)(out_h + row * ldo + v * 4) = (f16x4){(f16)y[0], (f16)y[1], (f16)y[2], (f16)y[3]};
+      if (out_f) *(f32x4*)(out_f + row * ldo + v * 4) = y;
+      const f32x4 z = y + *(const f32x4*)(add3 + row * ld_add3 + v * 4);
+      *(f16x4*)(out3 + row * ldo + v * 4) = (f16x4){(f16)z[0], (f16)z[1], (f16)z[2], (f16)z[3]};
+    }
+  }
+}
+
 __global__ __launch_bounds__(256) void add_split_f16_kernel(const float* __restrict__ a,
                                                             const float* __restrict__ b,
                                                             f16* __restrict__ o, int64_t n4, int64_t nb4,
@@ -91,6 +139,17 @@
     if (b) v += *(const f32x4*)(b + (i % nb4) * 4);
     if (o) *(f16x4*)(o + i * 4) = (f16x4){(f16)v[0], (f16)v[1], (f16)v[2], (f16)v[3]};
     if (of) *(f32x4*)(of + i * 4) = v;
+  }
+}
+
+__global__ __launch_bounds__(256) void add_cvt_f16_pair_kernel(const float* __restrict__ a, const float* __restrict__ b,
+                                                               f16* __restrict__ oa, f16* __restrict__ oab, int64_t n4,
+                                                               int64_t nb4) {
+  for (int64_t i = blockIdx.x * 256 + threadIdx.x; i < n4; i += (int64_t)gridDim.x * 256) {
+    const f32x4 v = *(const f32x4*)(a + i * 4);
+    const f32x4 s = v + *(const f32x4*)(b + (i % nb4) * 4);
+    *(f16x4*)(oa + i * 4) = (f16x4){(f16)v[0], (f16)v[1], (f16)v[2], (f16)v[3]};
+    *(f16x4*)(oab + i * 4) = (f16x4){(f16)s[0], (f16)s[1], (f16)s[2], (f16)s[3]};
   }
 }
 
@@ -126,6 +185,44 @@
   return ink_launch_status();
 }
 
+extern "C" int ink_layernorm_rows3(const float* x, int64_t ldx, const float* gamma, const float* beta, float eps,
+                                   int32_t rows_out, int32_t C, void* out_f16, float* out_f32, void* out3_f16,
+                                   int64_t ldo, int32_t act, const float* add3, int64_t ld_add3, void* stream) {
+  INK_CHECK_ARG(x && out3_f16 && add3);
+  INK_CHECK_ARG(act == INK_ACT_NONE || act == INK_ACT_GELU);
+  INK_CHECK_ARG(rows_out > 0 && C > 0 && C % 4 == 0 && C <= 2048);
+  INK_CHECK_ARG(ldx % 4 == 0 && ldo % 4 == 0 && ld_add3 % 4 == 0 && ldx >= C && ldo >= C && ld_add3 >= C);
+  INK_CHECK_ARG(ink_aligned<16>(x, gamma, beta, out_f32, add3) && ink_aligned<8>(out_f16, out3_f16));
+  const dim3 grid((rows_out + 3) / 4), block(256);
+  hipStream_t s = (hipStream_t)stream;
+  const int nv = (C / 4 + 63) / 64;
+#define INK_LN3(NV)                                                                                       \
+  hipLaunchKernelGGL(layernorm_rows3_kernel<NV>, grid, block, 0, s, x, ldx, gamma, beta, eps, rows_out, C, \
+                     (f16*)out_f16, out_f32, (f16*)out3_f16, ldo, act, add3, ld_add3)
+  switch (nv) {
+    case 1: INK_LN3(1); break;
+    case 2: INK_LN3(2); break;
+    case 3: INK_LN3(3); break;
+    case 4: INK_LN3(4); break;
+    case 5: INK_LN3(5); break;
+    default: INK_LN3(8); break;
+  }
+#undef INK_LN3
+  return ink_launch_status();
+}
+
+extern "C" int ink_add_cvt_f16_pair(const float* a, const float* b, int64_t n_b, void* out_a_f16, void* out_ab_f16,
+                                    int64_t n, void* stream) {
+  INK_CHECK_ARG(a && b && out_a_f16 && out_ab_f16 && n > 0 && n % 4 == 0);
+  INK_CHECK_ARG(n_b > 0 && n_b % 4 == 0 && n % n_b == 0);
+  INK_CHECK_ARG(ink_aligned<16>(a, b) && ink_aligned<8>(out_a_f16, out_ab_f16));
+  const int64_t n4 = n / 4;
+  const int blocks = (int)((n4 + 255) / 256 < 2048 ? (n4 + 255) / 256 : 2048);
+  hipLaunchKernelGGL(add_cvt_f16_pair_kernel, dim3(blocks), dim3(256), 0, (hipStream_t)stream, a, b,
+                     (f16*)out_a_f16, (f16*)out_ab_f16, n4, n_b / 4);
+  return ink_launch_status();
+}
+
 extern "C" int ink_add_cvt_f16(const float* a, const float* b, int64_t n_b, void* out_f16,
                                int64_t n, void* stream) {
   INK_CHECK_ARG(a && out_f16 && n > 0 && n % 4 == 0);
diff --git a/inklayer_amd/gdino.py b/inklayer_amd/gdino.py
--- a/inklayer_amd/gdino.py
+++ b/inklayer_amd/gdino.py
@@ -328,6 +328,8 @@
     fuse_ffn = True
     fuse_ffn_pre = True
     fold_fusion = True
+    grouped_launches = True
+    hoist_value = True
 
     def __init__(self, state_dict: Dict[str, torch.Tensor], cfg: Optional[GDinoConfig] = None,
                  device: str | torch.device = "cuda", encoded_text: Optional[torch.Tensor] = None,
@@ -810,9 +812,14 @@
                 ov, ol = ops.biattn_wide_varlen(qv, kl, B, S, tb.Tmax, tb.t_len, 256 ** -0.5)
             src = ops.gemm(ov, w[d + ".fu.outv.w"], w[d + ".fu.outv.b"], col_scale=w[d + ".fu.gv"], residual=vn, out=vn)
         text = ops.gemm(ol, w[d + ".fu.outl.w"], w[d + ".fu.outl.b"], col_scale=w[d + ".fu.gl"], residual=ln32)
-        qk = ops.gemm(ops.add_cvt_f16(text, self.pos_text if tb is None else tb.pos_text), w[d + ".txt.qk.w"],
-                      w[d + ".txt.qk.b"], out_dtype=F16)
-        vv = ops.gemm(ops.add_cvt_f16(text), w[d + ".txt.v.w"], w[d + ".txt.v.b"], out_dtype=F16)
+        pos_text = self.pos_text if tb is None else tb.pos_text
+        if self.grouped_launches:
+            t16, tp16 = ops.add_cvt_f16_pair(text, pos_text)
+            qk, vv = ops.gemm_grouped([dict(a=tp16, w=w[d + ".txt.qk.w"], bias=w[d + ".txt.qk.b"], out_dtype=F16),
+                                       dict(a=t16, w=w[d + ".txt.v.w"], bias=w[d + ".txt.v.b"], out_dtype=F16)])
+        else:
+            qk = ops.gemm(ops.add_cvt_f16(text, pos_text), w[d + ".txt.qk.w"], w[d + ".txt.qk.b"], out_dtype=F16)
+            vv = ops.gemm(ops.add_cvt_f16(text), w[d + ".txt.v.w"], w[d + ".txt.v.b"], out_dtype=F16)
         if tb is None:
             a = self._text_attn(qk[:, :256], qk[:, 256:], vv, B=B, n_heads=4, head_dim=64, scale=64 ** -0.5,
                                 blocked=self.text_blocked)
@@ -824,7 +831,12 @@
         ff = ops.gemm(ops.add_cvt_f16(text), w[d + ".txt.lin1.w"], w[d + ".txt.lin1.b"], act="relu", out_dtype=F16)
         text = ops.layernorm_rows(ops.gemm(ff, w[d + ".txt.lin2.w"], w[d + ".txt.lin2.b"], residual=text),
                                   w[d + ".txt.norm2.w"], w[d + ".txt.norm2.b"], 1e-5, out_dtype=F32)
-        if have16:
+        if self.grouped_launches:
+            if not have16:
+                ops.add_cvt_f16_pair(src, pl.pos, out_a=s16, out_ab=s16p)
+            proj, val = ops.gemm_grouped([dict(a=s16p, w=w[d + ".msda.proj.w"], bias=w[d + ".msda.proj.b"]),
+                                          dict(a=s16, w=w[d + ".msda.value.w"], bias=w[d + ".msda.value.b"], out_dtype=F16)])
+        elif have16:
             proj = ops.gemm(s16p, w[d + ".msda.proj.w"], w[d + ".msda.proj.b"])
             val = ops.gemm(s16, w[d + ".msda.value.w"], w[d + ".msda.value.b"], out_dtype=F16)
         else:
@@ -862,8 +874,7 @@
             tw16[:, :T] = text16.view(B, T, 256)
             tw16 = tw16.view(B * Tc, 256)
         logits = torch.empty((B, S, Tc), device=dev, dtype=F32)
-        for b in range(B):
-            ops.gemm(omn16[b * S:(b + 1) * S], tw16[b * Tc:(b + 1) * Tc], tbias[b], out=logits[b])
+        self._contrastive(omn16, S, tw16, Tc, tbias, logits)
         idx = ops.topk_rowmax(logits, nq)
         if stages is not None:
             stages["topk_logits"] = logits if Tc == T else logits[:, :, :T]
@@ -880,8 +891,15 @@
         hs16 = None
         if stages is not None:
             stages["hs"], stages["refs"] = [], [ref.clone()]
+        kvs = vals = [None] * cfg.dec_layers
+        if self.grouped_launches:
+            kvs = ops.gemm_grouped([dict(a=text16, w=w[f"d{i}.ca.kv.w"], bias=w[f"d{i}.ca.kv.b"], out_dtype=F16)
+                                    for i in range(cfg.dec_layers)])
+            if self.hoist_value:
+                vals = ops.gemm_grouped([dict(a=mem16, w=w[f"d{i}.msda.value.w"], bias=w[f"d{i}.msda.value.b"],
+                                              out_dtype=F16) for i in range(cfg.dec_layers)])
         for i in range(cfg.dec_layers):
-            output = self._dec_layer(i, output, ref, mem16, text16, pl, B)
+            output = self._dec_layer(i, output, ref, mem16, text16, pl, B, kv=kvs[i], val=vals[i])
             if stages is not None:
                 stages["hs"].append(output.clone())
             if i < cfg.dec_layers - 1:
@@ -894,17 +912,27 @@
                 hs16 = ops.layernorm_rows(output, w["dec.norm.w"], w["dec.norm.b"], 1e-5)
         boxes = ops.box_refine(self._mlp3("box", hs16), ref).view(B, nq, 4)
         out_logits = torch.empty((B, nq, Tc), device=dev, dtype=F32)
-        for b in range(B):
-            ops.gemm(hs16[b * nq:(b + 1) * nq], tw16[b * Tc:(b + 1) * Tc], tbias[b], out=out_logits[b])
+        self._contrastive(hs16, nq, tw16, Tc, tbias, out_logits)
         return (out_logits if Tc == T else out_logits[:, :, :T]), boxes
 
+    def _contrastive(self, rows16: torch.Tensor, n: int, tw16: torch.Tensor, Tc: int, tbias, out: torch.Tensor) -> None:
+        probs = [dict(a=rows16[b * n:(b + 1) * n], w=tw16[b * Tc:(b + 1) * Tc], bias=tbias[b], out=out[b])
+                 for b in range(out.shape[0])]
+        if self.grouped_launches:
+            ops.gemm_grouped(probs)
+        else:
+            for pr in probs:
+                ops.gemm(**pr)
+
     def _dec_layer(self, i: int, output: torch.Tensor, ref: torch.Tensor, mem16: torch.Tensor, text16: torch.Tensor,
-                   pl: _Plan, B: int) -> torch.Tensor:
+                   pl: _Plan, B: int, kv: Optional[torch.Tensor] = None, val: Optional[torch.Tensor] = None) -> torch.Tensor:
         w = self.w
         nq = output.shape[0] // B
         d = f"d{i}"
         qse = ops.sine_embed4(ref, w["dim_t"])
         qpos = ops.gemm(ops.gemm(qse, w["rph0.w"], w["rph0.b"], act="relu", out_dtype=F16), w["rph1.w"], w["rph1.b"])
+        if self.grouped_launches:
+            return self._dec_layer_grouped(d, output, qpos, ref, mem16, text16, pl, B, nq, kv, val)
         qk = ops.gemm(ops.add_cvt_f16(output, qpos), w[d + ".sa.qk.w"], w[d + ".sa.qk.b"], out_dtype=F16)
         vv = ops.gemm(ops.add_cvt_f16(output), w[d + ".sa.v.w"], w[d + ".sa.v.b"], out_dtype=F16)
         a = ops.flash_attn(qk[:, :256], qk[:, 256:], vv, n_batch=B, n_heads=8, head_dim=32, scale=32 ** -0.5,
@@ -929,6 +957,48 @@
         output = ops.layernorm_rows(ops.gemm(ff, w[d + ".lin2.w"], w[d + ".lin2.b"], residual=output),
                                     w[d + ".norm3.w"], w[d + ".norm3.b"], 1e-5, out_dtype=F32)
         return output
+
+    def _dec_layer_grouped(self, d: str, output: torch.Tensor, qpos: torch.Tensor, ref: torch.Tensor, mem16: torch.Tensor,
+                           text16: torch.Tensor, pl: _Plan, B: int, nq: int, kv: Optional[torch.Tensor],
+                           val: Optional[torch.Tensor]) -> torch.Tensor:
+        w, dev = self.w, self.dev
+
+        def norm(x, name, plain16=None, pos16=None):
+            out = torch.empty_like(x)
+            if pos16 is not None:
+                ops.layernorm_rows(x, w[name + ".w"], w[name + ".b"], 1e-5, out=out, out3=pos16, add3=qpos)
+            else:
+                ops.layernorm_rows(x, w[name + ".w"], w[name + ".b"], 1e-5, out=out, out2=plain16)
+            return out
+
+        def f16_like(x):
+            return torch.empty(x.shape, device=dev, dtype=F16)
+
+        o16, op16 = ops.add_cvt_f16_pair(output, qpos)
+        qk, vv = ops.gemm_grouped([dict(a=op16, w=w[d + ".sa.qk.w"], bias=w[d + ".sa.qk.b"], out_dtype=F16),
+                                   dict(a=o16, w=w[d + ".sa.v.w"], bias=w[d + ".sa.v.b"], out_dtype=F16)])
+        a = ops.flash_attn(qk[:, :256], qk[:, 256:], vv, n_batch=B, n_heads=8, head_dim=32, scale=32 ** -0.5,
+                           n_q=nq, n_k=nq)
+        op16 = f16_like(output)
+        output = norm(ops.gemm(a, w[d + ".sa.out.w"], w[d + ".sa.out.b"], residual=output), d + ".norm2", pos16=op16)
+        q = ops.gemm(op16, w[d + ".ca.q.w"], w[d + ".ca.q.b"], out_dtype=F16)
+        if kv is None:
+            kv = ops.gemm(text16, w[d + ".ca.kv.w"], w[d + ".ca.kv.b"], out_dtype=F16)
+        if self._tb is None:
+            a = self._text_attn(q, kv[:, :256], kv[:, 256:], B=B, n_heads=8, head_dim=32, scale=32 ** -0.5)
+        else:
+            a = ops.attn_midkeys_varlen(q, kv[:, :256], kv[:, 256:], B=B, n_heads=8, head_dim=32, scale=32 ** -0.5,
+                                        k_len=self._tb.t_len)
+        op16 = f16_like(output)
+        output = norm(ops.gemm(a, w[d + ".ca.out.w"], w[d + ".ca.out.b"], residual=output), d + ".canorm", pos16=op16)
+        proj = ops.gemm(op16, w[d + ".msda.proj.w"], w[d + ".msda.proj.b"])
+        if val is None:
+            val = ops.gemm(mem16, w[d + ".msda.value.w"], w[d + ".msda.value.b"], out_dtype=F16)
+        o = ops.msda_fused(val, proj, ref, pl.shapes, B, nq, ref_batched=True)
+        o16 = f16_like(output)
+        output = norm(ops.gemm(o, w[d + ".msda.out.w"], w[d + ".msda.out.b"], residual=output), d + ".norm1", plain16=o16)
+        ff = ops.gemm(o16, w[d + ".lin1.w"], w[d + ".lin1.b"], act="relu", out_dtype=F16)
+        return norm(ops.gemm(ff, w[d + ".lin2.w"], w[d + ".lin2.b"], residual=output), d + ".norm3")
 
     def forward(self, images_u8: Sequence[torch.Tensor], stages: Optional[dict] = None, allow_graph: bool = True):
         B = len(images_u8)
diff --git a/inklayer_amd/ops.py b/inklayer_amd/ops.py
--- a/inklayer_amd/ops.py
+++ b/inklayer_amd/ops.py
@@ -56,11 +56,11 @@
     return t.data_ptr()
 
 
-def gemm(a: torch.Tensor, w: torch.Tensor, bias: Optional[torch.Tensor] = None, *,
-         act: Optional[str] = None, residual: Optional[torch.Tensor] = None,
-         col_scale: Optional[torch.Tensor] = None, row_map: Optional[torch.Tensor] = None,
-         out: Optional[torch.Tensor] = None, out_dtype: torch.dtype = F32,
-         out_rows: Optional[int] = None) -> torch.Tensor:
+def _gemm_problem(a: torch.Tensor, w: torch.Tensor, bias: Optional[torch.Tensor] = None, *,
+                  act: Optional[str] = None, residual: Optional[torch.Tensor] = None,
+                  col_scale: Optional[torch.Tensor] = None, row_map: Optional[torch.Tensor] = None,
+                  out: Optional[torch.Tensor] = None, out_dtype: torch.dtype = F32,
+                  out_rows: Optional[int] = None):
     assert a.dtype == F16 and w.dtype == F16
     assert a.dim() == 2 and w.dim() == 2 and a.stride(1) == 1 and w.stride(1) == 1
     M, K = a.shape
@@ -88,6 +88,18 @@
     p.act = ACT[act]
     p.c_f16 = 1 if out.dtype == F16 else 0
     assert out.dtype in (F16, F32)
+    key = (M, N, K, act or '-', 'res' if residual is not None else '-', 'map' if row_map is not None else '-',
+           'f16' if p.c_f16 else 'f32')
+    return p, out, key
+
+
+def gemm(a: torch.Tensor, w: torch.Tensor, bias: Optional[torch.Tensor] = None, *,
+         act: Optional[str] = None, residual: Optional[torch.Tensor] = None,
+         col_scale: Optional[torch.Tensor] = None, row_map: Optional[torch.Tensor] = None,
+         out: Optional[torch.Tensor] = None, out_dtype: torch.dtype = F32,
+         out_rows: Optional[int] = None) -> torch.Tensor:
+    p, out, key = _gemm_problem(a, w, bias, act=act, residual=residual, col_scale=col_scale, row_map=row_map, out=out,
+                                out_dtype=out_dtype, out_rows=out_rows)
     if _GEMM_TRACE is None:
         check(_lib.lib().ink_gemm_f16(C.byref(p), _stream()), "ink_gemm_f16")
     else:
@@ -95,9 +107,39 @@
         e0.record()
         check(_lib.lib().ink_gemm_f16(C.byref(p), _stream()), "ink_gemm_f16")
         e1.record()
-        _GEMM_TRACE.append((2.0 * M * N * K, e0, e1, (M, N, K, act or '-', 'res' if residual is not None else '-',
-                                                      'map' if row_map is not None else '-', 'f16' if p.c_f16 else 'f32')))
-    return out
+        _GEMM_TRACE.append((2.0 * key[0] * key[1] * key[2], e0, e1, key))
+    return out
+
+
+GEMM_GROUP_MAX = 8
+GEMM_MIXED = 3
+
+
+def gemm_grouped(problems: Sequence[dict]) -> list:
+    built = [_gemm_problem(**pr) for pr in problems]
+    for c0 in range(0, len(built), GEMM_GROUP_MAX):
+        chunk = built[c0:c0 + GEMM_GROUP_MAX]
+        if all(b[0].M == 0 for b in chunk):
+            continue
+        n = len(chunk)
+        arr = (InkGemm * n)(*(b[0] for b in chunk))
+        rows = (C.c_int32 * n)(*(b[1].shape[0] for b in chunk))
+        traced = _GEMM_TRACE is not None
+        if traced:
+            e0, e1 = torch.cuda.Event(enable_timing=True), torch.cuda.Event(enable_timing=True)
+            e0.record()
+        rc = _lib.lib().ink_gemm_grouped(arr, rows, n, _stream())
+        if rc == GEMM_MIXED:
+            for pr, (p, out, _) in zip(problems[c0:c0 + GEMM_GROUP_MAX], chunk):
+                if p.M > 0:
+                    gemm(**{**pr, "out": out})
+            continue
+        check(rc, "ink_gemm_grouped")
+        if traced:
+            e1.record()
+            big = max((b[2] for b in chunk), key=lambda k: k[0] * k[1] * k[2])
+            _GEMM_TRACE.append((sum(2.0 * b[2][0] * b[2][1] * b[2][2] for b in chunk), e0, e1, big + ('group', n)))
+    return [b[1] for b in built]
 
 
 def layernorm_rows(x: torch.Tensor, gamma: Optional[torch.Tensor], beta: Optional[torch.Tensor],
@@ -106,7 +148,8 @@
                    out2: Optional[torch.Tensor] = None, act: Optional[str] = None,
                    split: bool = False, add: Optional[torch.Tensor] = None,
                    add_batch_rows: Optional[torch.Tensor] = None, rows_per_batch: int = 0,
-                   split_f32: Optional[torch.Tensor] = None) -> torch.Tensor:
+                   split_f32: Optional[torch.Tensor] = None, out3: Optional[torch.Tensor] = None,
+                   add3: Optional[torch.Tensor] = None) -> torch.Tensor:
     assert x.dtype == F32 and x.dim() == 2 and x.stride(1) == 1
     Cdim = x.shape[1]
     rows = gather.numel() if gather is not None else x.shape[0]
@@ -128,6 +171,15 @@
         assert split and out.stride(0) == 3 * Cdim and split_f32.dtype == F32 and split_f32.is_contiguous()
         assert tuple(split_f32.shape) == (rows, Cdim)
         of = split_f32.data_ptr()
+    if out3 is not None:
+        assert gather is None and add is None and not split and add3 is not None
+        assert out3.dtype == F16 and out3.shape == out.shape and out3.stride() == out.stride()
+        assert add3.dtype == F32 and add3.shape == out.shape and add3.stride(1) == 1
+        check(_lib.lib().ink_layernorm_rows3(x.data_ptr(), x.stride(0), _p(gamma), _p(beta), eps, rows, Cdim, oh, of,
+                                             out3.data_ptr(), out.stride(0), ACT[act], add3.data_ptr(), add3.stride(0),
+                                             _stream()), "ink_layernorm_rows3")
+        return out
+    assert add3 is None
     if gather is not None:
         assert gather.dtype == torch.int32
     if add is not None:
@@ -157,6 +209,21 @@
     check(_lib.lib().ink_add_cvt_f16(a.data_ptr(), _p(b), nb, out.data_ptr(), a.numel(), _stream()),
           "ink_add_cvt_f16")
     return out
+
+
+def add_cvt_f16_pair(a: torch.Tensor, b: torch.Tensor, out_a: Optional[torch.Tensor] = None,
+                     out_ab: Optional[torch.Tensor] = None) -> Tuple[torch.Tensor, torch.Tensor]:
+    assert a.dtype == F32 and a.is_contiguous()
+    assert b.dtype == F32 and b.is_contiguous() and a.numel() % b.numel() == 0
+    if out_a is None:
+        out_a = torch.empty(a.shape, device=a.device, dtype=F16)
+    if out_ab is None:
+        out_ab = torch.empty(a.shape, device=a.device, dtype=F16)
+    for o in (out_a, out_ab):
+        assert o.dtype == F16 and o.is_contiguous() and o.numel() == a.numel()
+    check(_lib.lib().ink_add_cvt_f16_pair(a.data_ptr(), b.data_ptr(), b.numel(), out_a.data_ptr(), out_ab.data_ptr(),
+                                          a.numel(), _stream()), "ink_add_cvt_f16_pair")
+    return out_a, out_ab
 
 
 def add_split_f16(a: torch.Tensor, b: Optional[torch.Tensor] = None) -> torch.Tensor:
```

Result: no change. 116.9 sketches/s (median of 6 runs) (+0.3%).
